# disanda/Deep-GAN-Encoders

Hardware: AMD Instinct MI355X
Metric: encoder-train images/sec (E_align_s2 step, StyleGAN2 FFHQ-1024) (higher is better)
Workload: dtype bf16; 1 GPU; E_align_s2 two-phase step, StyleGAN2-1024 G (train mode) + BE(startf=16, L=9) + LPIPS-VGG16 (seeded stand-in weights), batch 8/GPU; global_batch=8, img_size=1024, parallelism=dp1

## Files before the change

### deep-gan-encoders_amd/_lib.py

```python
import ctypes as C
import os

_HERE = os.path.dirname(os.path.abspath(__file__))
LIB_PATH = os.environ.get("DGE_LIB_PATH", os.path.join(_HERE, "libdge_hip.so"))


class DgeError(RuntimeError):
    pass


class ConvDesc(C.Structure):
    _fields_ = [
        ("x", C.c_void_p), ("w_packed", C.c_void_p), ("y", C.c_void_p), ("addend", C.c_void_p), ("dot_src", C.c_void_p),
        ("in_scale", C.c_void_p), ("in_shift", C.c_void_p), ("out_scale", C.c_void_p),
        ("bias", C.c_void_p), ("noise", C.c_void_p), ("noise_w", C.c_void_p), ("stats", C.c_void_p),
        ("B", C.c_int), ("H", C.c_int), ("W", C.c_int), ("Cin", C.c_int), ("Cout", C.c_int),
        ("ksize", C.c_int), ("up", C.c_int), ("in_s2d", C.c_int), ("noise_batch", C.c_int), ("noise_w_per_channel", C.c_int),
        ("act", C.c_int), ("bias_scale", C.c_float), ("gain", C.c_float), ("add_scale", C.c_float),
        ("dtype", C.c_int), ("in_up2", C.c_int), ("in_relu", C.c_int), ("stats_slots", C.c_int), ("w_layout", C.c_int),
        ("prep", C.c_int), ("prep_gain", C.c_float), ("prep_noise", C.c_void_p), ("prep_ns", C.c_void_p), ("prep_noise_batch", C.c_int),
        ("prep_stats", C.c_void_p), ("mask_relu", C.c_int), ("in_t2d", C.c_int),
        ("rgb_w", C.c_void_p), ("rgb_style", C.c_void_p), ("rgb_bias", C.c_void_p), ("rgb_out", C.c_void_p), ("rgb_wscale", C.c_float),
        ("rgb_skip_y", C.c_int), ("pool_out", C.c_int), ("pool_mask", C.c_void_p),
        ("prefetch_w", C.c_void_p), ("prefetch_ntot", C.c_int), ("prefetch_cin", C.c_int), ("in_bwd_coef", C.c_void_p),
        ("in_bwd_extra", C.c_void_p), ("in_bwd_extra_scale", C.c_float), ("fr_img4", C.c_void_p), ("fr_out", C.c_void_p),
    ]


class ConvPPDesc(C.Structure):
    _fields_ = [
        ("x", C.c_void_p), ("w_pp", C.c_void_p), ("y", C.c_void_p), ("w_bstride", C.c_longlong),
        ("out_scale", C.c_void_p), ("bias", C.c_void_p), ("noise", C.c_void_p), ("noise_w", C.c_void_p),
        ("B", C.c_int), ("H", C.c_int), ("W", C.c_int), ("Cin", C.c_int), ("Cout", C.c_int),
        ("noise_batch", C.c_int), ("noise_w_per_channel", C.c_int), ("act", C.c_int), ("bias_scale", C.c_float), ("gain", C.c_float),
        ("dgrad", C.c_int), ("in_s2d", C.c_int), ("stats_slots", C.c_int), ("prep", C.c_int), ("prep_noise_batch", C.c_int), ("mask_relu", C.c_int),
        ("in_t2d", C.c_int), ("add_scale", C.c_float), ("prep_gain", C.c_float),
        ("dot_src", C.c_void_p), ("addend", C.c_void_p), ("stats", C.c_void_p), ("prep_stats", C.c_void_p), ("prep_noise", C.c_void_p), ("prep_ns", C.c_void_p),
    ]


class DenseLayer(C.Structure):
    _fields_ = [("w", C.c_void_p), ("bias", C.c_void_p), ("I", C.c_int), ("O", C.c_int), ("wscale", C.c_float), ("bscale", C.c_float),
                ("add", C.c_float), ("act", C.c_int), ("gain", C.c_float)]


class S2GradEntry(C.Structure):
    _fields_ = [("P", C.c_void_p), ("st", C.c_void_p), ("d", C.c_void_p), ("s", C.c_void_p), ("bias", C.c_void_p), ("wsq", C.c_void_p),
                ("gs", C.c_void_p), ("wstyle", C.c_void_p),
                ("nslot_p", C.c_int), ("nslot_s", C.c_int), ("in_c", C.c_int), ("out_c", C.c_int), ("row", C.c_int), ("bscale", C.c_float)]


class SumPlanarEntry(C.Structure):
    _fields_ = [("partial", C.c_void_p), ("out", C.c_void_p), ("nslot", C.c_int), ("C", C.c_int), ("NS", C.c_int), ("pad", C.c_int)]


class NoisePlan(C.Structure):
    _fields_ = [("maps", C.c_void_p), ("jobs", C.c_void_p), ("nmaps", C.c_int), ("Bn", C.c_int), ("n_pool0", C.c_int), ("n_pool1", C.c_int),
                ("n_mom", C.c_int), ("npairs", C.c_int), ("n_chunk", C.c_int), ("pad", C.c_int), ("n_total", C.c_longlong),
                ("lev_total", C.c_longlong)]


_P, _I, _F = C.c_void_p, C.c_int, C.c_float
SIGNATURES = {
    "dge_conv2d": [C.POINTER(ConvDesc), _P],
    "dge_fir_t2d": [_P, _P, _P, _I, _I, _I, _I, _I, _P],
    "dge_up_dgrad_small": [C.POINTER(ConvDesc), _P],
    "dge_up_dgrad_small_supported": [_I, _I, _I, _I, _I, _I],
    "dge_s2_style_grads": [C.POINTER(S2GradEntry), _I, _P, _I, _I, _I, _F, _P],
    "dge_conv_small_supported": [_I, _I, _I, _I, _I, _I, _I, _I],
    "dge_torgb_bwd_prep": [_P, _P, _P, _P, _P, _P, _I, _P, _P, _P, _I, _I, _I, _F, _F, _I, _P],
    "dge_demod_bwd_prep": [_P, _I, _P, _P, _P, _I, _I, _F, _P],
    "dge_sum_slots": [_P, _P, _I, _I, _I, _P],
    "dge_sum_slots_planar": [_P, _P, _I, _I, _I, _P],
    "dge_set_deterministic": [_I],
    "dge_get_deterministic": [],
    "dge_packed_n": [_I],
    "dge_pack_conv_weight": [_P, _P, _I, _I, _I, _I, _I, _F, _P],
    "dge_pack_conv_weights_multi": [_P, _P, _I, _I, _P],
    "dge_pack_desc_bytes": [],
    "dge_weight_sumsq": [_P, _P, _I, _I, _I, _F, _P],
    "dge_linear": [_P, _I, _P, _P, _P, _I, _I, _I, _I, _F, _F, _F, _I, _F, _I, _P],
    "dge_pixelnorm": [_P, _P, _I, _I, _F, _P],
    "dge_truncation": [_P, _P, _P, _I, _I, _I, _F, _I, _I, _P],
    "dge_torgb": [_P, _P, _P, _P, _P, _P, _I, _I, _I, _I, _F, _I, _P],
    "dge_conv_rgb_supported": [_I, _I, _I, _I, _I, _I, _I],
    "dge_conv_in_bwd_supported": [_I, _I, _I, _I, _I, _I, _I],
    "dge_conv_in_bwd_fromrgb_supported": [_I, _I, _I, _I, _I, _I, _I],
    "dge_conv_in_bwd_x_supported": [_I, _I, _I, _I, _I, _I, _I],
    "dge_conv_pool_supported": [_I, _I, _I, _I, _I, _I, _I],
    "dge_rgb_upsample_add": [_P, _P, _I, _I, _I, _P],
    "dge_nchw_to_nhwc": [_P, _P, _I, _I, _I, _I, _I, _P],
    "dge_nhwc_to_nchw": [_P, _P, _I, _I, _I, _I, _P],
    "dge_fromrgb": [_P, _P, _P, _P, _P, _I, _I, _I, _I, _P],
    "dge_fromrgb2": [_P, _P, _P, _P, _P, _P, _I, _I, _I, _I, _P],
    "dge_stats_finalize": [_P, _P, _P, _P, _I, _I, _I, _F, _P],
    "dge_stats_finalize_slots": [_P, _I, _P, _P, _P, _I, _I, _I, _F, _P],
    "dge_blend": [_P, _P, _P, _P, _P, _P, _I, _I, _I, _I, _I, _F, _F, _I, _P],
    "dge_loss_reduce": [_P, _P, _P, _I, _I, _I, _I, _I, _I, _I, _I, _P],
    "dge_ssim_fwd": [_P, _P, _P, _P, _I, _I, _I, _P],
    "dge_ssim_box7": [_P, _P, _P, _I, _I, _I, _F, _F, _F, _P],
    "dge_ssim_bwd": [_P, _P, _P, _P, _I, _I, _I, _F, _I, _P],
    "dge_space_loss_finalize": [_P, _P, _P, _P, _F, _F, _I, _P],
    "dge_space_loss_bwd": [_P, _P, _P, _P, _P, _I, _I, _I, _I, _I, _I, _I, _I, _F, _F, _I, _P],
    "dge_axpy_scalar": [_P, _P, _P, C.c_long, _F, _I, _P],
    "dge_lreq_adam_multi": [_I, _P, _P, _P, _P, _P, _F, _F, _P, _P, _P],
    "dge_modconv_bwd_prep": [_P, _P, _P, _P, _P, _P, _I, _I, _I, _I, _F, _I, _P],
    "dge_demod_bwd": [_P, _P, _P, _P, _P, _I, _I, _F, _P],
    "dge_linear_t": [_P, _I, _I, _P, _P, _P, _I, _I, _I, _I, _I, _F, _I, _P],
    "dge_torgb_bwd": [_P, _P, _P, _P, _P, _P, _I, _I, _I, _F, _I, _P],
    "dge_up2_bwd": [_P, _P, _I, _I, _I, _P],
    "dge_conv_wgrad": [_P, _P, _P, _P, _P, _I, _I, _I, _I, _I, _I, _I, _P],
    "dge_act_bwd": [_P, _P, _P, _P, _P, _I, _I, _I, _I, _I, _I, _F, _F, _I, _P],
    "dge_in_bwd_coef": [_P, _P, _P, _P, _P, _P, _I, _I, _I, _P],
    "dge_in_bwd_coef_slots": [_P, _I, _P, _P, _P, _P, _P, _I, _I, _I, _P],
    "dge_in_bwd": [_P, _P, _P, _P, _P, _P, _P, _I, _I, _I, _I, _I, _F, _I, _I, _P],
    "dge_chan_sum": [_P, _P, _I, _I, _I, _F, _I, _P],
    "dge_fromrgb_bwd": [_P, _P, _P, _P, _I, _I, _I, _I, _P],
    "dge_head_entry_size": [],
    "dge_heads_bwd": [_P, _I, _I, _P, _I, _P, _P, _P, _P, _I, _I, _P],
    "dge_head_rows_entry_size": [],
    "dge_heads_rows_fwd": [_P, _I, _P, _P, C.c_long, C.c_long, _I, _I, _I, _P],
    "dge_heads_rows_bwd": [_P, _I, _I, _P, C.c_long, C.c_long, _I, _P, _P, _P, _P, _I, _I, _P],
    "dge_dense_wgrad": [_P, _I, _P, _I, _P, _P, _I, _I, _I, _I, _P],
    "dge_lpips_prep": [_P, _P, _I, _I, _I, _P, _P, _I, _P],
    "dge_lpips_prep_bwd": [_P, _P, _I, _I, _I, _P, _F, _I, _I, _P],
    "dge_maxpool2": [_P, _P, _I, _I, _I, _I, _I, _P],
    "dge_maxpool2_bwd": [_P, _P, _P, _P, _I, _I, _I, _I, _I, _P],
    "dge_lpips_head": [_P, _P, _P, _P, _I, _I, _I, _F, _I, _P],
    "dge_mean": [_P, _P, _I, _P],
    "dge_blur_noise_act": [_P, _P, _P, _P, _P, _P, _I, _I, _I, _I, _I, _I, _I, _I, _P],
    "dge_affine_compose": [_P, _P, _P, _P, _P, _I, _I, _P],
    "dge_lerp_layers": [_P, _P, _I, _P, _P, _I, _I, _I, _P],
    "dge_linear_rows": [_P, _I, _P, _P, _P, _P, _P, _P, _I, _I, _I, _F, _F, _F, _P],
    "dge_demod_rows": [_P, _P, _P, _P, _P, _P, _P, _P, _I, _I, _F, _P],
    "dge_fromrgb_dgrad": [_P, _P, _P, _P, _I, _I, _I, _I, _P],
    "dge_nearest_up2": [_P, _P, _I, _I, _I, _I, _F, _I, _P],
    "dge_sg1_in_bwd_coef": [_P, _P, _P, _P, _P, _P, _I, _I, _I, _P],
    "dge_dot_stats": [_P, _P, _P, _I, _I, _I, _I, _P],
    "dge_nearest_up2_bwd": [_P, _P, _P, _P, _I, _I, _I, _I, _I, _P],
# ... 4 lines not shown
    "dge_slice_up_bwd": [_P, _P, _I, _I, _I, _I, _I, _I, _I, _P],
    "dge_softmax_rows": [_P, C.c_long, _I, _I, _P],
    "dge_softmax_rows_bwd": [_P, _P, C.c_long, _I, _I, _P],
    "dge_rgb_tanh_bwd": [_P, _P, _P, _I, _I, _I, _I, _P],
    "dge_sn_group": [_P, _I, _I, _I, _P, _F, _I, _P],
    "dge_sn_entry_size": [],
    "dge_cbn_sn_wgrad_entry_size": [],
    "dge_cbn_sn_wgrad_group": [_P, _I, C.c_longlong, _I, _P, _I, _I, _P, _P],
    "dge_upconv_supported": [_I, _I, _I],
    "dge_pack_upconv_weight": [_P, _P, _I, _I, _F, _I, _P],
    "dge_upconv_fir": [_P, _P, _P, _P, _P, _P, _I, _P, _I, _P, _F, _F, _I, _I, _I, _I, _I, _I, _I, _P],
    "dge_up_dgrad_stream_supported": [_I, _I, _I, _I, _I, _I],
    "dge_up_dgrad_stream": [_P, _P, _P, _P, _P, _P, _P, _P, _I, _I, _F, _P, _I, _P, _P, _I, _I, _I, _I, _I, _I, _P],
    "dge_cbn_affine": [_P, _P, _I, _P, _P, _F, _P, _P, _I, _I, _P],
    "dge_slice_up": [_P, _P, _I, _I, _I, _I, _I, _I, _I, _P],
    "dge_attention": [_P, _P, _P, _P, _I, _I, _I, _I, _I, _I, _P],
    "dge_rgb_tanh": [_P, _P, _I, _I, _I, _I, _P],
    "dge_guided_relu_bwd": [_P, _P, _P, C.c_long, _I, _I, _P],
    "dge_maxpool2_relu_bwd": [_P, _P, _P, _I, _I, _I, _I, _I, _I, _P],
    "dge_maxpool2_bwd_relu": [_P, _P, _P, _P, _I, _I, _I, _I, _I, _P],
    "dge_adaptive_pool7": [_P, _P, _I, _I, _I, _I, _I, _P],
    "dge_adaptive_pool7_bwd": [_P, _P, _I, _I, _I, _I, _I, _P],
    "dge_class_target": [_P, _P, _P, _P, _I, _I, _P],
    "dge_gather_row": [_P, _P, _P, _I, _I, _F, _P],
    "dge_class_target_rows": [_P, _P, _P, _P, _I, _I, _P],
    "dge_gather_rows": [_P, _P, _P, _I, _I, _P],
    "dge_campp_map": [_P, _P, _P, _P, _P, _I, _I, _I, _I, _I, _P],
    "dge_cam_resize": [_P, _P, _P, _I, _I, _I, _I, _I, _P],
    "dge_mask2cam_blocks": [_I],
    "dge_mask2cam": [_P, _P, _P, _P, _P, _P, _P, _I, _I, _P],
    "dge_mask2cam_rows": [_P, _P, _P, _P, _P, _P, _I, _I, _P],
    "dge_class_target_groups": [_P, _P, _P, _P, _I, _I, _I, _P],
    "dge_gather_row_groups": [_P, _P, _P, _I, _I, _I, _F, _P],
    "dge_mask2cam_groups": [_P, _P, _P, _P, _P, _P, _P, _I, _I, _I, _P],
    "dge_randn": [_P, _I, _P, _P, _P, _P, C.c_ulonglong, _P, _P],
    "dge_version": [],
    "dge_env_reload": [],
    "dge_blend_pool_mask": [_P, _P, _P, _P, _P, _I, _I, _I, _I, _F, _F, _I, _P],
    "dge_act_bwd_mask": [_P, _P, _P, _P, _P, _I, _I, _I, _I, _I, _F, _F, _I, _P],
    "dge_loss_reduce3": [_P, _P, _P, _I, _I, _I, _I, _P, _I, _P],
    "dge_crop_pool_multi": [_P, _P, _P, _P, _I, _I, _I, _I, _P],
    "dge_space_loss_bwd3": [_P, _P, _P, _P, _P, _I, _I, _I, _P, _P, _P, _P, _I, _P],
    "dge_space_loss_bwd_split": [_P, _P, _P, _P, _P, _I, _I, _I, _P, _P, _P, _P, _I, _P],
    "dge_in_bwd_fromrgb": [_P, _P, _P, _I, _P, _P, _P, _P, _I, _P, _P, _P, _I, _I, _I, _I, _I, _F, _I, _P],
    "dge_in_bwd_fromrgb_img": [_P, _P, _P, _I, _P, _P, _P, _P, _I, _P, _P, _P, _P, _P, _I, _I, _I, _I, _I, _F, _I, _P],
    "dge_affine_bwd_fromrgb_img": [_P, _P, _P, _P, _P, _P, _P, _P, _I, _I, _I, _I, _I, _F, _I, _P],
    "dge_in_bwd_fused": [_P, _P, _P, _I, _P, _P, _P, _P, _I, _P, _P, _P, _P, _I, _I, _I, _I, _I, _F, _I, _I, _P],
    "dge_sum_slots_planar_multi": [C.POINTER(SumPlanarEntry), _I, _P],
    "dge_heads_fwd": [_P, _I, _P, _P, _I, _I, _I, _P],
    "dge_conv_pp_supported": [_I, _I, _I, _I, _I, _I],
    "dge_pack_conv_pp": [_P, _P, _I, _I, _F, _P, _P, _F, _I, _I, _P],
    "dge_dense_chain": [_P, _I, C.POINTER(DenseLayer), _I, _P, _I, _I, _I, _F, _P],
    "dge_conv_wgrad_dots": [_P, _P, _P, _P, _P, _P, _P, _I, _I, _I, _I, _I, _I, _I, _P],
    "dge_pack_conv_pp_rows": [_P, _I, _P, _I, _I, _P, _I, _P, _F, _I, _I, _P],
    "dge_conv_pp": [C.POINTER(ConvPPDesc), _P],
    "dge_up_pp_supported": [_I, _I, _I, _I, _I, _I],
    "dge_pack_up_pp": [_P, _P, _I, _I, _P, _P, _F, _I, _P],
    "dge_up_pp": [_P, _P, C.c_longlong, _P, _P, _I, _P, _P, _F, _F, _I, _I, _I, _I, _I, _I, _P],
    "dge_latent_pnorm_fwd": [_P, _P, _P, C.c_long, _I, _P],
    "dge_latent_pnorm_bwd": [_P, _P, _P, _P, C.c_long, _I, _F, _P],
    "dge_wplus_lerp": [_P, _P, _I, _F, _P, _I, _I, _I, _P],
    "dge_wplus_lerp_bwd": [_P, _F, _P, C.c_long, _I, _P],
    "dge_embed_track": [_P, _P, _P, C.c_long, _P, _P, _P, _P, _P, _I, _I, _I, _F, _F, _P],
    "dge_loss_reduce_rows": [_P, _P, _P, _I, _I, _I, _I, _P, _I, _I, _P],
    "dge_ssim_fwd_rows": [_P, _P, _P, _P, _I, _I, _I, _P],
    "dge_space_loss_finalize_rows": [_P, _I, _P, _P, _P, _P, _P, _I, _I, _P, _P, _I, _P],
    "dge_space_loss_bwd_rows": [_P, _P, _P, _P, _P, _I, _I, _I, _I, _P, _P, _P, _P, _I, _I, _P],
    "dge_latent_pnorm_rows_fwd": [_P, _P, _P, _I, C.c_long, _I, _P],
    "dge_latent_pnorm_rows_bwd": [_P, _P, _P, _P, _I, C.c_long, _I, _F, _P],
    "dge_embed_track_rows": [_P, _P, _P, _I, C.c_long, _P, _P, _P, _P, _P, _I, _I, _I, _F, _F, _P],
    "dge_mapping_bwd": [_P, _I, C.POINTER(DenseLayer), _I, _P, _P, _I, _P, _P, _I, _I, _I, _F, _P],
    "dge_mapping_bwd_wide_work_bytes": [_I],
    "dge_mapping_bwd_wide": [_P, _I, C.POINTER(DenseLayer), _I, _P, _P, _I, _P, _P, _I, _I, _I, _F, _P, C.c_longlong, _P],
    "dge_quantize_u8": [_P, _I, _P, _I, _I, _I, _I, _P],
    "dge_image_metrics_u8_work_bytes": [_I, _I, _I],
    "dge_image_metrics_u8": [_P, _P, _I, _I, _I, _P, _P, _P, _P, _P],
    "dge_minmax_unit_slots": [C.c_long],
    "dge_minmax_unit": [_P, _P, C.c_long, _P, _P],
    "dge_s2_noise_grad": [_P, _P, _P, _P, _I, _I, _I, _I, _F, _I, _I, _P],
    "dge_noise_map_size": [],
    "dge_noise_job_size": [],
    "dge_noise_reg_work_bytes": [C.POINTER(NoisePlan)],
    "dge_noise_reg": [C.POINTER(NoisePlan), _P, _P, _P, _F, _I, _P, C.c_longlong, _P],
    "dge_noise_normalize_work_bytes": [C.POINTER(NoisePlan)],
    "dge_noise_normalize": [C.POINTER(NoisePlan), _P, _P, C.c_longlong, _P],
    "dge_adam_multi": [_I, _P, _P, _P, _P, _P, C.c_double, C.c_double, _F, _F, _F, _P, _P],
    "dge_w_broadcast": [_P, _P, _F, _P, _P, _I, _I, _I, _P],
    "dge_w_broadcast_bwd": [_P, _P, _I, _I, _I, _P],
    "dge_rows_mean_std_work_bytes": [C.c_longlong, _I],
    "dge_rows_mean_std": [_P, C.c_longlong, _I, _P, _P, _P, C.c_longlong, _P],
    "dge_area_pool_bwd": [_P, _P, _I, _I, _I, _I, _P],
}

_lib = None


def lib():
    global _lib
    if _lib is None:
        if not os.path.exists(LIB_PATH):
            raise DgeError(f"{LIB_PATH} is missing: build it with deep-gan-encoders_amd/csrc/build.sh "
                           "(__graft_entry__.build()). There is no fallback path.")
        _lib = C.CDLL(LIB_PATH)
        for name, args in SIGNATURES.items():
            fn = getattr(_lib, name)
            fn.argtypes = args
# ... 19 lines not shown
```

### deep-gan-encoders_amd/autograd_enc_bwd.py

```python
import os
from types import SimpleNamespace

import torch

from . import ops
from .enc_steps import blocks, conv_bwd, grads_in_order, heads_backward, red_param_grads, skip_bwd
from .weight_cache import pack_cache, packed

FUSE_IN_BWD = not os.environ.get("DGE_NO_FUSED_IN_BWD")
FUSE_IMG_GRAD = not os.environ.get("DGE_NO_FUSED_IMG_GRAD")

FROMRGB, BLOCK_INPUT, SEPARATE = "FromRGB reduction", "block input", "separate passes"


def _conv2_part(c, blk, rec, pre, Cc, C2, H, g_out, gms2):
    B, dev, dt, grads, params = c.B, c.dev, c.dt, c.grads, c.params
    x1 = rec["x1"]
    extra, extra_pool, extra_scale = None, False, 1.0
    g_pre2 = g_y2 = dots2 = None
    fuse2 = False
    if blk.has_last_conv:
        has3 = Cc != C2
        red2 = ops.zeros((3 if has3 else 2, C2), dev) if params else None
        g_pre2 = ops.act_bwd_mask(g_out, rec["m2"], rec["n2"], scale=0.111 * 0.25, red=red2, planar=True, defer=c.later)
        sum_g = red_param_grads(grads, pre, 2, red2, planar=True) if params else None
        gW2 = ops.zeros(tuple(blk.conv_2.weight.shape), dev) if params else None
        dots2 = ops.SlotStats(B, Cc, dev)
        if params and FUSE_IN_BWD and ops.conv_in_bwd_supported(B, H, H, C2, Cc, dt):
            fuse2 = ops.conv_wgrad_dots(g_pre2, x1, gW2, rec["sc2"], rec["sh2"], blk.conv_2.weight, dots2)
        if fuse2:
            grads[pre + "conv_2.weight"] = gW2
        else:
            g_y2, _ = conv_bwd(c.cache, grads, pre + "conv_2", blk.conv_2, g_pre2, x1, dt, H, rec["sc2"], rec["sh2"], params, dots=dots2,
                               dw=gW2)
        if has3:
            extra = skip_bwd(c.cache, grads, pre, blk, g_out, rec["xp"], dt, sum_g, params, post=c.post)
            extra_pool, extra_scale = True, 0.25
        else:
            extra, extra_pool, extra_scale = g_out, True, 0.889 * 0.25
    elif g_out is not None:
        if Cc != C2:
            raise ops.DgeError("E.BE: a gradient on the const output of a last block with a channel change (conv_3 on the unpooled "
                               "input) is not implemented; not reachable with maxf-clamped widths")
        g_y2 = ops.blend(g_out, alpha=0.111)
        dots2 = ops.dot_stats(g_y2, x1)
        extra, extra_pool, extra_scale = g_out, False, 0.889
    coef2 = (dots2, gms2, rec["musig2"], rec["sc2"], rec["sh2"], H * H)
    red1 = ops.zeros((2, Cc), dev) if params else None
    if fuse2:
        redp = ops.SlotStats(B, Cc, dev)
        g_pre1 = ops.conv2d(g_pre2, packed(c.cache, blk.conv_2, dt, ops.PACK_DGRAD, H), Cc, 3, dot_src=x1,
                            in_bwd=dict(coef=ops.in_bwd_coef(*coef2), noise=rec["n1"].reshape(B, H, H), red=redp))
        ops._sum_planar(redp.buf.view(-1, Cc, 2), red1, c.later)
    else:
        g_pre1 = ops.in_bwd(g_y2, x1, coef2, noise=rec["n1"], act=True, red=red1, planar=True, defer=c.later)
    if params:
        red_param_grads(grads, pre, 1, red1, planar=True)
    return g_pre1, extra, extra_pool, extra_scale


def _conv1_form(c, j, Cc, H, extra, extra_pool):
    if not FUSE_IN_BWD or not c.params:
        return SEPARATE
    if j == 0 and c.need_img:
        return SEPARATE
    if j == 0:
        ok = c.saved.get("img4") is not None and ops.conv_in_bwd_fromrgb_supported(c.B, H, H, Cc, Cc, c.dt)
        return FROMRGB if ok else SEPARATE
    ok = (extra is None or extra_pool) and ops.conv_in_bwd_x_supported(c.B, H, H, Cc, Cc, c.dt)
    return BLOCK_INPUT if ok else SEPARATE


def _img_grad_fused(c, Cc):
    return FUSE_IMG_GRAD and ops.in_bwd_fromrgb_img_supported(Cc, c.dt)


def _conv1_part(c, j, blk, rec, pre, Cc, H, g_pre1, gms1, extra, extra_pool, extra_scale):
    B, dev, dt, grads = c.B, c.dev, c.dt, c.grads
    x = rec["x"]
    gW1 = ops.zeros(tuple(blk.conv_1.weight.shape), dev) if c.params else None
    dots1 = ops.SlotStats(B, Cc, dev)
    form = _conv1_form(c, j, Cc, H, extra, extra_pool)
    if form != SEPARATE:
        covered = ops.conv_wgrad_dots(g_pre1, x, gW1, rec["sc1"], rec["sh1"], blk.conv_1.weight, dots1)
        if covered:
            grads[pre + "conv_1.weight"] = gW1
        else:
            form = SEPARATE
    coef1 = (dots1, gms1, rec["musig1"], rec["sc1"], rec["sh1"], H * H)
    if form == FROMRGB:
        frh = ops.SlotStats(B, Cc, dev)
        ops.conv2d(g_pre1, packed(c.cache, blk.conv_1, dt, ops.PACK_DGRAD, H), Cc, 3, dot_src=x, out=x.new_empty((1, 1, 1, 1)),
                   in_bwd=dict(coef=ops.in_bwd_coef(*coef1), fr=frh, img4=c.saved["img4"], extra=extra if extra_pool else None,
                               extra_scale=extra_scale))
        return None, ops._sum_planar(frh.buf.view(-1, Cc, 4), torch.empty((4, Cc), dtype=torch.float32, device=dev), c.later)
    if form == BLOCK_INPUT:
        return ops.conv2d(g_pre1, packed(c.cache, blk.conv_1, dt, ops.PACK_DGRAD, H), Cc, 3, dot_src=x,
                          in_bwd=dict(coef=ops.in_bwd_coef(*coef1), extra=extra, extra_scale=extra_scale)), None
    g_y1, _ = conv_bwd(c.cache, grads, pre + "conv_1", blk.conv_1, g_pre1, x, dt, H, rec["sc1"], rec["sh1"], c.params, dots=dots1, dw=gW1)
    if j == 0 and c.need_img and _img_grad_fused(c, Cc):
        c.g_img, fr = ops.in_bwd_fromrgb_img(g_y1, x, coef1, c.E.FromRGB.from_rgb.weight.detach(), c.saved["img"].float() if c.params else None,
                                             extra=extra, extra_pool=extra_pool, extra_scale=extra_scale, defer=c.later)
        return None, fr
    if j == 0 and Cc <= 512 and c.params and not c.need_img:
        return None, ops.in_bwd_fromrgb(g_y1, x, coef1, c.saved["img"].float(), extra=extra, extra_pool=extra_pool,
# ... 48 lines not shown
```

### deep-gan-encoders_amd/csrc/capi.hip

```cpp
#include <stdarg.h>
#include <stdio.h>
#include "common.h"
#include "conv_params.h"
#include "../../include/dge_hip.h"

static thread_local char g_err[512] = "";
void dge_set_error(const char* fmt, ...) {
    va_list ap; va_start(ap, fmt); vsnprintf(g_err, sizeof(g_err), fmt, ap); va_end(ap);
}
extern "C" const char* dge_last_error(void) { return g_err; }
static thread_local char g_kernel[160] = "";
void dge_note_kernel(const char* fmt, ...) {
    va_list ap; va_start(ap, fmt); vsnprintf(g_kernel, sizeof(g_kernel), fmt, ap); va_end(ap);
}
extern "C" const char* dge_last_kernel(void) { return g_kernel; }
extern "C" int dge_version(void) { return 100; }

#include <vector>
static std::vector<void (*)(const DgeDet*)>& det_setters() { static std::vector<void (*)(const DgeDet*)> v; return v; }
void dge_det_register(void (*setter)(const DgeDet*)) { det_setters().push_back(setter); }
static DgeDet g_det_host = {0, nullptr, nullptr, 0, 0};
int dge_det_upload_failed = 0;
bool dge_det_fits(long long ndomains, long long nslots, long long L) {
    return !g_det_host.enabled || (ndomains * nslots * L <= g_det_host.ws_floats && ndomains <= (long long)g_det_host.ncounters);
// ... 41 lines not shown
}
#include <mutex>
static std::once_flag g_env_once;
const DgeEnv& dge_env() { std::call_once(g_env_once, [] { if (!g_env_loaded) env_load(); }); return g_env; }
extern "C" void dge_env_reload(void) { env_load(); }

static int conv_desc_to_params(const dge_conv_desc* d, ConvParams& p, bool units) {
    DGE_CHECK(d && d->x && d->w_packed && d->y, "conv2d: null tensor");
    DGE_CHECK(d->B > 0 && d->H > 0 && d->W > 0 && d->Cin > 0 && d->Cout > 0, "conv2d: bad shape");
    DGE_CHECK(d->dtype == DGE_F32 || d->dtype == DGE_BF16, "conv2d: bad dtype %d", d->dtype);
    DGE_CHECK(!(d->up && d->stats), "conv2d: stats are not available in up mode");
    DGE_CHECK(!(d->up && d->in_s2d), "conv2d: up and in_s2d are exclusive");
    DGE_CHECK(!d->in_up2 || (!d->in_s2d && d->H % 2 == 0 && d->W % 2 == 0), "conv2d: in_up2 needs even H, W and no in_s2d");
    DGE_CHECK(!d->in_s2d || d->Cin % 4 == 0, "conv2d: in_s2d needs Cin %% 4 == 0");
    DGE_CHECK(!d->dot_src || d->stats || d->mask_relu || d->in_bwd_coef, "conv2d: dot_src needs a stats buffer");
    DGE_CHECK(!d->mask_relu || (d->dot_src && !d->prep && !d->up), "conv2d: mask_relu needs dot_src and excludes prep / up");
    DGE_CHECK(!d->in_relu || d->in_scale || d->in_shift, "conv2d: in_relu is applied together with the prologue affine");
    DGE_CHECK(d->gain > 0.f, "conv2d: gain must be positive (it is folded through the activation)");
    DGE_CHECK((((uintptr_t)d->in_scale | (uintptr_t)d->in_shift) & 15) == 0, "conv2d: in_scale/in_shift must be 16-byte aligned");
    DGE_CHECK(!d->noise || d->noise_w, "conv2d: noise without noise_w");
    p.x = d->x; p.w = d->w_packed; p.y = d->y; p.addend = d->addend; p.dot_src = d->dot_src;
    p.in_scale = d->in_scale; p.in_shift = d->in_shift; p.out_scale = d->out_scale;
    p.bias = d->bias; p.noise = d->noise; p.noise_w = d->noise_w; p.stats = d->stats;
    p.B = d->B; p.H = d->H; p.W = d->W; p.Cin = d->Cin; p.Cout = d->Cout;
    p.Ntot_valid = d->up ? 4 * d->Cout : d->Cout;
    p.Ntot = dge_packed_n(p.Ntot_valid);
    p.up = d->up; p.in_s2d = d->in_s2d; p.in_up2 = d->in_up2; p.in_relu = d->in_relu;
    const int OH = d->up ? 2 * d->H : d->H, OW = d->up ? 2 * d->W : d->W;
    p.noise_bstride = d->noise_batch > 1 ? OH * OW : 0;
    p.noise_w_stride = d->noise_w_per_channel ? 1 : 0;
    p.act = d->act; p.bias_scale = d->bias_scale; p.gain = d->gain; p.add_scale = d->add_scale;
    p.tiles_x = p.tiles_y = 0;
    p.w_frag = d->w_layout == 1 ? 1 : 0;
    p.prep = d->prep ? 1 : 0;
    p.mask_relu = d->mask_relu ? 1 : 0;
    p.in_t2d = d->in_t2d ? 1 : 0;
    DGE_CHECK(!d->in_t2d || (d->ksize == 3 && !d->up && !d->in_s2d && !d->in_up2 && !d->in_scale && !d->in_shift && (d->w_layout == 0 || units)),
              "conv2d: in_t2d is a plain 3x3 launch (no other read mode, no prologue affine, row-major weights)");
    p.prep_gain = d->prep_gain; p.prep_noise = d->prep_noise; p.prep_ns = d->prep_ns; p.prep_stats = d->prep_stats;
    p.prep_noise_bstride = d->prep_noise_batch > 1 ? OH * OW : 0;
    DGE_CHECK(!d->prep || (d->dot_src && d->prep_stats && d->prep_gain > 0.f && !d->up), "conv2d: prep needs dot_src, prep_stats, a positive prep_gain and no up mode");
    DGE_CHECK(!d->prep || !dge_get_deterministic(), "conv2d: the fused tail backward (prep) is not offered in deterministic mode; run dge_modconv_bwd_prep");
    DGE_CHECK(d->w_layout == 0 || d->w_layout == 1, "conv2d: bad w_layout %d", d->w_layout);
    p.stats_slots = d->stats_slots > 0 ? d->stats_slots : 1;
    p.rgb_w = d->rgb_out ? d->rgb_w : nullptr; p.rgb_style = d->rgb_style; p.rgb_bias = d->rgb_bias; p.rgb_out = d->rgb_out;
    p.rgb_wscale = d->rgb_wscale; p.rgb_skip_y = (d->rgb_out && d->rgb_skip_y) ? 1 : 0;
    p.pool_out = d->pool_out ? 1 : 0; p.pool_mask = d->pool_out ? (unsigned*)d->pool_mask : nullptr;
    const bool pf = d->w_layout == 1 && d->prefetch_w && d->prefetch_ntot >= 64 && d->prefetch_ntot % 64 == 0 &&
                    (d->prefetch_cin == 512 || d->prefetch_cin == 256);
    p.pf_w = pf ? d->prefetch_w : nullptr; p.pf_ntot = pf ? d->prefetch_ntot : 0; p.pf_cin = pf ? d->prefetch_cin : 0;
    p.in_coef = d->in_bwd_coef;
    p.in_extra = d->in_bwd_coef ? d->in_bwd_extra : nullptr; p.in_extra_scale = d->in_bwd_extra_scale;
    p.fr_img4 = d->in_bwd_coef ? d->fr_img4 : nullptr; p.fr_out = d->in_bwd_coef ? d->fr_out : nullptr;
    if (d->in_bwd_coef) {
        DGE_CHECK(!dge_get_deterministic(), "conv2d: in_bwd_coef is not offered in deterministic mode; run dge_in_bwd");
        DGE_CHECK(d->ksize == 3 && !d->up && dge_conv_stream_eligible(p, d->dtype, d->ksize), "conv2d: in_bwd_coef is offered where "
                  "dge_conv_in_bwd_supported() says so, with dot_src and prep_stats, without stats / prep");
    }
    if (d->pool_out)
        DGE_CHECK(!d->up && dge_conv_pool_ok(p, d->dtype, d->ksize), "conv2d: the pooled epilogue is offered where dge_conv_pool_supported() "
                  "says so (conv_2 of the first encoder blocks on the streaming kernel)");
    if (d->rgb_out) {
        DGE_CHECK(d->rgb_w && d->rgb_style && d->rgb_bias, "conv2d: rgb_out needs rgb_w, rgb_style, rgb_bias");
        DGE_CHECK(dge_conv_rgb_ok(p, d->dtype, d->ksize), "conv2d: the fused toRGB is offered where dge_conv_rgb_supported() says so "
                  "(bf16 3x3 32 -> 32 launches of the streaming kernel)");
    }
    return 0;
}

extern "C" int dge_conv2d(const dge_conv_desc* d, hipStream_t s) {
    ConvParams p;
    if (const int rc = conv_desc_to_params(d, p, false)) return rc;
    return dge_conv_launch(p, d->dtype, d->ksize, s);
}

extern "C" int dge_up_dgrad_small(const dge_conv_desc* d, hipStream_t s) {
    DGE_CHECK(d && d->in_t2d && d->w_layout == 1 && d->ksize == 3 && d->Cin % 4 == 0, "up_dgrad_small: an in_t2d launch with fragment-ordered unit weights");
    DGE_CHECK(!d->bias && !d->noise && d->act == DGE_ACT_NONE && !d->mask_relu && !d->in_bwd_coef && !d->rgb_out && !d->pool_out && !d->in_relu,
              "up_dgrad_small: data-gradient epilogue only (out_scale, addend, dot_src + stats, prep)");
    DGE_CHECK(dge_up_dgrad_small_supported(d->B, d->H, d->W, d->Cin / 4, d->Cout, d->dtype),
              "up_dgrad_small: unsupported launch %dx%d, %d <- %d channels, dtype %d", d->H, d->W, d->Cout, d->Cin / 4, d->dtype);
    ConvParams p;
    if (const int rc = conv_desc_to_params(d, p, true)) return rc;
    p.Cin = d->Cin / 4;
    return dge_up_dgrad_small_launch(p, s);
}

extern "C" int dge_conv_pool_supported(int B, int H, int W, int Cin, int Cout, int ksize, int dtype) {
    ConvParams p = {};
    p.B = B; p.H = H; p.W = W; p.Cin = Cin; p.Cout = Cout; p.Ntot_valid = Cout; p.Ntot = dge_packed_n(Cout);
    p.in_shift = (const float*)16; p.noise_w_stride = 1;
    return dge_conv_pool_ok(p, dtype, ksize) ? 1 : 0;
}

extern "C" int dge_conv_in_bwd_supported(int B, int H, int W, int Cin, int Cout, int ksize, int dtype) {
    ConvParams p = {};
    p.B = B; p.H = H; p.W = W; p.Cin = Cin; p.Cout = Cout; p.Ntot_valid = Cout; p.Ntot = dge_packed_n(Cout);
    p.dot_src = (const void*)16; p.prep_stats = (float*)16; p.in_coef = (const float*)16;
    return (ksize == 3 && !dge_get_deterministic() && dge_conv_stream_eligible(p, dtype, ksize)) ? 1 : 0;
}
extern "C" int dge_conv_in_bwd_x_supported(int B, int H, int W, int Cin, int Cout, int ksize, int dtype) {
    ConvParams p = {};
    p.B = B; p.H = H; p.W = W; p.Cin = Cin; p.Cout = Cout; p.Ntot_valid = Cout; p.Ntot = dge_packed_n(Cout);
    p.dot_src = (const void*)16; p.in_coef = (const float*)16;
    return (ksize == 3 && !dge_get_deterministic() && dge_conv_stream_eligible(p, dtype, ksize)) ? 1 : 0;
}
extern "C" int dge_conv_in_bwd_fromrgb_supported(int B, int H, int W, int Cin, int Cout, int ksize, int dtype) {
    ConvParams p = {};
    p.B = B; p.H = H; p.W = W; p.Cin = Cin; p.Cout = Cout; p.Ntot_valid = Cout; p.Ntot = dge_packed_n(Cout);
    p.dot_src = (const void*)16; p.in_coef = (const float*)16; p.fr_img4 = (const float*)16; p.fr_out = (float*)16;
    return (ksize == 3 && !dge_get_deterministic() && dge_conv_stream_eligible(p, dtype, ksize)) ? 1 : 0;
}

extern "C" int dge_conv_rgb_supported(int B, int H, int W, int Cin, int Cout, int ksize, int dtype) {
    ConvParams p = {};
    p.B = B; p.H = H; p.W = W; p.Cin = Cin; p.Cout = Cout; p.Ntot_valid = Cout; p.Ntot = dge_packed_n(Cout);
    return dge_conv_rgb_ok(p, dtype, ksize) ? 1 : 0;
}

__global__ void sum_slots_kernel(const float* __restrict__ partial, float* __restrict__ out, int nslot, int n, int accumulate) {
    const int i = blockIdx.x * blockDim.x + threadIdx.x;
    if (i >= n) return;
    float s = 0.f;
    int k = 0;
    for (; k + 8 <= nslot; k += 8) {
        float v[8];
#pragma unroll
        for (int j = 0; j < 8; j++) v[j] = partial[(size_t)(k + j) * n + i];
#pragma unroll
        for (int j = 0; j < 8; j++) s += v[j];
    }
    for (; k < nslot; k++) s += partial[(size_t)k * n + i];
    out[i] = accumulate ? out[i] + s : s;
}
__global__ void sum_slots_planar_kernel(const float* __restrict__ partial, float* __restrict__ out, int nslot, int C, int NS) {
    const int i = blockIdx.x * blockDim.x + threadIdx.x;
    if (i >= C * NS) return;
    float s = 0.f;
    int k = 0;
    for (; k + 8 <= nslot; k += 8) {
        float v[8];
#pragma unroll
        for (int j = 0; j < 8; j++) v[j] = partial[(size_t)(k + j) * C * NS + i];
#pragma unroll
        for (int j = 0; j < 8; j++) s += v[j];
    }
    for (; k < nslot; k++) s += partial[(size_t)k * C * NS + i];
    out[(size_t)(i % NS) * C + i / NS] = s;
}
extern "C" int dge_sum_slots_planar(const float* partial, float* out, int nslot, int C, int NS, hipStream_t s) {
    DGE_CHECK(nslot >= 1 && C >= 1 && NS >= 1, "sum_slots_planar: bad sizes");
    hipLaunchKernelGGL(sum_slots_planar_kernel, dim3((C * NS + 255) / 256), dim3(256), 0, s, partial, out, nslot, C, NS);
    DGE_LAUNCH_CHECK("sum_slots_planar");
// ... 40 lines not shown
```

### deep-gan-encoders_amd/csrc/conv_params.h

```cpp
#pragma once
#include <hip/hip_runtime.h>

struct ConvParams {
    const void* x;
    const void* w;
    void* y;
    const void* addend;
    const void* dot_src;
    const float* in_scale;
    const float* in_shift;
    const float* out_scale;
    const float* bias;
    const float* noise;
    const float* noise_w;
    float* stats;
    int stats_slots;
    int B, H, W, Cin, Cout;
    int Ntot;
    int Ntot_valid;
    int up;
    int in_s2d;
    int in_relu;
    int in_up2;
    int noise_bstride;
    int noise_w_stride;
    int act;
    float bias_scale, gain, add_scale;
    int tiles_x, tiles_y;
    int dbg;
    int w_frag;
    int prep;
    float prep_gain;
    const float* prep_noise;
    const float* prep_ns;
    int prep_noise_bstride;
    float* prep_stats;
    int mask_relu;
    int in_t2d;
    const float* rgb_w;
    const float* rgb_style;
    const float* rgb_bias;
    float* rgb_out;
    float rgb_wscale;
    int rgb_skip_y;
    int pool_out;
    unsigned* pool_mask;
    const void* pf_w;
    int pf_ntot, pf_cin;
    const float* in_coef;
    const void* in_extra; float in_extra_scale; const float* fr_img4; float* fr_out;
};

int dge_conv_launch(const ConvParams& p, int dtype, int ksize, hipStream_t s);
extern "C" int dge_conv_ntile(int ntot);

bool dge_conv_stream_eligible(const ConvParams& p, int dtype, int ksize);
int dge_conv_stream_launch(const ConvParams& p, hipStream_t s);
bool dge_conv_rgb_ok(const ConvParams& p, int dtype, int ksize);
bool dge_conv_pool_ok(const ConvParams& p, int dtype, int ksize);
bool dge_conv_small_shape_ok(int H, int W, int cin, int ntot, int ksize, int in_s2d, int in_up2, int dtype);
int dge_conv_small_launch(const ConvParams& p, hipStream_t s);
extern "C" int dge_up_dgrad_small_supported(int B, int H, int W, int C, int N, int dtype);
int dge_up_dgrad_small_launch(const ConvParams& p, hipStream_t s);
bool dge_conv_pw_eligible(const ConvParams& p, int dtype, int ksize);
int dge_conv_pw_launch(const ConvParams& p, hipStream_t s);
```

### deep-gan-encoders_amd/csrc/conv_stream.hip

```cpp
#include <type_traits>
#include "common.h"
#include <stdlib.h>
#include "conv_params.h"

namespace {

typedef __attribute__((ext_vector_type(4))) unsigned rsrc_t;
#define DGE_LDS " lds\n\t"

__device__ __forceinline__ unsigned rfl(unsigned v) { return __builtin_amdgcn_readfirstlane(v); }
__device__ __forceinline__ unsigned lds_off(const void* p) {
    return (unsigned)(size_t)(const __attribute__((address_space(3))) unsigned char*)p;
}
constexpr int ilog2(int v) { return v <= 1 ? 0 : 1 + ilog2(v >> 1); }

__device__ __forceinline__ rsrc_t make_rsrc(unsigned long long base, unsigned bytes) {
    rsrc_t r;
    r[0] = rfl((unsigned)base); r[1] = rfl((unsigned)(base >> 32) & 0xffffu); r[2] = rfl(bytes); r[3] = 0x00020000u;
    return r;
}

#define DGE_P(off) "buffer_load_dwordx4 %1, %3, 0 offen offset:" #off " lds\n\t"
#define DGE_PB(off) "buffer_load_dwordx4 %4, %3, 0 offen offset:" #off " lds\n\t"
#define DGE_M0 "s_mov_b32 m0, %2\n\ts_nop 0\n\t"
#define DGE_MASK(m) "s_mov_b64 %0, exec\n\ts_mov_b64 exec, " #m "\n\t"
#define DGE_UNMASK "s_mov_b64 exec, %0"
template <int CIN, int TEAM>
__device__ __forceinline__ void dma_row(int wave, unsigned voff, unsigned voff_b, unsigned voff_c, rsrc_t rs, rsrc_t rs_null,
                                        unsigned m0v, unsigned m0_dummy) {
    unsigned long long keep;
    if constexpr (CIN == 16 && TEAM == 1) {
        asm volatile(DGE_M0 DGE_P(0) DGE_MASK(0xf) DGE_P(1024) DGE_UNMASK : "=&s"(keep) : "v"(voff), "s"(m0v), "s"(rs) : "memory");
    } else if constexpr (CIN == 16 && TEAM == 2) {
        if (wave == 0) asm volatile(DGE_M0 DGE_P(0) : "=&s"(keep) : "v"(voff), "s"(m0v), "s"(rs) : "memory");
        else asm volatile(DGE_M0 DGE_MASK(0xf) DGE_P(1024) DGE_UNMASK : "=&s"(keep) : "v"(voff), "s"(m0v), "s"(rs) : "memory");
    } else if constexpr (CIN == 32 && TEAM == 1) {
        asm volatile(DGE_M0 DGE_P(0) DGE_P(1024) DGE_MASK(0xff) DGE_P(2048) DGE_UNMASK : "=&s"(keep) : "v"(voff), "s"(m0v), "s"(rs) : "memory");
    } else if constexpr (CIN == 32 && TEAM == 2) {
        if (wave == 0) asm volatile(DGE_M0 DGE_P(0) DGE_MASK(0xff) DGE_P(2048) DGE_UNMASK : "=&s"(keep) : "v"(voff), "s"(m0v), "s"(rs) : "memory");
        else asm volatile(DGE_M0 DGE_P(1024) "s_mov_b32 m0, %5\n\ts_nop 0\n\tbuffer_load_dwordx4 %1, %4, 0 offen lds"
                          : "=&s"(keep) : "v"(voff), "s"(m0v), "s"(rs), "s"(rs_null), "s"(m0_dummy) : "memory");
    } else if constexpr (CIN == 64 && TEAM == 1) {
        asm volatile(DGE_M0 DGE_P(0) DGE_PB(1024) DGE_P(2048) DGE_PB(3072)
                     "s_mov_b32 m0, %6\n\t" DGE_MASK(0xffff) "buffer_load_dwordx4 %5, %3, 0 offen lds\n\t" DGE_UNMASK
                     : "=&s"(keep) : "v"(voff), "s"(m0v), "s"(rs), "v"(voff_b), "v"(voff_c), "s"(m0v + 4096u) : "memory");
    } else {
        if (wave == 0)
            asm volatile(DGE_M0 DGE_P(0) DGE_P(2048)
                         "s_mov_b32 m0, %5\n\t" DGE_MASK(0xffff) "buffer_load_dwordx4 %4, %3, 0 offen lds\n\t" DGE_UNMASK
                         : "=&s"(keep) : "v"(voff), "s"(m0v), "s"(rs), "v"(voff_c), "s"(m0v + 4096u) : "memory");
        else
            asm volatile(DGE_M0 DGE_P(1024) DGE_P(3072) "s_mov_b32 m0, %5\n\ts_nop 0\n\tbuffer_load_dwordx4 %1, %4, 0 offen lds"
                         : "=&s"(keep) : "v"(voff_b), "s"(m0v), "s"(rs), "s"(rs_null), "s"(m0_dummy) : "memory");
    }
}
__device__ __forceinline__ void dma_piece(unsigned voff, rsrc_t rs, unsigned m0v) {
    asm volatile("s_mov_b32 m0, %1\n\ts_nop 0\n\tbuffer_load_dwordx4 %0, %2, 0 offen lds" : : "v"(voff), "s"(m0v), "s"(rs) : "memory");
}
template <int NP> __device__ __forceinline__ void dma_dot(unsigned voff, unsigned voff1, rsrc_t rs, unsigned m0v) {
    if constexpr (NP == 1)
        asm volatile("s_mov_b32 m0, %1\n\ts_nop 0\n\tbuffer_load_dwordx4 %0, %2, 0 offen lds" : : "v"(voff), "s"(m0v), "s"(rs) : "memory");
    else
        asm volatile("s_mov_b32 m0, %1\n\ts_nop 0\n\tbuffer_load_dwordx4 %0, %2, 0 offen lds\n\t"
                     "buffer_load_dwordx4 %3, %2, 0 offen offset:1024 lds" : : "v"(voff), "s"(m0v), "s"(rs), "v"(voff1) : "memory");
}

enum { FL_GEN = 0, FL_ENC = 1, FL_ENC_STATS = 2, FL_DOT = 3, FL_DOT_PREP = 4, FL_GEN_RGB = 5, FL_ENC_POOL = 6, FL_DOT_IN = 7, FL_DOT_FR = 8, FL_DOT_INX = 9 };

template <int CIN, int COUT, int FL>
struct SC {
    static constexpr int PXB = CIN * 2, CH = PXB / 16, LOGCH = ilog2(CH), KS = CIN / 16;
    static constexpr int TEAM = COUT == 64 ? 2 : 1;
    static constexpr int TPW = 4 / TEAM;
    static constexpr int MT = COUT / 32 > 0 ? COUT / 32 : 1;
    static constexpr int MTW = MT / TEAM;
    static constexpr int HW = 34, RB = HW * PXB;
    static constexpr int PIECES = (RB + 1023) / 1024;
    static constexpr bool PREP = FL == FL_DOT_PREP, RGB = FL == FL_GEN_RGB, POOL = FL == FL_ENC_POOL, FRB = FL == FL_DOT_FR, INX = FL == FL_DOT_INX, INB = FL == FL_DOT_IN || FRB || INX;
    static_assert(!RGB || COUT == 32 || (COUT == 64 && TEAM == 2), "fused toRGB: 32 output channels per wave, one wave or a 2-wave team per pixel");
    static constexpr bool DOT = FL == FL_DOT || PREP || INB, STATS = FL == FL_ENC_STATS, ENC = FL == FL_ENC || FL == FL_ENC_STATS || POOL;
    static constexpr bool NOISE = !DOT || PREP || (INB && !FRB && !INX);
    static constexpr int NR = 6;
    static constexpr int dot_depth(int nr) { for (int d = 4; d >= 1; d--) if (d <= nr - 3 && nr % (d + 1) == 0) return d; return 1; }
    static constexpr int D = DOT ? dot_depth(6) : 2;
    static constexpr int DR = DOT ? D + 1 : NR;
    static_assert(NR % DR == 0, "dot ring period");
    static constexpr int CPB = COUT * 2;
    static constexpr int CW = COUT / TEAM >= 32 ? 32 : 16;
    static constexpr int DCH = CW * MTW * 2 / 16;
    static constexpr int LOGDCH = ilog2(DCH);
    static constexpr int DROWB = 32 * DCH * 16, DPIECES = DROWB / 1024;
    static_assert(!DOT || MTW == 1, "data-gradient mode: one M tile per wave");
    static constexpr int XPW = TEAM == 2 ? (PIECES + 1) / 2 : PIECES;
    static constexpr int LPR = XPW + (DOT ? DPIECES : 0) + (FRB ? 2 : 0) + (INX ? 1 : 0);
    static constexpr int X_OFF = 0;
    static constexpr int XRING = NR * RB;
    static constexpr int N_OFF = (XRING + 1023) / 1024 * 1024;
    static constexpr int NRING = NOISE ? 2048 : 0;
    static_assert(NR <= 8, "a noise piece holds 8 rows");
    static constexpr int D_OFF = N_OFF + TEAM * NRING;
    static constexpr int DRING = DOT ? DR * DROWB : 0;
    static constexpr int E_OFF = D_OFF + TEAM * DRING;
    static constexpr int ERING = FRB ? 2 * DR * 512 : (INX ? DR * 1024 : 0);
    static_assert(!INX || (CIN == COUT && CIN >= 32), "block-input flavour: 32 -> 32, 64 -> 64");
    static_assert(!FRB || (CIN == 16 && COUT == 16 && TEAM == 1), "FromRGB reduction flavour: 16 -> 16");
    static constexpr int T_OFF = E_OFF + TEAM * ERING;
    static constexpr int TBYTES = 32 * MTW * 16 * 4;
    static constexpr int DUMMY_OFF = T_OFF + TEAM * TBYTES;
    static constexpr int RGBX_OFF = DUMMY_OFF + (TEAM == 2 ? 1024 : 0);
    static constexpr int LDS_BYTES = RGBX_OFF + (RGB && TEAM == 2 ? 1024 : 0);
    static constexpr int NEED = 4 * 9 * KS * MTW + 32 * MTW + 16 + (ENC ? 16 * MTW : 0) + (STATS || DOT ? 32 * MTW : 0) + (DOT ? 16 : 0) + (PREP ? 16 : 0) + (RGB ? 11 : 0) + (POOL ? 20 * MTW : 0) + 36;
    static constexpr int WPE = ((PREP || INB) && CIN == 64) ? 1 : (NEED <= 128 ? 4 : (NEED <= 168 ? 3 : 2));
    static_assert(D <= NR - 3, "the slot of the row being fetched must be dead");
    static_assert((D - 1) * LPR + 1 < 64, "vmcnt range");
};

template <int LOGC> __device__ __forceinline__ int chunk_swz(int px) { return (px >> (4 - LOGC)) & ((1 << LOGC) - 1); }

template <int CW> __device__ __forceinline__ int chan_of_row(int m) {
    const int j = m >> 3, k = (m >> 2) & 1, i = m & 3;
    if (CW == 16) return j < 2 ? 8 * k + 4 * j + i : -1;
    return 16 * (j >> 1) + 8 * k + 4 * (j & 1) + i;
}

template <int CIN, int COUT, int FL>
__global__ __launch_bounds__((64 * SC<CIN, COUT, FL>::TEAM * SC<CIN, COUT, FL>::TPW), (SC<CIN, COUT, FL>::WPE))
void conv_stream_kernel(ConvParams p, int nstrips, int nseg, int seg_rows, int njobs, int jobs_per_xcd) {
    using C = SC<CIN, COUT, FL>;
    extern __shared__ __attribute__((aligned(1024))) unsigned char lds_all[];
#ifdef DGE_SC_TIMING
    const long long tj0 = __builtin_readcyclecounter();
#endif
    const int lane = threadIdx.x & 63;
    const int wid = (int)rfl(threadIdx.x >> 6);
    const int team = wid / C::TEAM;
    const int wave = wid % C::TEAM;
    unsigned char* __restrict__ lds = lds_all + team * C::LDS_BYTES;
    const unsigned lds0 = lds_off(lds_all) + team * C::LDS_BYTES;
    const int n31 = lane & 31, kh = lane >> 5;

    int job = ((blockIdx.x & 7) * jobs_per_xcd + (blockIdx.x >> 3)) * C::TPW + team;
    if ((blockIdx.x >> 3) >= jobs_per_xcd || job >= njobs) return;
    const int strip = job % nstrips; job /= nstrips;
    const int seg = job % nseg;
    const int b = job / nseg;
    const int x0 = strip * 32;
    const int r0 = seg * seg_rows;
    const int rows = min(seg_rows, p.H - r0);
    const bool full_strip = x0 + 32 <= p.W;
    const bool edge_strip = x0 == 0 || x0 + 32 >= p.W;

    const unsigned xrow_bytes = (unsigned)p.W * C::PXB, yrow_bytes = (unsigned)p.W * C::CPB;
    const unsigned long long Xb = (unsigned long long)p.x + (unsigned long long)b * p.H * xrow_bytes;
    unsigned char* __restrict__ Yb = (unsigned char*)p.y + (size_t)b * p.H * yrow_bytes;
    const float* __restrict__ nzsrc = (C::PREP || C::INB) ? p.prep_noise : p.noise;
    const unsigned long long NZb = nzsrc ? (unsigned long long)(nzsrc + (size_t)b * ((C::PREP || C::INB) ? p.prep_noise_bstride : p.noise_bstride)) : Xb;
    const unsigned nzrow_bytes = nzsrc ? (unsigned)p.W * 4 : 0;
    const unsigned long long DOTb = C::DOT ? (unsigned long long)p.dot_src + (unsigned long long)b * p.H * yrow_bytes : Xb;

    unsigned voff, voff_b = 0, voff_c = 0;
    {
        const int px = lane >> C::LOGCH, cs = lane & (C::CH - 1);
        const int gx = x0 - 1 + px;
        voff = (unsigned)(gx * C::PXB + ((cs ^ chunk_swz<C::LOGCH>(px)) << 4));
        if constexpr (CIN == 64) {
            voff_b = (unsigned)(gx * C::PXB + ((cs ^ chunk_swz<C::LOGCH>(px + 8)) << 4));
            voff_c = voff + 4096;
        }
    }
    const unsigned nvoff = (unsigned)(((lane >> 3) * p.W + x0 + (lane & 7) * 4) * 4);
    unsigned dvoff = 0, dvoff1 = 0;
    if constexpr (C::DOT) {
        const int px = lane >> C::LOGDCH, cs = lane & (C::DCH - 1);
        const int chunk0 = wave * 4;
        dvoff = (unsigned)((x0 + px) * C::CPB + ((chunk0 + (cs ^ chunk_swz<C::LOGDCH>(px))) << 4));
        constexpr int PPP = 64 / C::DCH;
        dvoff1 = (unsigned)((x0 + px + PPP) * C::CPB + ((chunk0 + (cs ^ chunk_swz<C::LOGDCH>(px + PPP))) << 4)) - 1024u;
    }
    const rsrc_t rs_null = make_rsrc(Xb, 0);
    const unsigned exrow_bytes = (C::FRB || C::INX) ? (unsigned)(p.W >> 1) * C::CPB : 0u, imrow_bytes = C::FRB ? (unsigned)p.W * 16u : 0u;
    const unsigned long long EXb = ((C::FRB || C::INX) && p.in_extra) ? (unsigned long long)p.in_extra + (unsigned long long)b * (p.H >> 1) * exrow_bytes : Xb;
    const unsigned long long IMb = C::FRB ? (unsigned long long)p.fr_img4 + (unsigned long long)b * p.H * imrow_bytes : Xb;
    const unsigned evoff = C::INX ? (unsigned)(((x0 >> 1) + (lane >> 2)) * C::CPB + wave * 64 + (((lane & 3) ^ chunk_swz<2>(lane >> 2)) << 4))
                                  : (unsigned)((x0 >> 1) * 32 + (lane & 31) * 16);
    const unsigned ivoff = (unsigned)((x0 + (lane & 31)) * 16);

    unsigned long long xptr = Xb + (unsigned long long)(long long)(r0 - 1) * xrow_bytes;
    unsigned long long dptr = DOTb + (unsigned long long)(long long)(r0 - 2) * yrow_bytes;
    auto issue = [&](int h, int slot, int slot_d) {
        const int gy = r0 - 1 + h;
        const bool xv = (unsigned)gy < (unsigned)p.H && h <= rows + 1;
        const rsrc_t rx = make_rsrc(xptr, xv ? xrow_bytes : 0u);
        xptr += xrow_bytes;
        const unsigned m0x = lds0 + C::X_OFF + slot * C::RB;
        dma_row<CIN, C::TEAM>(wave, voff, voff_b, voff_c, rx, rs_null, m0x, lds0 + C::DUMMY_OFF);
        const bool ov = h >= 2 && h <= rows + 1;
        if constexpr (C::DOT) {
            const rsrc_t rd = make_rsrc(dptr, ov ? yrow_bytes : 0u);
            dptr += yrow_bytes;
            dma_dot<C::DPIECES>(dvoff, dvoff1, rd, lds0 + C::D_OFF + wave * C::DRING + slot_d * C::DROWB);
        }
        if constexpr (C::INX) {
            const int oy = gy - 1;
            const rsrc_t re = make_rsrc(EXb + (unsigned long long)(ov ? (oy >> 1) : 0) * exrow_bytes, (ov && p.in_extra) ? exrow_bytes : 0u);
            dma_piece(evoff, re, lds0 + C::E_OFF + wave * C::ERING + slot_d * 1024);
        }
        if constexpr (C::FRB) {
            const int oy = gy - 1;
            const rsrc_t re = make_rsrc(EXb + (unsigned long long)(ov ? (oy >> 1) : 0) * exrow_bytes, (ov && p.in_extra) ? exrow_bytes : 0u);
            const rsrc_t ri = make_rsrc(IMb + (unsigned long long)(ov ? oy : 0) * imrow_bytes, ov ? imrow_bytes : 0u);
            unsigned long long keep;
            asm volatile(DGE_MASK(0xffffffff) "s_mov_b32 m0, %2\n\ts_nop 0\n\tbuffer_load_dwordx4 %1, %3, 0 offen lds\n\t"
                         "s_mov_b32 m0, %4\n\ts_nop 0\n\tbuffer_load_dwordx4 %5, %6, 0 offen lds\n\t" DGE_UNMASK
                         : "=&s"(keep) : "v"(evoff), "s"(lds0 + C::E_OFF + slot_d * 512), "s"(re), "s"(lds0 + C::E_OFF + C::DR * 512 + slot_d * 512), "v"(ivoff), "s"(ri) : "memory");
        }
    };
    auto issue_noise = [&](int q, unsigned buf_off) {
        const int gy = r0 + q;
        const bool v = nzsrc != nullptr && gy < p.H && q < rows;
        const rsrc_t rn = make_rsrc(NZb + (unsigned long long)(v ? gy : 0) * nzrow_bytes, v ? (unsigned)(p.H - gy) * nzrow_bytes : 0u);
        dma_piece(nvoff, rn, lds0 + C::N_OFF + wave * C::NRING + buf_off);
    };
    asm volatile("s_waitcnt vmcnt(0)" ::: "memory");
    if constexpr (C::NOISE) issue_noise(0, 0u);
    StaticFor<C::D + 2>::run([&](auto hc) { constexpr int h = decltype(hc)::value; issue(h, h % C::NR, (h + C::NR - 2) % C::NR % C::DR); });

    uint4 wf[C::MTW][9][C::KS];
    float* __restrict__ TT = (float*)(lds + C::T_OFF + wave * C::TBYTES);
    {
        const bf16_t* __restrict__ Wp = (const bf16_t*)p.w;
        float sc[C::KS][8], rt[C::KS][8];
#pragma unroll
        for (int ks = 0; ks < C::KS; ks++) {
            const int k0 = ks * 16 + kh * 8;
#pragma unroll
            for (int e = 0; e < 8; e++) {
                sc[ks][e] = p.in_scale ? p.in_scale[b * CIN + k0 + e] : 1.f;
                const float sh = (C::ENC && p.in_shift) ? p.in_shift[b * CIN + k0 + e] : 0.f;
                rt[ks][e] = sc[ks][e] != 0.f ? sh / sc[ks][e] : 0.f;
            }
        }
#pragma unroll
        for (int mt = 0; mt < C::MTW; mt++) {
            const int cl = chan_of_row<C::CW>(n31);
            const int o = (wave * C::MTW + mt) * 32 + cl;
            const bool ov = cl >= 0 && o < COUT;
            float osc = p.gain;
            if (!C::DOT && p.out_scale && ov) osc *= p.out_scale[b * COUT + o];
            if (C::INB && ov) osc *= p.in_coef[((size_t)b * COUT + o) * 3];
            const int oc = ov ? o : 0;
            float c_bias = (!C::DOT && p.bias) ? p.bias[oc] : 0.f;
            float c_nw = (C::NOISE && p.noise) ? p.noise_w[oc * p.noise_w_stride] : 0.f;
            float c_osc = (C::DOT && !C::INB && p.out_scale) ? p.out_scale[b * COUT + oc] : 1.f;
            float c_in1 = 0.f, c_in2 = 0.f;
            if constexpr (C::INB) { c_in1 = p.in_coef[((size_t)b * COUT + oc) * 3 + 1]; c_in2 = p.in_coef[((size_t)b * COUT + oc) * 3 + 2]; }
            float tall = 0.f, tleft = 0.f, tright = 0.f;
            {
                const bf16_t* __restrict__ wrow = Wp + (size_t)(ov ? o : 0) * CIN + kh * 8;
#pragma unroll
                for (int tap = 0; tap < 9; tap++)
#pragma unroll
                    for (int ks = 0; ks < C::KS; ks++) wf[mt][tap][ks] = *(const uint4*)(wrow + (size_t)tap * p.Ntot * CIN + ks * 16);
            }
#pragma unroll
            for (int tap = 0; tap < 9; tap++) {
                float tt = 0.f;
#pragma unroll
                for (int ks = 0; ks < C::KS; ks++) {
                    uint4 v = ov ? wf[mt][tap][ks] : make_uint4(0, 0, 0, 0);
                    float f[8];
                    unpack16(v, f, (bf16_t*)nullptr);
#pragma unroll
                    for (int e = 0; e < 8; e++) f[e] *= sc[ks][e] * osc;
                    v = pack16(f, (bf16_t*)nullptr);
                    if constexpr (C::ENC) {
                        unpack16(v, f, (bf16_t*)nullptr);
#pragma unroll
                        for (int e = 0; e < 8; e++) tt += f[e] * rt[ks][e];
                    }
                    wf[mt][tap][ks] = v;
                }
                if constexpr (C::ENC) {
                    tt += __shfl_xor(tt, 32, 64);
                    if (kh == 0 && ov) TT[(mt * 32 + cl) * 16 + tap] = tt;
                    tall += tt;
                    if (tap % 3 == 0) tleft += tt;
                    if (tap % 3 == 2) tright += tt;
                }
            }
            if (kh == 0 && ov) {
                const int e = (mt * 32 + cl) * 16;
                float bb = (!C::DOT && p.bias) ? c_bias * p.bias_scale * p.gain : 0.f;
                if constexpr (C::ENC) { TT[e + 9] = tall; TT[e + 10] = tleft; TT[e + 11] = tright; bb += tall; }
                if constexpr (C::INB) bb = c_in2;
                TT[e + 12] = bb;
                TT[e + 13] = (C::NOISE && p.noise) ? c_nw * p.gain : 0.f;
                TT[e + 14] = C::INB ? c_in1 : c_osc;
            }
        }
    }
    auto chan_of_reg = [&](int mt, int r) { return mt * 32 + (C::CW == 16 ? 8 * kh + r : 16 * (r >> 3) + 8 * kh + (r & 7)); };
    constexpr int NREG = C::CW == 16 ? 8 : 16;
    f32x16_t biasv[C::MTW], zero16;
#pragma unroll
    for (int r = 0; r < 16; r++) zero16[r] = 0.f;
    float nwv[C::MTW][C::ENC ? 16 : 1], oscv[C::DOT ? 16 : 1];
#pragma unroll
    for (int mt = 0; mt < C::MTW; mt++)
#pragma unroll
        for (int r = 0; r < 16; r++) {
            const bool live = r < NREG;
            biasv[mt][r] = live ? TT[chan_of_reg(mt, r) * 16 + 12] : 0.f;
            if constexpr (C::ENC) nwv[mt][r] = live ? TT[chan_of_reg(mt, r) * 16 + 13] : 0.f;
            if constexpr (C::DOT) oscv[r] = live ? TT[chan_of_reg(mt, r) * 16 + 14] : 0.f;
            if constexpr (C::ENC) {
                const int gxl = x0 + n31;
                if (live && edge_strip && (gxl == 0 || gxl == p.W - 1)) {
                    const float* __restrict__ T = TT + chan_of_reg(mt, r) * 16;
                    biasv[mt][r] -= (gxl == 0 ? T[10] : 0.f) + (gxl == p.W - 1 ? T[11] : 0.f);
                }
            }
        }
    const float nw_uniform = (!C::ENC && C::NOISE && p.noise) ? p.noise_w[0] * p.gain : 0.f;
    const float slope = p.act == DGE_ACT_LRELU ? 0.2f : (p.act == DGE_ACT_RELU ? 0.f : 1.f);

    uint4 rgbA[C::RGB ? 2 : 1];
    float rgbb[3] = {0.f, 0.f, 0.f};
    if constexpr (C::RGB) {
        const int row = n31 & 7, part = n31 >> 3;
        const bool live = row < 3 && part < 2;
#pragma unroll
        for (int ks = 0; ks < 2; ks++) {
            float f[8];
#pragma unroll
            for (int e = 0; e < 8; e++) {
                const int c = wave * 32 + 16 * ks + 8 * kh + e;
                const float wv = live ? p.rgb_w[row * COUT + c] * p.rgb_wscale * p.rgb_style[b * COUT + c] : 0.f;
                const float hi = __uint_as_float(__float_as_uint(wv) & 0xffff0000u);
                f[e] = part == 0 ? hi : wv - hi;
            }
            rgbA[ks] = pack16(f, (bf16_t*)nullptr);
        }
#pragma unroll
        for (int k = 0; k < 3; k++) rgbb[k] = wave == 0 ? p.rgb_bias[k] : 0.f;
    }
    float rgbh[3] = {0.f, 0.f, 0.f};
    typedef __attribute__((address_space(3))) float* lds_wfp;
    auto rgb_flush = [&](int srow) {
        if (kh == 0 && x0 + n31 < p.W) {
            const unsigned a = lds0 + C::RGBX_OFF + (unsigned)(srow & 1) * 384 + n31 * 4;
            float* __restrict__ ro = p.rgb_out + ((size_t)b * 3 * p.H + (r0 + srow)) * p.W + x0 + n31;
            const size_t plane = (size_t)p.H * p.W;
#pragma unroll
// ... 4 lines not shown
    unsigned loff[3][C::KS];
#pragma unroll
    for (int dx = 0; dx < 3; dx++)
#pragma unroll
        for (int ks = 0; ks < C::KS; ks++) {
            const int px = n31 + dx;
            loff[dx][ks] = lds0 + C::X_OFF + px * C::PXB + (((ks * 2 + kh) ^ chunk_swz<C::LOGCH>(px)) << 4);
        }
    const unsigned nzoff = lds0 + C::N_OFF + wave * C::NRING + n31 * 4;
    unsigned doff[2] = {0, 0};
    if constexpr (C::DOT) {
#pragma unroll
        for (int q = 0; q < 2; q++)
            doff[q] = lds0 + C::D_OFF + wave * C::DRING + n31 * C::DCH * 16 + (((2 * q + kh) ^ chunk_swz<C::LOGDCH>(n31)) << 4);
    }
    typedef unsigned u32x4_t __attribute__((ext_vector_type(4)));
    typedef const __attribute__((address_space(3))) u32x4_t* lds_u4p;
    typedef const __attribute__((address_space(3))) float* lds_fp;
    auto lds_u4 = [&](unsigned a) { const u32x4_t t = *(lds_u4p)a; return make_uint4(t[0], t[1], t[2], t[3]); };
    auto lds_f = [&](unsigned a) { return *(lds_fp)a; };

    const int gx = x0 + n31;
    const bool pv = gx < p.W;
    const unsigned yoff = (unsigned)gx * C::CPB + (unsigned)(wave * C::MTW * 32 * 2) + kh * 16;
    const bool pool_lane = C::POOL && (n31 & 1) == 0 && pv;
    const unsigned py_voff = pool_lane ? (unsigned)(gx >> 1) * C::CPB + (unsigned)(wave * C::MTW * 64) + kh * 16 : 0x80000000u;
    const unsigned pm_voff = pool_lane ? ((unsigned)(gx >> 1) * (COUT / 8) + (unsigned)(wave * C::MTW * 4) + kh) * 4u : 0x80000000u;
    const unsigned pool_px = C::POOL ? (unsigned)(p.H >> 1) * (unsigned)(p.W >> 1) : 0u;
    const __amdgpu_buffer_rsrc_t rs_pool = __builtin_amdgcn_make_buffer_rsrc((unsigned char*)p.y + (size_t)b * pool_px * C::CPB, 0, (int)(pool_px * C::CPB), 0x00020000);
    const __amdgpu_buffer_rsrc_t rs_mask = __builtin_amdgcn_make_buffer_rsrc((C::POOL && p.pool_mask) ? (unsigned char*)p.pool_mask + (size_t)b * pool_px * (COUT / 8) * 4 : (unsigned char*)p.y, 0,
                                                                               (C::POOL && p.pool_mask) ? (int)(pool_px * (COUT / 8) * 4) : 0, 0x00020000);

    float s0[C::MTW][(C::STATS || C::DOT) ? 16 : 1], s1[C::MTW][(C::STATS || C::DOT) ? 16 : 1], s2[(C::PREP || C::INB) ? 16 : 1];
    if constexpr (C::STATS || C::DOT) {
#pragma unroll
        for (int mt = 0; mt < C::MTW; mt++)
#pragma unroll
            for (int r = 0; r < 16; r++) { s0[mt][r] = 0.f; s1[mt][r] = 0.f; }
    }
    if constexpr (C::PREP || C::INB) {
#pragma unroll
        for (int r = 0; r < 16; r++) s2[r] = 0.f;
    }
    float prow[C::POOL ? C::MTW : 1][C::POOL ? 16 : 1];
    unsigned psign[C::POOL ? C::MTW : 1];
    const float pg_pos = p.prep_gain, pg_neg = 0.2f * p.prep_gain, pz_pos = 1.f / p.prep_gain, pz_neg = 1.f / (0.2f * p.prep_gain);
    const float pns = (C::PREP && p.prep_noise && p.prep_ns) ? p.prep_ns[0] : 0.f;
    const float fr_es = (C::FRB || C::INX) ? p.in_extra_scale : 0.f;

#define DGE_T(k)
    auto step = [&](auto ic, int s, unsigned npar) {
        constexpr int I = decltype(ic)::value;
        DGE_T(0);
        constexpr int NAFTER = (C::D - 1) * C::LPR + ((C::NOISE && I >= 1 && I <= C::D - 1) ? 1 : 0);
        asm volatile("s_waitcnt vmcnt(%0)" :: "i"(NAFTER) : "memory");
        if constexpr (C::RGB && C::TEAM == 2) asm volatile("s_waitcnt lgkmcnt(0)" ::: "memory");
        if constexpr (C::TEAM == 2) __builtin_amdgcn_s_barrier();
        if constexpr (C::RGB && C::TEAM == 2) { if (wave == 0 && s > 0) rgb_flush(s - 1); }
        DGE_T(1);
        if constexpr (C::NOISE && I == 0) issue_noise(s + C::NR, npar ^ 1024u);
        issue(s + 2 + C::D, (I + 2 + C::D) % C::NR, (I + C::D) % C::DR);
        DGE_T(2);

        const int gy = r0 + s;
        constexpr int NQ = 9 * C::KS;
        constexpr int PF = NQ < 6 ? NQ : 6;
        auto frag_addr = [&](auto qc) {
            constexpr int q = decltype(qc)::value;
            constexpr int tap = q / C::KS, ks = q % C::KS, dy = tap / 3, dx = tap % 3;
            return loff[dx][ks] + (unsigned)(((I + dy) % C::NR) * C::RB);
        };
        float nz = 0.f;
        if constexpr (C::NOISE) nz = lds_f(nzoff + npar + I * 128);
        uint4 bq[PF];
        StaticFor<PF>::run([&](auto qc) { bq[decltype(qc)::value] = lds_u4(frag_addr(qc)); });
        f32x16_t acc[C::MTW];
        StaticFor<NQ>::run([&](auto qc) {
            constexpr int q = decltype(qc)::value;
            constexpr int tap = q / C::KS, ks = q % C::KS;
            const bf16x8_t bf = *(const bf16x8_t*)&bq[q % PF];
#pragma unroll
            for (int mt = 0; mt < C::MTW; mt++) {
                acc[mt] = __builtin_amdgcn_mfma_f32_32x32x16_bf16(*(const bf16x8_t*)&wf[mt][tap][ks], bf, q == 0 ? ((C::DOT && !C::INB) ? zero16 : biasv[mt]) : acc[mt], 0, 0, 0);
            }
            if constexpr (q + PF < NQ) bq[q % PF] = lds_u4(frag_addr(std::integral_constant<int, q + PF>{}));
        });

        __builtin_amdgcn_sched_group_barrier(0x100, PF + (C::NOISE ? 1 : 0), 0);
        StaticFor<NQ - PF>::run([&](auto) {
            __builtin_amdgcn_sched_group_barrier(0x008, C::MTW, 0);
            __builtin_amdgcn_sched_group_barrier(0x100, 1, 0);
        });
        __builtin_amdgcn_sched_group_barrier(0x008, PF * C::MTW, 0);
        DGE_T(3);
        unsigned char* __restrict__ yrow = Yb + (size_t)gy * yrow_bytes;
#pragma unroll
        for (int mt = 0; mt < C::MTW; mt++) {
            float v[16];
#pragma unroll
            for (int r = 0; r < 16; r++) v[r] = acc[mt][r];
            if constexpr (C::ENC) {
                const bool top = gy == 0, bot = gy == p.H - 1;
                if (top | bot) {
                    const float cl = gx == 0 ? 1.f : 0.f, cr = gx == p.W - 1 ? 1.f : 0.f;
#pragma unroll
                    for (int r = 0; r < NREG; r++) {
                        const float* __restrict__ T = TT + chan_of_reg(mt, r) * 16;
                        float corr = 0.f;
                        if (top) corr += T[0] + T[1] + T[2] - cl * T[0] - cr * T[2];
                        if (bot) corr += T[6] + T[7] + T[8] - cl * T[6] - cr * T[8];
                        v[r] -= corr;
                    }
                }
            }
            if constexpr (C::DOT) {
                uint4 dd[2];
                dd[0] = lds_u4(doff[0] + (I % C::DR) * C::DROWB);
                if constexpr (NREG == 16) dd[1] = lds_u4(doff[1] + (I % C::DR) * C::DROWB);
                const float nzs = C::PREP ? pns * nz : 0.f;
                float exf[8], exx[C::INX ? 2 : 1][8];
                if constexpr (C::INX) {
#pragma unroll
                    for (int q = 0; q < NREG / 8; q++)
                        unpack16(lds_u4(lds0 + C::E_OFF + wave * C::ERING + (I % C::DR) * 1024 + (n31 >> 1) * 64 + (((2 * q + kh) ^ chunk_swz<2>(n31 >> 1)) << 4)), exx[q], (bf16_t*)nullptr);
                }
                float4 fr_im = make_float4(0.f, 0.f, 0.f, 0.f);
                if constexpr (C::FRB) {
                    unpack16(lds_u4(lds0 + C::E_OFF + (I % C::DR) * 512 + (n31 >> 1) * 32 + kh * 16), exf, (bf16_t*)nullptr);
                    const uint4 t4 = lds_u4(lds0 + C::E_OFF + C::DR * 512 + (I % C::DR) * 512 + n31 * 16);
                    fr_im = make_float4(__uint_as_float(t4.x), __uint_as_float(t4.y), __uint_as_float(t4.z), __uint_as_float(t4.w));
                }
#pragma unroll
                for (int q = 0; q < NREG / 8; q++) {
                    float d[8];
                    unpack16(dd[q], d, (bf16_t*)nullptr);
#pragma unroll
                    for (int e = 0; e < 8; e++) {
                        const int r = 8 * q + e;
                        if constexpr (C::INX) {
                            v[r] = fmaf(fr_es, exx[C::INX ? q : 0][e], fmaf(oscv[r], d[e], v[r]));
                            continue;
                        }
                        if constexpr (C::FRB) {
                            const float gp = (fmaf(oscv[r], d[e], v[r]) + fr_es * exf[e]) * (d[e] > 0.f ? 1.f : 0.2f);
                            s0[0][r] = fmaf(gp, fr_im.x, s0[0][r]); s0[0][8 + r] = fmaf(gp, fr_im.y, s0[0][8 + r]);
                            s1[0][r] = fmaf(gp, fr_im.z, s1[0][r]); s1[0][8 + r] += gp;
// ... 160 lines not shown
                float va = 0.f, vc = 0.f, vt = 0.f;
#pragma unroll
                for (int r = 0; r < NREG; r++) {
                    float a = s0[mt][r], c = s1[mt][r], t2 = (C::PREP || C::INB) ? s2[r] : 0.f;
#pragma unroll
                    for (int m = 1; m < 32; m <<= 1) {
                        a += __shfl_xor(a, m, 64); c += __shfl_xor(c, m, 64);
                        if constexpr (C::PREP || C::INB) t2 += __shfl_xor(t2, m, 64);
                    }
                    if (n31 == r) { va = a; vc = c; vt = t2; }
                }
                if (n31 < NREG) {
                    const int ch = wave * C::MTW * 32 + chan_of_reg(mt, n31);
                    if constexpr (C::INB) {
                        if (PST) { atomicAdd(PST + ch * 2, vc); atomicAdd(PST + ch * 2 + 1, vt); }
                    } else if constexpr (C::PREP) {
                        atomicAdd(ST + ch * 2, va);
                        if (PST) { atomicAdd(PST + ch * 2, vt); atomicAdd(PST + ch * 2 + 1, vc); }
                    } else if (det) { dvec[ch * 2] = va; dvec[ch * 2 + 1] = vc; }
                    else { atomicAdd(ST + ch * 2, va); atomicAdd(ST + ch * 2 + 1, vc); }
                }
            }
            if (!C::PREP && !C::INB && det && det_arrive_wave(b, nseg * nstrips * C::TEAM)) {
                for (int idx = lane; idx < COUT * 2; idx += 64)
                    p.stats[(size_t)b * COUT * 2 + idx] = det_sum(b, nseg * nstrips, COUT * 2, idx);
            }
        }
    }
}

template <int CIN, int COUT, int FL>
int launch_stream(const ConvParams& p0, hipStream_t s) {
    using C = SC<CIN, COUT, FL>;
    ConvParams p = p0;
    auto kern = conv_stream_kernel<CIN, COUT, FL>;
    static int caps[16] = {0};
    int dev = 0;
    (void)hipGetDevice(&dev);
    int& cap = caps[dev >= 0 && dev < 16 ? dev : 0];
    if (!cap) {
        (void)hipFuncSetAttribute((const void*)kern, hipFuncAttributeMaxDynamicSharedMemorySize, C::LDS_BYTES * C::TPW);
        int occ = 0, ncu = 256;
        (void)hipDeviceGetAttribute(&ncu, hipDeviceAttributeMultiprocessorCount, dev);
        if (hipOccupancyMaxActiveBlocksPerMultiprocessor(&occ, (const void*)kern, 64 * C::TEAM * C::TPW, C::LDS_BYTES * C::TPW) != hipSuccess || occ < 1) occ = 1;
        cap = occ * ncu * C::TPW;
    }
    const int nstrips = (p.W + 31) / 32;
    int nseg = cap / (p.B * nstrips);
    if (dge_env().stream_nseg > 0) nseg = dge_env().stream_nseg;
    int maxseg = p.H / 16; if (maxseg < 1) maxseg = 1;
    if (nseg > maxseg) nseg = maxseg;
    if (nseg < 1) nseg = 1;
    int seg_rows = (p.H + nseg - 1) / nseg;
    if (C::POOL) seg_rows += seg_rows & 1;
    nseg = (p.H + seg_rows - 1) / seg_rows;
    const int njobs = p.B * nstrips * nseg;
    const int nwg = (njobs + C::TPW - 1) / C::TPW;
    const int jobs_per_xcd = (nwg + 7) / 8;
    const char* fl = FL == FL_GEN ? "gen" : (FL == FL_ENC ? "enc" : (FL == FL_ENC_STATS ? "enc_stats" : (FL == FL_DOT ? "dot" : (FL == FL_DOT_PREP ? "dot_prep" : (FL == FL_GEN_RGB ? "gen_rgb" : (FL == FL_DOT_IN ? "dot_in" : (FL == FL_DOT_FR ? "dot_fromrgb" : (FL == FL_DOT_INX ? "dot_inx" : "enc_pool"))))))));
    dge_note_kernel("conv_stream<bf16,%d,%d,%s>", CIN, COUT, fl);
    hipLaunchKernelGGL(kern, dim3((unsigned)(jobs_per_xcd * 8)), dim3(64 * C::TEAM * C::TPW), C::LDS_BYTES * C::TPW, s, p, nstrips, nseg, seg_rows, njobs, jobs_per_xcd);
    DGE_LAUNCH_CHECK("conv_stream");
    return 0;
}

template <int CIN, int COUT>
int launch_flavour(const ConvParams& p, hipStream_t s) {
    if (p.in_coef && p.fr_out) {
        if constexpr (CIN == 16 && COUT == 16) return launch_stream<CIN, COUT, FL_DOT_FR>(p, s);
        dge_set_error("conv_stream: the FromRGB reduction epilogue is built for 16 -> 16 only");
        return -1;
    }
    if (p.in_coef && !p.prep_stats) {
        if constexpr (CIN == COUT && CIN >= 32) return launch_stream<CIN, COUT, FL_DOT_INX>(p, s);
        dge_set_error("conv_stream: the block-input instance-norm backward epilogue is built for 32 -> 32 and 64 -> 64 only");
        return -1;
    }
    if (p.in_coef) {
        if constexpr ((CIN == 32 && COUT == 16) || (CIN == 64 && COUT == 32)) return launch_stream<CIN, COUT, FL_DOT_IN>(p, s);
        dge_set_error("conv_stream: the instance-norm backward epilogue is built for 32 -> 16 and 64 -> 32 only");
        return -1;
    }
    if (p.dot_src) {
        if constexpr (CIN == COUT && CIN >= 32) {
            if (p.prep) return launch_stream<CIN, COUT, FL_DOT_PREP>(p, s);
        }
        if (p.prep) { dge_set_error("conv_stream: the fused tail backward is built for 32->32 and 64->64 only"); return -1; }
        return launch_stream<CIN, COUT, FL_DOT>(p, s);
    }
    const bool enc = p.stats || p.in_shift || (p.noise && p.noise_w_stride != 0);
    if (p.rgb_out) {
        if constexpr ((CIN == 32 && COUT == 32) || (CIN == 64 && COUT == 64)) { if (!enc) return launch_stream<CIN, COUT, FL_GEN_RGB>(p, s); }
        dge_set_error("conv_stream: the fused toRGB is built for the generator flavour of 32 -> 32 and 64 -> 64 only");
        return -1;
    }
    if (p.pool_out) {
        if constexpr ((CIN == 16 && COUT == 32) || (CIN == 32 && COUT == 64)) { if (!p.stats) return launch_stream<CIN, COUT, FL_ENC_POOL>(p, s); }
        dge_set_error("conv_stream: the pooled epilogue is built for the encoder's 16 -> 32 and 32 -> 64 layers without statistics");
        return -1;
    }
    if constexpr (CIN == 64) {
        if (enc) { dge_set_error("conv_stream: encoder flavour with Cin = 64 is not built"); return -1; }
    } else {
        if (p.stats) return launch_stream<CIN, COUT, FL_ENC_STATS>(p, s);
        if (enc) return launch_stream<CIN, COUT, FL_ENC>(p, s);
    }
    return launch_stream<CIN, COUT, FL_GEN>(p, s);
}

}

bool dge_conv_stream_eligible(const ConvParams& p, int dtype, int ksize) {
    if (dtype != DGE_BF16 || ksize != 3 || p.up || p.in_s2d || p.in_up2 || p.in_relu || p.addend || p.mask_relu || p.in_t2d) return false;
    if (!(p.Cin == 16 || p.Cin == 32 || p.Cin == 64) || !(p.Cout == 16 || p.Cout == 32 || p.Cout == 64)) return false;
    if (p.W % 4 != 0 || p.W < 64 || p.H < 32) return false;
    if ((long)p.H * p.W < 128L * 128) return false;
    {
        const long px = (long)p.B * p.H * p.W;
        const bool enc = p.stats || p.in_shift || (p.noise && p.noise_w_stride != 0);
        if (!dge_env().force_stream) {
            if (!p.dot_src && px < (enc ? (1L << 20) : (1L << 18))) return false;
            if (p.dot_src && px < (1L << 16)) return false;
        }
    }
    if ((long)p.W * p.Cin * 2 >= (1L << 31) || (long)p.H * p.W * 64 * 2 >= (1L << 40)) return false;
    if (p.dot_src && !p.stats && !p.in_coef) return false;
    if (p.in_coef && !p.fr_out && p.prep_stats && !(p.dot_src && !p.prep && !p.stats && ((p.Cin == 32 && p.Cout == 16) || (p.Cin == 64 && p.Cout == 32)))) return false;
    if (p.in_coef && !p.fr_out && !p.prep_stats && !(p.dot_src && !p.prep && !p.stats && p.Cin == p.Cout && p.Cin >= 32 && p.H % 2 == 0 && p.W % 2 == 0)) return false;
    if (p.fr_out && !(p.in_coef && p.dot_src && p.fr_img4 && !p.prep && !p.stats && p.Cin == 16 && p.Cout == 16 && p.H % 2 == 0 && p.W % 2 == 0)) return false;
    if (p.prep && !(p.Cin == p.Cout && p.Cin >= 32)) return false;
    if (p.Cin == 64 && !p.dot_src && (p.stats || p.in_shift || (p.noise && p.noise_w_stride != 0))) return false;
    if (p.dot_src && (p.bias || p.noise || p.in_shift || p.act != DGE_ACT_NONE)) return false;
    if (p.noise && p.noise_w == nullptr) return false;
    if (dge_env().no_stream) return false;
    return true;
}

bool dge_conv_pool_ok(const ConvParams& p, int dtype, int ksize) {
    return ((p.Cin == 16 && p.Cout == 32) || (p.Cin == 32 && p.Cout == 64)) && !p.dot_src && !p.stats && !p.rgb_out && p.H % 2 == 0 && p.W % 2 == 0 &&
           dge_conv_stream_eligible(p, dtype, ksize);
}

bool dge_conv_rgb_ok(const ConvParams& p, int dtype, int ksize) {
    return ((p.Cin == 32 && p.Cout == 32) || (p.Cin == 64 && p.Cout == 64)) && !p.dot_src && !p.stats && !p.in_shift && !(p.noise && p.noise_w_stride != 0) &&
           dge_conv_stream_eligible(p, dtype, ksize);
}

int dge_conv_stream_launch(const ConvParams& p, hipStream_t s) {
#define GO(CI, CO) if (p.Cin == CI && p.Cout == CO) return launch_flavour<CI, CO>(p, s)
#ifdef DGE_SC_ONLY
#define GO2(...) GO(__VA_ARGS__)
    GO2(DGE_SC_ONLY);
#undef GO2
#else
    GO(16, 16); GO(16, 32); GO(16, 64); GO(32, 16); GO(32, 32); GO(32, 64); GO(64, 16); GO(64, 32); GO(64, 64);
#endif
#undef GO
    dge_set_error("conv_stream: unsupported channel configuration %d -> %d", p.Cin, p.Cout);
    return -1;
}
```

### deep-gan-encoders_amd/csrc/enc_bwd_kernels.hip

```cpp
#include <stdlib.h>
#include "common.h"
#include "../../include/dge_hip.h"

template <int NTAP>
__device__ __forceinline__ void wgrad_flush(const f32x16_t (&acc)[NTAP], float* smem, float* __restrict__ dW, int o0, int i0,
                                            int Co, int Ci, int tid, int lane, int wave) {
    float* red = smem;
    float* stage = smem + 4096;
#pragma unroll
    for (int t = 0; t < NTAP; t++) {
        __syncthreads();
#pragma unroll
        for (int r = 0; r < 16; r++) red[wave * 1024 + r * 64 + lane] = acc[t][r];
        __syncthreads();
#pragma unroll
        for (int q = 0; q < 4; q++) {
            const int e = tid + q * 256;
            const int r = e >> 6, ln = e & 63;
            const int ol = (r & 3) + 8 * (r >> 2) + 4 * (ln >> 5), il = ln & 31;
            stage[(ol * 32 + il) * NTAP + t] = (red[e] + red[1024 + e]) + (red[2048 + e] + red[3072 + e]);
        }
    }
    __syncthreads();
    const int ni = (Ci - i0 < 32 ? Ci - i0 : 32) * NTAP;
// ... 323 lines not shown
__global__ __launch_bounds__(256) void act_bwd_mask_kernel(const T* __restrict__ gup, const unsigned* __restrict__ mask,
                                                            const float* __restrict__ noise, T* __restrict__ gpre,
                                                            float* __restrict__ red_out, int H, int W, int C, float scale, float slope) {
    constexpr int EP = Elem<T>::PER16;
    __shared__ float red[256 * NS * EP];
    const int b = blockIdx.y;
    const int cpt = C / EP, ppi = 256 / cpt;
    const int chunk = threadIdx.x % cpt, slot = threadIdx.x / cpt;
    const int UW = W / 2, UHW = (H / 2) * UW, HW = H * W;
    float s[NS][EP];
#pragma unroll
    for (int k = 0; k < NS; k++)
#pragma unroll
        for (int e = 0; e < EP; e++) s[k][e] = 0.f;
    const int stride = gridDim.x * ppi;
    for (int q0 = blockIdx.x * ppi; q0 < UHW; q0 += 2 * stride) {
        const int qq[2] = {q0 + slot, q0 + slot + stride};
        bool ok[2]; uint4 gv[2]; unsigned mv[2]; int p00[2]; float nzv[2][4];
#pragma unroll
        for (int h = 0; h < 2; h++) {
            ok[h] = slot < ppi && qq[h] < UHW;
            gv[h] = make_uint4(0, 0, 0, 0); mv[h] = 0; p00[h] = 0;
#pragma unroll
            for (int c4 = 0; c4 < 4; c4++) nzv[h][c4] = 0.f;
            if (ok[h]) {
                gv[h] = *(const uint4*)(gup + ((size_t)b * UHW + qq[h]) * C + chunk * EP);
                mv[h] = mask[((size_t)b * UHW + qq[h]) * cpt + chunk];
                const int oy = qq[h] / UW, ox = qq[h] - oy * UW;
                p00[h] = (2 * oy) * W + 2 * ox;
                if (noise) {
#pragma unroll
                    for (int c4 = 0; c4 < 4; c4++) nzv[h][c4] = noise[(size_t)b * HW + p00[h] + (c4 >> 1) * W + (c4 & 1)];
                }
            }
        }
#pragma unroll
        for (int h = 0; h < 2; h++) {
            if (!ok[h]) continue;
            float g[EP];
            unpack16(gv[h], g, (T*)nullptr);
            const unsigned m = mv[h];
#pragma unroll
            for (int e = 0; e < EP; e++) { if constexpr (NS == 3) s[2][e] += g[e]; g[e] *= scale; }
#pragma unroll
            for (int c4 = 0; c4 < 4; c4++) {
                const int p = p00[h] + (c4 >> 1) * W + (c4 & 1);
                const float nz = nzv[h][c4];
                float o[EP];
#pragma unroll
                for (int e = 0; e < EP; e++) {
                    o[e] = g[e] * (((m >> (c4 * EP + e)) & 1u) ? 1.f : slope);
                    s[0][e] += o[e]; s[1][e] += o[e] * nz;
                }
                *(uint4*)(gpre + ((size_t)b * HW + p) * C + chunk * EP) = pack16(o, (T*)nullptr);
            }
        }
    }
    if (red_out) block_chan_flush<EP, NS>(s, cpt, ppi, red_out + (size_t)b * C * NS, C, red);
}

__global__ void in_bwd_coef_kernel(const float* __restrict__ dots, const float* __restrict__ gms, const float* __restrict__ musig,
                                   const float* __restrict__ sc, const float* __restrict__ sh, float* __restrict__ coef,
                                   int B, int C, float inv_n, int nslot) {
    const int idx = blockIdx.x * blockDim.x + threadIdx.x;
    if (idx >= B * C) return;
    const int b = idx / C, c = idx % C;
    const float r = sc[idx], s = sh[idx];
    float S2 = 0.f, S1 = 0.f;
    if (dots) {
        const float2 ss = sum_slot_pairs(dots + (size_t)idx * 2, (size_t)B * C * 2, nslot);
        S2 = ss.x; S1 = ss.y;
    }
    const float m1 = S1 * inv_n, m2 = (r * S2 + s * S1) * inv_n;
    const float mu = musig[(size_t)b * 2 * C + c], sg = musig[(size_t)b * 2 * C + C + c];
    const float gmu = gms ? gms[(size_t)b * 2 * C + c] : 0.f, gsg = gms ? gms[(size_t)b * 2 * C + C + c] : 0.f;
    const float k = sg > 0.f ? gsg * inv_n / sg : 0.f;
    coef[(size_t)idx * 3 + 0] = r;
    coef[(size_t)idx * 3 + 1] = -r * r * m2 + k;
    coef[(size_t)idx * 3 + 2] = -r * m1 - r * m2 * s + gmu * inv_n - k * mu;
}

struct InCoefSrc { const float* dots; const float* gms; const float* musig; const float* sc; const float* sh; int nslot, B; float inv_n; };
template <typename T, bool FR>
__global__ __launch_bounds__(256) void in_bwd_kernel(const T* __restrict__ gy, const T* __restrict__ X, const float* __restrict__ coef,
                                                      const T* __restrict__ extra, const float* __restrict__ noise,
                                                      T* __restrict__ gout, float* __restrict__ red_out, int H, int W, int C,
                                                      int extra_pool, float extra_scale, int act, InCoefSrc cs,
                                                      const float* __restrict__ img, float* __restrict__ fr_out) {
    constexpr int EP = Elem<T>::PER16;
    __shared__ float red[256 * (FR ? 4 : 2) * EP];
    __shared__ float lcoef[3 * 512];
    const int b = blockIdx.y;
    const int cpt = C / EP, ppi = 256 / cpt;
    const int chunk = threadIdx.x % cpt, slot = threadIdx.x / cpt;
    const int HW = H * W, UW = extra_pool ? W / 2 : W, UHW = extra_pool ? HW / 4 : HW;
    float s[FR ? 4 : 2][EP], A[EP], Bc[EP], Cc[EP];
    if (!coef) {
        for (int c = threadIdx.x; c < C; c += 256) {
            const int idx = b * C + c;
            const float r = cs.sc[idx], sft = cs.sh[idx];
            float S2 = 0.f, S1 = 0.f;
            if (cs.dots) { const float2 ss = sum_slot_pairs(cs.dots + (size_t)idx * 2, (size_t)cs.B * C * 2, cs.nslot); S2 = ss.x; S1 = ss.y; }
            const float m1 = S1 * cs.inv_n, m2 = (r * S2 + sft * S1) * cs.inv_n;
            const float mu = cs.musig[(size_t)b * 2 * C + c], sg = cs.musig[(size_t)b * 2 * C + C + c];
            const float gmu = cs.gms ? cs.gms[(size_t)b * 2 * C + c] : 0.f, gsg = cs.gms ? cs.gms[(size_t)b * 2 * C + C + c] : 0.f;
            const float k = sg > 0.f ? gsg * cs.inv_n / sg : 0.f;
            lcoef[c * 3 + 0] = r;
// ... 324 lines not shown
    const HeadEntry e = tab[blockIdx.z];
    const int lane = threadIdx.x & 63, wave = threadIdx.x >> 6;
    const int k = blockIdx.x * 64 + lane, b = blockIdx.y;
    if (blockIdx.x * 64 >= e.I) return;
    const int per = (O + 15) / 16, o0 = wave * per, o1 = min(O, o0 + per);
    float acc[8];
#pragma unroll
    for (int j = 0; j < 8; j++) acc[j] = 0.f;
    if (k < e.I) {
        const float* gr = g + (size_t)b * ldg + e.gcol;
        int o = o0;
        for (; o + 7 < o1; o += 8) {
#pragma unroll
            for (int j = 0; j < 8; j++) acc[j] += gr[o + j] * e.W[(size_t)(o + j) * e.I + k];
        }
        for (; o < o1; o++) acc[0] += gr[o] * e.W[(size_t)o * e.I + k];
    }
    part[wave][lane] = ((acc[0] + acc[1]) + (acc[2] + acc[3])) + ((acc[4] + acc[5]) + (acc[6] + acc[7]));
    __syncthreads();
    if (wave == 0 && k < e.I) {
        float s = 0.f;
#pragma unroll
        for (int j = 0; j < 16; j++) s += part[j][lane];
        gms_all[e.moff + (size_t)b * e.I + k] = s;
    }
}
__global__ void head_bwd_param_kernel(const HeadEntry* __restrict__ tab, const float* __restrict__ g, int ldg,
                                      const float* __restrict__ musig_all, float* __restrict__ gw_all, float* __restrict__ gb_all,
                                      int B, int O) {
    const HeadEntry e = tab[blockIdx.y];
    const int total = O * e.I;
    for (int idx = blockIdx.x * 256 + threadIdx.x; idx < total; idx += gridDim.x * 256) {
        const int o = idx / e.I, i = idx - o * e.I;
        float s = 0.f, sb = 0.f;
        for (int b = 0; b < B; b++) {
            const float gv = g[(size_t)b * ldg + e.gcol + o];
            s += gv * musig_all[e.moff + (size_t)b * e.I + i]; sb += gv;
        }
        gw_all[e.woff + idx] = s;
        if (i == 0) gb_all[e.boff + o] = sb;
    }
}

#define CHAN_OK(C, ep) ((C) % (ep) == 0 && (C) / (ep) <= 256 && 256 % ((C) / (ep)) == 0)

int dge_wgrad_dma_try(const void* g, const void* x, const float* sc, const float* sh, float* dw, int B, int H, int W, int cout, int cin,
                      const float* wdot, float* dots, int dots_slots, hipStream_t s);
extern "C" int dge_conv_wgrad_dots(const void* g, const void* x, const float* in_scale, const float* in_shift, float* dw, const float* w,
                                   float* dots, int dots_slots, int B, int H, int W, int cout, int cin, int dtype, hipStream_t s) {
    DGE_CHECK(g && x && dw && w && dots && in_scale && in_shift && dots_slots >= 1, "conv_wgrad_dots: null tensor");
    if (dtype != DGE_BF16) return 1;
    return dge_wgrad_dma_try(g, x, in_scale, in_shift, dw, B, H, W, cout, cin, w, dots, dots_slots, s);
}
extern "C" int dge_conv_wgrad(const void* g, const void* x, const float* in_scale, const float* in_shift, float* dw, int B, int H,
                              int W, int cout, int cin, int ksize, int dtype, hipStream_t s) {
    DGE_CHECK(ksize == 1 || ksize == 3, "conv_wgrad: ksize %d unsupported", ksize);
    const int ep = dtype == DGE_BF16 ? 8 : 4;
    DGE_CHECK(cout % ep == 0 && cin % ep == 0, "conv_wgrad: channels must be multiples of %d", ep);
    DGE_CHECK((in_scale == nullptr) == (in_shift == nullptr), "conv_wgrad: in_scale and in_shift go together");
    if (dtype == DGE_BF16 && ksize == 3) {
        const int r = dge_wgrad_dma_try(g, x, in_scale, in_shift, dw, B, H, W, cout, cin, nullptr, nullptr, 1, s);
        if (r <= 0) return r;
    }
    const bool tall = dtype == DGE_BF16 && H >= 16 && !dge_env().wgrad_th8;
    const int tx = (W + 15) / 16, ty = tall ? (H + 15) / 16 : (H + 7) / 8;
    const int ntiles = tx * ty * B;
    const int noi = ((cout + 31) / 32) * ((cin + 31) / 32);
    int groups = 512 / noi; if (groups < 1) groups = 1;
    if (dge_env().wgrad_groups > 0) groups = dge_env().wgrad_groups;
    if (groups > ntiles) groups = ntiles;
    dim3 grid(noi, groups);
    if (dtype == DGE_BF16) dge_note_kernel("conv_wgrad_tr<%d,%d>", ksize, tall ? 16 : 8);
    else dge_note_kernel("conv_wgrad<f32,%d>", ksize);
#define WG(T, KS) hipLaunchKernelGGL((conv_wgrad_kernel<T, KS>), grid, dim3(256), 0, s, (const T*)g, (const T*)x, in_scale, in_shift, dw, B, H, W, cout, cin, tx, ty, groups)
    if (dtype == DGE_BF16) {
#define WT(KS, TH) hipLaunchKernelGGL((conv_wgrad_tr_kernel<KS, TH>), grid, dim3(256), 0, s, (const bf16_t*)g, (const bf16_t*)x, in_scale, in_shift, dw, B, H, W, cout, cin, tx, ty, groups)
        if (ksize == 3) { if (tall) WT(3, 16); else WT(3, 8); }
        else { if (tall) WT(1, 16); else WT(1, 8); }
#undef WT
    }
    else { if (ksize == 3) WG(float, 3); else WG(float, 1); }
#undef WG
    DGE_LAUNCH_CHECK("conv_wgrad");
    return 0;
}

__global__ __launch_bounds__(256) void head_fwd_kernel(const HeadEntry* __restrict__ tab, const float* __restrict__ musig_all,
                                                       float* __restrict__ w, int ldw, int B, int O) {
    const HeadEntry e = tab[blockIdx.y];
    const int wave = (blockIdx.x * 256 + threadIdx.x) >> 6, lane = threadIdx.x & 63;
    if (wave >= B * O) return;
    const int b = wave / O, o = wave - b * O;
    const float* xr = musig_all + e.moff + (size_t)b * e.I;
    const float* wr = e.W + (size_t)o * e.I;
    float s = 0.f;
    for (int i = lane; i < e.I; i += 64) s = fmaf(xr[i], wr[i], s);
    s = wave_sum(s);
    if (lane == 0) w[(size_t)b * ldw + e.gcol + o] = s + (e.bias ? e.bias[o] : 0.f);
}
extern "C" int dge_heads_fwd(const void* dev_entries, int n, const float* musig_all, float* w, int ldw, int B, int O, hipStream_t s) {
    DGE_CHECK(n >= 1 && n <= 65535 && B >= 1 && O >= 1, "heads_fwd: bad sizes");
    hipLaunchKernelGGL(head_fwd_kernel, dim3((B * O * 64 + 255) / 256, n), dim3(256), 0, s, (const HeadEntry*)dev_entries, musig_all, w, ldw, B, O);
    DGE_LAUNCH_CHECK("heads_fwd");
    return 0;
}

// ... 279 lines not shown
```

### deep-gan-encoders_amd/csrc/wgrad_dma.hip

```cpp
#include <stdlib.h>
#include <type_traits>
#include "common.h"
#include "../../include/dge_hip.h"

namespace {

typedef __attribute__((ext_vector_type(4))) unsigned rsrc_t;
typedef short v4s_t __attribute__((ext_vector_type(4)));
typedef __attribute__((address_space(3))) v4s_t* lds_v4s_ptr;

__device__ __forceinline__ unsigned rfl(unsigned v) { return __builtin_amdgcn_readfirstlane(v); }
__device__ __forceinline__ unsigned lds_off(const void* p) {
    return (unsigned)(size_t)(const __attribute__((address_space(3))) unsigned char*)p;
}
__device__ __forceinline__ rsrc_t make_rsrc(unsigned long long base, unsigned bytes) {
    rsrc_t r;
    r[0] = rfl((unsigned)base); r[1] = rfl((unsigned)(base >> 32) & 0xffffu); r[2] = rfl(bytes); r[3] = 0x00020000u;
    return r;
}
__device__ __forceinline__ void dma16(unsigned voff, rsrc_t rs, unsigned m0v) {
    asm volatile("s_mov_b32 m0, %1\n\ts_nop 0\n\tbuffer_load_dwordx4 %0, %2, 0 offen lds" : : "v"(voff), "s"(m0v), "s"(rs) : "memory");
}
constexpr unsigned DEAD = 0x7fffffffu;

template <int TH_, int GP_, int XP_, int NW_, int NS_>
struct WCfg {
    static constexpr int TH = TH_, GP = GP_, XP = XP_, NW = NW_, NS = NS_;
    static constexpr int TW = 16, HH = TH + 2, HWD = TW + 2;
    static constexpr int GBYTES = TH * TW * GP;
    static constexpr int XBYTES = ((HH * HWD + 4) * XP + 1023) / 1024 * 1024;
    static constexpr int NGP = GBYTES / 1024, NXP = XBYTES / 1024, NP = NGP + NXP;
    static constexpr int PW = (NP + NW - 1) / NW;
    static constexpr int STAGE = GBYTES + XBYTES;
    static constexpr int RING = NS * STAGE;
    static constexpr int FLUSH = (NW * 1024 + 1024 * 9) * 4;
    static constexpr int MAIN = RING > FLUSH ? RING : FLUSH;
    static constexpr int GTAB_OFF = MAIN, TAB_OFF = GTAB_OFF + 9 * 32 * 4;
    static constexpr int RW = TH / NW;
    static_assert(TH % NW == 0 && (NS - 2) * PW <= 63 && GBYTES % 1024 == 0 && NS >= 2 && NS <= 5, "configuration");
    static int lds_bytes() { return TAB_OFF + 64 * 4; }
};

#ifdef DGE_WG_TIMING
__device__ long long wg_tlog[64 * 6];
#define DGE_WT(k) do { __builtin_amdgcn_sched_barrier(0); const long long t_ = __builtin_readcyclecounter(); __builtin_amdgcn_sched_barrier(0); \
                       if (tlogon && t - t_begin >= 8 && t - t_begin < 40) wg_tlog[(t - t_begin - 8) * 6 + k] = t_; } while (0)
#else
#define DGE_WT(k)
#endif

template <class C>
__global__ __launch_bounds__(C::NW * 64, 2) void wgrad_dma_kernel(const bf16_t* __restrict__ g, const bf16_t* __restrict__ X,
                                                                const float* __restrict__ sc, const float* __restrict__ sh,
                                                                float* __restrict__ dW, int B, int H, int W, int Co, int Ci,
                                                                int tiles_x, int tiles_y, int per_group, int gps,
                                                                const float* __restrict__ Wdot, float* __restrict__ dots, int dots_slots) {
    constexpr int TH = C::TH, GP = C::GP, XP = C::XP, NW = C::NW, NS = C::NS, NT = NW * 64;
    extern __shared__ __attribute__((aligned(1024))) unsigned char lds[];
    float* gtab = (float*)(lds + C::GTAB_OFF);
    float* sctab = (float*)(lds + C::TAB_OFF);
    float* ktab = sctab + 32;
    const int tid = threadIdx.x, lane = tid & 63;
    const int wave = __builtin_amdgcn_readfirstlane(tid >> 6);
    const int n_it = (Ci + 31) / 32;
    const int noi = gridDim.x, lin = blockIdx.x + noi * blockIdx.y;
    int grp_id = blockIdx.y, oi = blockIdx.x;
    if (!(gridDim.y & 7)) { const int slot = lin >> 3; grp_id = (slot / noi) * 8 + (lin & 7); oi = slot % noi; }
    const int o0 = (oi / n_it) * 32, i0 = (oi % n_it) * 32;
    const int tps = tiles_x * tiles_y;
    if (grp_id >= B * gps) return;
    const int smp = grp_id / gps, part = grp_id - smp * gps;
    const int t_begin = smp * tps + part * per_group;
    const int t_end = t_begin + per_group < (smp + 1) * tps ? t_begin + per_group : (smp + 1) * tps;
    if (t_begin >= t_end) return;
    const bool aff = sc != nullptr;
    if (aff && tid < 32) {
        const int ch = i0 + tid;
        sctab[tid] = ch < Ci ? sc[smp * Ci + ch] : 1.f;
        ktab[tid] = ch < Ci ? sh[smp * Ci + ch] : 0.f;
    }
    __syncthreads();
    f32x16_t acc[9];
#pragma unroll
    for (int t = 0; t < 9; t++)
#pragma unroll
        for (int r = 0; r < 16; r++) acc[t][r] = 0.f;

    constexpr int CG = GP / 16, CX = XP / 16, PPG = 1024 / GP, PPX = 1024 / XP;
    constexpr int PG = C::NGP / NW, PX = (C::NXP + NW - 1) / NW;
    static_assert(C::NGP % NW == 0 && PG + PX == C::PW, "piece split");
    const int cg = lane % CG, pg = lane / CG, cx = lane % CX, px = lane / CX;
    const bool g_alive = o0 + cg * 8 < Co, x_alive = i0 + cx * 8 < Ci;
    const bool last_x = wave + NW * (PX - 1) < C::NXP;
    const int pw_mine = PG + PX - (last_x ? 0 : 1);
    unsigned rel_g[PG], rel_x[PX];
#pragma unroll
    for (int j = 0; j < PG; j++) {
        const int q = (wave + NW * j) * PPG + pg;
        rel_g[j] = g_alive ? (unsigned)((((q >> 4) * W + (q & 15)) * Co + o0 + cg * 8) * 2) : DEAD;
    }
#pragma unroll
    for (int j = 0; j < PX; j++) {
        const int q = (wave + NW * j) * PPX + px, hy = q / C::HWD, hx = q - hy * C::HWD;
        rel_x[j] = (q < C::HH * C::HWD && x_alive) ? (unsigned)((((hy - 1) * W + (hx - 1)) * Ci + i0 + cx * 8) * 2) : DEAD;
    }
    const unsigned lds0 = lds_off(lds);
    const unsigned sample_g = (unsigned)H * W * Co * 2, sample_x = (unsigned)H * W * Ci * 2;
    int irem = t_begin - smp * tps, ity = irem / tiles_x, itx = irem - ity * tiles_x;
    auto issue = [&](int stage) {
        const unsigned mg = lds0 + stage * C::STAGE + wave * 1024, mx = mg + C::GBYTES;
        const int y0 = ity * TH, x0 = itx * 16;
        const rsrc_t rg = make_rsrc((unsigned long long)g + (unsigned long long)smp * sample_g, sample_g);
        const rsrc_t rx = make_rsrc((unsigned long long)X + (unsigned long long)smp * sample_x, sample_x);
        const unsigned gbase = (unsigned)((y0 * W + x0) * Co * 2), xbase = (unsigned)((y0 * W + x0) * Ci * 2);
        const bool interior = (y0 >= 1) & (y0 + TH + 1 <= H) & (x0 >= 1) & (x0 + 17 <= W);
        if (interior) {
#pragma unroll
            for (int j = 0; j < PG; j++) dma16(gbase + rel_g[j], rg, mg + j * NW * 1024);
#pragma unroll
            for (int j = 0; j < PX - 1; j++) dma16(xbase + rel_x[j], rx, mx + j * NW * 1024);
            if (last_x) dma16(xbase + rel_x[PX - 1], rx, mx + (PX - 1) * NW * 1024);
        } else {
#pragma unroll
            for (int j = 0; j < PG; j++) {
                const int q = (wave + NW * j) * PPG + pg;
                const bool ok = (rel_g[j] != DEAD) & (y0 + (q >> 4) < H) & (x0 + (q & 15) < W);
                dma16(ok ? gbase + rel_g[j] : DEAD, rg, mg + j * NW * 1024);
            }
#pragma unroll
            for (int j = 0; j < PX; j++) {
                const int q = (wave + NW * j) * PPX + px, hy = q / C::HWD, hx = q - hy * C::HWD;
                const bool ok = (rel_x[j] != DEAD) & ((unsigned)(y0 + hy - 1) < (unsigned)H) & ((unsigned)(x0 + hx - 1) < (unsigned)W);
                if (j < PX - 1 || last_x) dma16(ok ? xbase + rel_x[j] : DEAD, rx, mx + j * NW * 1024);
            }
        }
        if (++itx == tiles_x) { itx = 0; ++ity; }
    };
    auto wait_tile = [&](int nfly) {
        const bool full = pw_mine == C::PW;
#define DGE_W(N) asm volatile("s_waitcnt vmcnt(%0)" :: "i"(N) : "memory")
        if (nfly <= 0) DGE_W(0);
        else if (nfly == 1) { if (full) DGE_W(C::PW); else DGE_W(C::PW - 1); }
        else if (nfly == 2) { if (full) DGE_W(2 * C::PW > 63 ? 63 : 2 * C::PW); else DGE_W(2 * (C::PW - 1) > 63 ? 63 : 2 * (C::PW - 1)); }
        else { if (full) DGE_W(3 * C::PW > 63 ? 63 : 3 * C::PW); else DGE_W(3 * (C::PW - 1) > 63 ? 63 : 3 * (C::PW - 1)); }
#undef DGE_W
    };

    const int grp = lane >> 4, li = lane & 15, kg = lane >> 5;
    const int frag_g = (kg * 8 + (li >> 2)) * GP + (GP == 64 ? (grp & 1) * 32 : 0) + (li & 3) * 8;
    const int frag_x = (kg * 8 + (li >> 2)) * XP + (XP == 64 ? (grp & 1) * 32 : 0) + (li & 3) * 8;
    auto trd = [&](const unsigned char* p) { return __builtin_amdgcn_ds_read_tr16_b64_v4i16((lds_v4s_ptr)p); };

    float s_tot = 0.f, s_top = 0.f, s_bot = 0.f, s_lft = 0.f, s_rgt = 0.f, s_tl = 0.f, s_tr = 0.f, s_bl = 0.f, s_br = 0.f;
    int crem = t_begin - smp * tps, cty = crem / tiles_x, ctx = crem - cty * tiles_x;

    auto gather_sums = [&]() {
        float v[9] = {s_tot, s_top, s_bot, s_lft, s_rgt, s_tl, s_tr, s_bl, s_br};
        float* part = (float*)lds;
        __syncthreads();
#pragma unroll
        for (int k = 0; k < 9; k++) {
            v[k] += __shfl_xor(v[k], 32, 64);
            if (lane < 32) part[(wave * 9 + k) * 32 + lane] = v[k];
        }
        __syncthreads();
        for (int idx = tid; idx < 9 * 32; idx += NT) {
            float t = 0.f;
#pragma unroll
            for (int w = 0; w < NW; w++) t += part[w * 9 * 32 + idx];
            gtab[idx] = t;
        }
        __syncthreads();
    };

#pragma unroll
    for (int s = 0; s < NS - 1; s++) if (t_begin + s < t_end) issue(s);
    int stage = 0;
#ifdef DGE_WG_TIMING
    const bool tlogon = lin == 40 && tid == 0;
#endif
    for (int t = t_begin; t < t_end; t++) {
        const int younger = t_end - 1 - t;
        DGE_WT(0);
        wait_tile(younger < NS - 2 ? younger : NS - 2);
        DGE_WT(1);
        __syncthreads();
        DGE_WT(2);
        if (t + NS - 1 < t_end) issue(stage == 0 ? NS - 1 : stage - 1);
        DGE_WT(3);
        const unsigned char* sg = lds + stage * C::STAGE;
        const unsigned char* sx = sg + C::GBYTES;
        const int y0 = cty * TH, x0 = ctx * 16;
        const bool edge_tile = (y0 == 0) | (y0 + TH >= H) | (x0 == 0) | (x0 + 16 >= W);
        uint4 av[2];
        uint4 xv[2][3];
        uint32_t xw[2][3];
        auto frags = [&](int rr, uint4& a, uint4 (&x3)[3], uint32_t (&w3)[3]) {
            const int row = C::RW * wave + rr;
            const unsigned char* ga = sg + row * 16 * GP + frag_g;
            const v4s_t a0 = trd(ga), a1 = trd(ga + 4 * GP);
            const uint2 a01 = *(const uint2*)&a0, a23 = *(const uint2*)&a1;
            a = make_uint4(a01.x, a01.y, a23.x, a23.y);
#pragma unroll
            for (int dy = 0; dy < 3; dy++) {
                const unsigned char* xa = sx + (row + dy) * C::HWD * XP + frag_x;
                const v4s_t q0 = trd(xa), q1 = trd(xa + 4 * XP), q2 = trd(xa + 8 * XP);
                const uint2 w01 = *(const uint2*)&q0, w23 = *(const uint2*)&q1;
                x3[dy] = make_uint4(w01.x, w01.y, w23.x, w23.y);
                w3[dy] = (*(const uint2*)&q2).x;
            }
        };
        frags(0, av[0], xv[0], xw[0]);
        StaticFor<C::RW>::run([&](auto rc) {
            constexpr int rr = decltype(rc)::value;
            if constexpr (rr + 1 < C::RW) frags(rr + 1, av[(rr + 1) & 1], xv[(rr + 1) & 1], xw[(rr + 1) & 1]);
            const uint4 a4 = av[rr & 1];
            const bf16x8_t a = *(const bf16x8_t*)&a4;
#pragma unroll
            for (int dy = 0; dy < 3; dy++) {
                const uint4 v0 = xv[rr & 1][dy];
                const uint32_t w4 = xw[rr & 1][dy];
                const uint4 b1 = make_uint4(__builtin_amdgcn_alignbit(v0.y, v0.x, 16), __builtin_amdgcn_alignbit(v0.z, v0.y, 16),
                                            __builtin_amdgcn_alignbit(v0.w, v0.z, 16), __builtin_amdgcn_alignbit(w4, v0.w, 16));
                const uint4 b2 = make_uint4(v0.y, v0.z, v0.w, w4);
                acc[dy * 3 + 0] = __builtin_amdgcn_mfma_f32_32x32x16_bf16(a, *(const bf16x8_t*)&v0, acc[dy * 3 + 0], 0, 0, 0);
                acc[dy * 3 + 1] = __builtin_amdgcn_mfma_f32_32x32x16_bf16(a, *(const bf16x8_t*)&b1, acc[dy * 3 + 1], 0, 0, 0);
                acc[dy * 3 + 2] = __builtin_amdgcn_mfma_f32_32x32x16_bf16(a, *(const bf16x8_t*)&b2, acc[dy * 3 + 2], 0, 0, 0);
            }
            if (aff) {
                const bf16x2_t one2 = {(__bf16)1.0f, (__bf16)1.0f};
                float rs = __builtin_amdgcn_fdot2_f32_bf16(*(const bf16x2_t*)&a4.x, one2, 0.f, false);
                rs = __builtin_amdgcn_fdot2_f32_bf16(*(const bf16x2_t*)&a4.y, one2, rs, false);
                rs = __builtin_amdgcn_fdot2_f32_bf16(*(const bf16x2_t*)&a4.z, one2, rs, false);
                rs = __builtin_amdgcn_fdot2_f32_bf16(*(const bf16x2_t*)&a4.w, one2, rs, false);
                s_tot += rs;
                if (edge_tile) {
                    const int gy = y0 + C::RW * wave + rr;
                    const float ftop = gy == 0 ? 1.f : 0.f, fbot = gy == H - 1 ? 1.f : 0.f;
                    const float fl = (x0 == 0 && kg == 0) ? __uint_as_float(a4.x << 16) : 0.f;
                    const int pc = W - 1 - x0;
                    float fr = 0.f;
                    if ((unsigned)pc < 16u) {
                        const int ws = (pc & 7) >> 1;
                        const uint32_t wv = ws == 0 ? a4.x : (ws == 1 ? a4.y : (ws == 2 ? a4.z : a4.w));
                        fr = (pc >> 3) == kg ? __uint_as_float((pc & 1) ? (wv & 0xffff0000u) : (wv << 16)) : 0.f;
                    }
                    s_top = fmaf(ftop, rs, s_top); s_bot = fmaf(fbot, rs, s_bot);
                    s_lft += fl; s_rgt += fr;
                    s_tl = fmaf(ftop, fl, s_tl); s_tr = fmaf(ftop, fr, s_tr);
                    s_bl = fmaf(fbot, fl, s_bl); s_br = fmaf(fbot, fr, s_br);
                }
            }
        });
#ifdef DGE_WG_TIMING
        asm volatile("s_nop 0" :: "v"(acc[0][0]), "v"(acc[8][15]));
#endif
        DGE_WT(4);
        if (++ctx == tiles_x) { ctx = 0; ++cty; }
        stage = stage + 1 == NS ? 0 : stage + 1;
    }
    if (aff) gather_sums();
    float* red = (float*)lds;
    float* stg = red + NW * 1024;
    float d_s2 = 0.f, d_s1 = 0.f;
    static_assert(NT % 64 == 0, "flush: a thread's elements share the input channel");
#pragma unroll
    for (int t = 0; t < 9; t++) {
        __syncthreads();
#pragma unroll
        for (int r = 0; r < 16; r++) red[wave * 1024 + r * 64 + lane] = acc[t][r];
        __syncthreads();
        for (int e = tid; e < 1024; e += NT) {
            const int r = e >> 6, ln = e & 63;
            const int ol = (r & 3) + 8 * (r >> 2) + 4 * (ln >> 5), il = ln & 31;
            float s = 0.f;
#pragma unroll
            for (int w = 0; w < NW; w++) s += red[w * 1024 + e];
            if (aff) {
                const int dy = t / 3, dx = t - dy * 3;
                float G = gtab[ol];
                if (dy != 1) G -= gtab[(dy == 0 ? 32 : 64) + ol];
                if (dx != 1) G -= gtab[(dx == 0 ? 96 : 128) + ol];
                if (dy != 1 && dx != 1) G += gtab[160 + 32 * ((dy >> 1) * 2 + (dx >> 1)) + ol];
                if (dots) {
                    const float wv = (o0 + ol < Co && i0 + il < Ci) ? bf2f(f2bf(Wdot[((size_t)(o0 + ol) * Ci + i0 + il) * 9 + t])) : 0.f;
                    d_s2 = fmaf(wv, s, d_s2); d_s1 = fmaf(wv, G, d_s1);
                }
                s = fmaf(s, sctab[il], ktab[il] * G);
            }
            stg[(ol * 32 + il) * 9 + t] = s;
        }
    }
    __syncthreads();
    if (dots) {
        red[tid * 2] = d_s2; red[tid * 2 + 1] = d_s1;
        __syncthreads();
        if (tid < 64) {
            const int il = tid & 31, k = tid >> 5;
            float v = 0.f;
            for (int j = 0; j < NT / 32; j++) v += red[(il + 32 * j) * 2 + k];
            if (i0 + il < Ci) atomicAdd(dots + ((size_t)(grp_id % dots_slots) * B * Ci + (size_t)smp * Ci + i0 + il) * 2 + k, v);
        }
    }
    const int ni = (Ci - i0 < 32 ? Ci - i0 : 32) * 9;
    if (det_on()) {
        const int L = 1024 * 9, nslots = B * gps;
        float* dslot = det_slot(oi, noi, grp_id, nslots, L);
        for (int idx = tid; idx < L; idx += NT) dslot[idx] = stg[idx];
        if (det_arrive_wg(oi, nslots)) {
            for (int idx = tid; idx < L; idx += NT) {
                const int ol = idx / (32 * 9), j = idx - ol * (32 * 9);
                if (o0 + ol < Co && j < ni) dW[((size_t)(o0 + ol) * Ci + i0) * 9 + j] += det_sum(oi, nslots, L, idx);
            }
        }
        return;
    }
    for (int idx = tid; idx < 1024 * 9; idx += NT) {
        const int ol = idx / (32 * 9), j = idx - ol * (32 * 9);
        if (o0 + ol < Co && j < ni) atomicAdd(dW + ((size_t)(o0 + ol) * Ci + i0) * 9 + j, stg[idx]);
    }
}

template <class C>
int launch(const void* g, const void* x, const float* sc, const float* sh, float* dw, int B, int H, int W, int cout, int cin,
           const float* wdot, float* dots, int dots_slots, hipStream_t s) {
    const int tx = (W + 15) / 16, ty = (H + C::TH - 1) / C::TH;
    const int tps = tx * ty;
    const int noi = ((cout + 31) / 32) * ((cin + 31) / 32);
    const int lds_bytes = C::lds_bytes();
    static int attr_bytes[16] = {0};
    int dev = 0;
    (void)hipGetDevice(&dev);
    auto kern = wgrad_dma_kernel<C>;
    if (dev < 0 || dev >= 16 || attr_bytes[dev] < lds_bytes) {
        const hipError_t e = hipFuncSetAttribute((const void*)kern, hipFuncAttributeMaxDynamicSharedMemorySize, lds_bytes);
        if (e != hipSuccess) {
            dge_set_error("wgrad_dma: cannot raise the dynamic LDS limit to %d bytes: %s", lds_bytes, hipGetErrorString(e));
            return -3;
        }
        if (dev >= 0 && dev < 16) attr_bytes[dev] = lds_bytes;
    }
    const int wg_per_cu = 2 * lds_bytes <= 160 * 1024 ? 2 : 1;
    const int groups_env = dge_env().wgrad_groups;
    int gps = groups_env > 0 ? groups_env : (256 * wg_per_cu + noi * B - 1) / (noi * B);
    gps = gps < 1 ? 1 : (gps > tps ? tps : gps);
    const int per = (tps + gps - 1) / gps;
    gps = (tps + per - 1) / per;
    const int groups = B * gps;
    const int groups8 = groups < 8 ? groups : (groups + 7) / 8 * 8;
    if (!dge_det_fits(noi, (long long)B * gps, 1024 * 9)) return 1;
    dge_note_kernel("wgrad_dma<%d,%d,%d,%d>", C::TH, C::GP, C::XP, C::NS);
    hipLaunchKernelGGL(kern, dim3(noi, groups8), dim3(C::NW * 64), lds_bytes, s, (const bf16_t*)g, (const bf16_t*)x, sc, sh, dw, B, H, W,
                       cout, cin, tx, ty, per, gps, wdot, dots, dots_slots < 1 ? 1 : dots_slots);
    DGE_LAUNCH_CHECK("wgrad_dma");
    return 0;
}

}

#ifdef DGE_WG_TIMING
extern "C" int dge_wgrad_tlog(long long* out, int n) {
    return (int)hipMemcpyFromSymbol(out, HIP_SYMBOL(wg_tlog), (size_t)n * sizeof(long long), 0, hipMemcpyDeviceToHost);
}
#endif
int dge_wgrad_dma_try(const void* g, const void* x, const float* sc, const float* sh, float* dw, int B, int H, int W, int cout, int cin,
                      const float* wdot, float* dots, int dots_slots, hipStream_t s) {
    static int off = -1;
    if (off < 0) off = getenv("DGE_NO_WGRAD_DMA") ? 1 : 0;
    if (off) return 1;
    if (cout % 8 || cin % 8) return 1;
    if (dots && (!sc || !wdot || !dge_det_fits(1LL << 40, 1, 1))) return 1;
    if ((size_t)H * W * cout * 2 >= (1u << 30) || (size_t)H * W * cin * 2 >= (1u << 30)) return 1;
    const int tps = ((W + 15) / 16) * ((H + 15) / 16);
    const int noi = ((cout + 31) / 32) * ((cin + 31) / 32);
    if (tps < 16 || noi * B > 1024) return 1;
    const bool g32 = cout <= 16, x32 = cin <= 16;
    {
        static const int cfg = getenv("DGE_WGRAD_CFG") ? atoi(getenv("DGE_WGRAD_CFG")) : 0;
#define WTRY(...) return launch<WCfg<__VA_ARGS__>>(g, x, sc, sh, dw, B, H, W, cout, cin, wdot, dots, dots_slots, s)
        if (cfg == 1) { if (g32 && x32) WTRY(8, 32, 32, 4, 5); if (!g32 && x32) WTRY(8, 64, 32, 4, 4); if (!g32 && !x32) WTRY(8, 64, 64, 4, 4); }
        if (cfg == 2) { if (g32 && x32) WTRY(16, 32, 32, 4, 4); if (!g32 && x32) WTRY(16, 64, 32, 4, 3); if (!g32 && !x32) WTRY(16, 64, 64, 4, 3); }
        if (cfg == 3) { if (g32 && x32) WTRY(8, 32, 32, 4, 3); if (!g32 && x32) WTRY(8, 64, 32, 4, 3); if (!g32 && !x32) WTRY(8, 64, 64, 4, 3); }
#undef WTRY
    }
    if (g32 && x32) return launch<WCfg<16, 32, 32, 4, 3>>(g, x, sc, sh, dw, B, H, W, cout, cin, wdot, dots, dots_slots, s);
    if (!g32 && x32) return launch<WCfg<16, 64, 32, 4, 2>>(g, x, sc, sh, dw, B, H, W, cout, cin, wdot, dots, dots_slots, s);
    if (g32 && !x32) return launch<WCfg<16, 32, 64, 4, 2>>(g, x, sc, sh, dw, B, H, W, cout, cin, wdot, dots, dots_slots, s);
    if (cin <= 32 && cout <= 64) return launch<WCfg<8, 64, 64, 4, 3>>(g, x, sc, sh, dw, B, H, W, cout, cin, wdot, dots, dots_slots, s);
    return launch<WCfg<16, 64, 64, 4, 2>>(g, x, sc, sh, dw, B, H, W, cout, cin, wdot, dots, dots_slots, s);
}
```

### deep-gan-encoders_amd/ops.py

```python
import ctypes as C
import math

import torch

from ._lib import lib, check, ConvDesc, ConvPPDesc, DgeError, last_kernel

F32, BF16 = 0, 1
ACT_NONE, ACT_LRELU, ACT_RELU, LIN_RSQRT = 0, 1, 2, 3
PACK_FWD, PACK_UPFOLD, PACK_DGRAD, PACK_UPFOLD_DGRAD, PACK_SG1_UP, PACK_SG1_UP_DGRAD, PACK_UPT2D_DGRAD = 0, 1, 2, 3, 4, 5, 6
PACK_UPT2D_UNITS = 7
PACK_FRAG = 0x100
import os as _os
import weakref as _weakref
KERNEL_LOG = None
PROFILE = None


class _ZeroArena:

    def __init__(self):
        self.buf, self.off, self.high, self.active = None, 0, 0, False


_ARENA = _ZeroArena()
# ... 363 lines not shown
        return stats.alloc(nslot), nslot, None
    if stats is None or nslot == 1 or not spread_plain:
        return stats, 1, None
    partial = zeros((nslot,) + tuple(stats.shape), device)
    return partial, nslot, lambda: sum_slots(partial, stats)


def _prep_values(prep, nslot):
    pn = prep.get("noise")
    return float(prep["gain"]), pn, prep.get("ns") if pn is not None else None, 1 if pn is None else pn.shape[0], prep["stats"].alloc(nslot)


def _set_prep(d, prep, nslot):
    gain, pn, ns, nb, st = _prep_values(prep, nslot)
    d.prep, d.prep_gain, d.prep_noise, d.prep_ns, d.prep_noise_batch, d.prep_stats = 1, gain, _f32(pn), _f32(ns), nb, _f32(st)


def _weight_images(in_scale, out_scale):
    t = in_scale if out_scale is None else out_scale
    return 1 if t is None else t.shape[0]


class _PrefetchChain:

    def __init__(self, on=True):
        self.on, self.prev, self.next = on, {}, {}

    def link(self, stream, w_packed):
        if not self.on:
            return None
        key = w_packed.data_ptr()
        prev = self.prev.get(stream)
        if prev is not None and prev != key:
            if len(self.next) > 512:
                self.next.clear()
            self.next[(stream, prev)] = (key, w_packed.shape[1], w_packed.shape[2], _weakref.ref(w_packed))
        self.prev[stream] = key
        nxt = self.next.get((stream, key))
        if nxt is None:
            return None
        t = nxt[3]()
        if t is None or t.data_ptr() != nxt[0]:
            del self.next[(stream, key)]
            return None
        return nxt[:3]


_PREFETCH = _PrefetchChain(on=not _os.environ.get("DGE_NO_PREFETCH"))


def conv2d(x, w_packed, cout, ksize=3, up=False, in_scale=None, in_shift=None, out_scale=None, bias=None,
           bias_scale=1.0, noise=None, noise_w=None, act=ACT_NONE, gain=1.0, addend=None, add_scale=1.0, stats=None,
           out=None, in_s2d=False, dot_src=None, in_up2=False, in_relu=False, prep=None, relu_mask=None, in_t2d=False, rgb=None, pool_out=False, pool_mask=False,
           in_bwd=None):
    B, H, W, Cin = x.shape
    if in_s2d:
        H, W, Cin = H // 2, W // 2, Cin * 4
    if in_up2:
        H, W = 2 * H, 2 * W
    if in_t2d:
        H, W = H - 1, W - 1
    dt = dtype_of(x)
    OH, OW = (2 * H, 2 * W) if up else (H, W)
    mask = None
    if pool_out:
        if out is not None or up:
            raise DgeError("conv2d: pool_out allocates its own result and excludes up")
        out = torch.empty((B, OH // 2, OW // 2, cout), dtype=x.dtype, device=x.device)
        if pool_mask:
            mask = torch.empty((B, (OH // 2) * (OW // 2), cout // 8), dtype=torch.int32, device=x.device)
    if out is None:
        out = torch.empty((B, OH, OW, cout), dtype=x.dtype, device=x.device)
    d = ConvDesc()
    d.pool_out, d.pool_mask = 1 if pool_out else 0, _p(mask)
    dot_src = _mask_as_dot_src("conv2d", relu_mask, dot_src, prep)
    d.mask_relu = 0 if relu_mask is None else 1
    d.in_t2d = 1 if in_t2d else 0
    d.x, d.w_packed, d.y, d.addend, d.dot_src = _p(x), _p(w_packed), _p(out), _p(addend), _p(dot_src)
    d.in_scale, d.in_shift, d.out_scale = _f32(in_scale), _f32(in_shift), _f32(out_scale)
    st, nslot, finish = _stats_target(stats, B, H, W, 16, x.device)
    d.bias, d.noise, d.noise_w, d.stats = _f32(bias), _f32(noise), _f32(noise_w), _f32(st)
    d.stats_slots = nslot
    d.B, d.H, d.W, d.Cin, d.Cout = B, H, W, Cin, cout
    d.ksize, d.up, d.in_s2d, d.in_up2 = ksize, 1 if up else 0, 1 if in_s2d else 0, 1 if in_up2 else 0
    d.in_relu = 1 if in_relu else 0
    d.w_layout = 1 if getattr(w_packed, "_dge_frag", False) else 0
    if d.w_layout:
        nxt = _PREFETCH.link(_stream().value or 0, w_packed)
        if nxt is not None:
            d.prefetch_w, d.prefetch_ntot, d.prefetch_cin = C.c_void_p(nxt[0]), int(nxt[1]), int(nxt[2])
    if prep is not None:
        if stats is None or dot_src is None:
            raise DgeError("conv2d: prep needs stats and dot_src")
        _set_prep(d, prep, nslot)
    if in_bwd is not None:
        if dot_src is None or stats is not None or prep is not None:
            raise DgeError("conv2d: in_bwd needs dot_src and excludes stats / prep")
        d.stats_slots = _stats_slots(B, H, W, 16)
        pn = in_bwd.get("noise")
        d.in_bwd_coef = _f32(in_bwd["coef"])
        d.prep_noise, d.prep_noise_batch = _f32(pn), 1 if pn is None else pn.shape[0]
        if in_bwd.get("fr") is not None:
            d.fr_img4, d.in_bwd_extra, d.in_bwd_extra_scale = _f32(in_bwd["img4"]), _p(in_bwd.get("extra")), float(in_bwd.get("extra_scale", 1.0))
            in_bwd["fr"].buf = zeros((d.stats_slots, B, cout, 4), x.device)
            d.fr_out = _f32(in_bwd["fr"].buf)
        elif in_bwd.get("red") is not None:
            d.prep_stats = _f32(in_bwd["red"].alloc(d.stats_slots))
        else:
            d.prep_noise = None
            d.in_bwd_extra, d.in_bwd_extra_scale = _p(in_bwd.get("extra")), float(in_bwd.get("extra_scale", 1.0))
    if rgb is not None:
        d.rgb_w, d.rgb_style, d.rgb_bias, d.rgb_out = _f32(rgb["w"]), _f32(rgb["style"]), _f32(rgb["bias"]), _f32(rgb["out"])
        d.rgb_wscale, d.rgb_skip_y = float(rgb["wscale"]), 1 if rgb.get("skip_y") else 0
    d.noise_batch = 1 if noise is None else noise.shape[0]
    d.noise_w_per_channel = 0 if (noise_w is None or noise_w.numel() == 1) else 1
    d.act, d.bias_scale, d.gain, d.add_scale, d.dtype = act, bias_scale, gain, add_scale, dt
    if w_packed.dtype != x.dtype:
        raise DgeError("conv2d: packed weight dtype differs from activation dtype")
    taps_cin = 9.0 * Cin if up else 9.0 * (Cin // 4) if (in_s2d or in_t2d) else float(ksize * ksize) * Cin
    skip_y = rgb is not None and rgb.get("skip_y")
    _launch(lib().dge_conv2d, (C.byref(d), _stream()), "dge_conv2d", taps_cin * cout * H * W * B, (B, H, W, Cin, cout, ksize, up, in_s2d),
            (x, None if skip_y else out, addend, dot_src, w_packed, rgb["out"] if rgb is not None else None))
    if finish is not None:
        finish()
    if skip_y:
        return None
    if pool_out and pool_mask:
        return out, mask
    return out


def conv_in_bwd_supported(B, H, W, cin, cout, dtype):
    return bool(lib().dge_conv_in_bwd_supported(int(B), int(H), int(W), int(cin), int(cout), 3, int(dtype)))


def conv_in_bwd_x_supported(B, H, W, cin, cout, dtype):
    return bool(lib().dge_conv_in_bwd_x_supported(int(B), int(H), int(W), int(cin), int(cout), 3, int(dtype)))


def conv_in_bwd_fromrgb_supported(B, H, W, cin, cout, dtype):
    return bool(lib().dge_conv_in_bwd_fromrgb_supported(int(B), int(H), int(W), int(cin), int(cout), 3, int(dtype)))


def up_pp_supported(B, H, W, cin, cout, dtype):
    return bool(lib().dge_up_pp_supported(int(B), int(H), int(W), int(cin), int(cout), int(dtype)))


def pack_up_pp(w_units, cout, cin, in_scale=None, out_scale=None, gain=1.0, out=None):
    if w_units.dtype != torch.bfloat16:
        raise DgeError("pack_up_pp: expects the bf16 units of pack_upconv_weight")
    nb = _weight_images(in_scale, out_scale)
    if out is None:
        out = torch.empty((nb, 9 * cin * cout), dtype=torch.bfloat16, device=w_units.device)
    check(lib().dge_pack_up_pp(_p(w_units), _p(out), int(cout), int(cin), _f32(in_scale), _f32(out_scale), float(gain), nb, _stream()),
          "dge_pack_up_pp")
    return out


def up_pp(x, w_img, cout, bias=None, bias_scale=1.0, noise=None, noise_w=None, act=ACT_NONE, gain=1.0):
    B, H, W, Cin = x.shape
    if x.dtype != torch.bfloat16 or not x.is_cuda:
        raise DgeError("up_pp: bf16 CUDA activations only (the HIP path has no CPU fallback)")
    y = torch.empty((B, 2 * H, 2 * W, cout), dtype=x.dtype, device=x.device)
    nbs = 0 if (noise is None or noise.shape[0] == 1) else 4 * H * W
    if noise_w is not None and noise_w.numel() != 1:
        raise DgeError("up_pp: one noise strength per layer (stylegan2_generator.py:911-916)")
    wbs = 0 if w_img.shape[0] == 1 else w_img.stride(0)

    _launch(lib().dge_up_pp, (_p(x), _p(w_img), int(wbs), _p(y), _f32(noise), nbs, _f32(noise_w), _f32(bias), float(bias_scale),
                              float(gain), int(act), B, H, W, Cin, int(cout), _stream()), "dge_up_pp",
            9.0 * Cin * cout * H * W * B, (B, H, W, Cin, cout, 3, "upfir", False), (x, y), wbytes=18 * Cin * cout * B, log=True)
    return y


def conv_pp_supported(B, H, W, cin, cout, dtype):
    return bool(lib().dge_conv_pp_supported(int(B), int(H), int(W), int(cin), int(cout), int(dtype)))


def pack_conv_pp(w, wscale=1.0, in_scale=None, out_scale=None, gain=1.0, dgrad=False, out=None):
    cout, cin = w.shape[0], w.shape[1]
    N, K = (cin, cout) if dgrad else (cout, cin)
    nb = _weight_images(in_scale, out_scale)
    if out is None:
        out = torch.empty((nb, 9 * N * K), dtype=torch.bfloat16, device=w.device)
    check(lib().dge_pack_conv_pp(_f32(w.detach().contiguous()), _p(out), N, K, float(wscale), _f32(in_scale), _f32(out_scale), float(gain),
                                 nb, 1 if dgrad else 0, _stream()), "dge_pack_conv_pp")
# ... 169 lines not shown
    B, FH, FW, Cc = g.shape
    H, W = FH // 2, FW // 2
    z = torch.empty((B, H + 1, W + 1, 4 * Cc), dtype=g.dtype, device=g.device)
    check(lib().dge_fir_t2d(_p(g), _f32(scale), _p(z), B, H, W, Cc, dtype_of(g), _stream()), "dge_fir_t2d")
    return z


def s2_style_grads(blocks, g_wp, wscale):
    from ._lib import S2GradEntry
    arr = (S2GradEntry * len(blocks))()
    B, nrows, K = g_wp.shape
    for e, blk in zip(arr, blocks):
        e.wstyle, e.row = _f32(blk["wstyle"]), int(blk["row"])
        if "gs" in blk:
            e.gs, e.in_c = _f32(blk["gs"]), blk["gs"].shape[1]
            continue
        P, st = blk["P"], blk["st"]
        e.nslot_p, e.nslot_s = 1, 1
        if isinstance(P, SlotStats):
            e.nslot_p, P = P.nslot, P.buf
        if isinstance(st, SlotStats):
            e.nslot_s, st = st.nslot, st.buf
        e.P, e.st, e.d, e.s, e.bias, e.wsq = _f32(P), _f32(st), _f32(blk["d"]), _f32(blk["s"]), _f32(blk["bias"]), _f32(blk["wsq"])
        e.out_c, e.in_c = blk["d"].shape[1], blk["s"].shape[1]
        e.bscale = float(blk["bscale"])
    check(lib().dge_s2_style_grads(arr, len(blocks), _p(g_wp), B, nrows, K, float(wscale), _stream()), "dge_s2_style_grads")
    return g_wp


def torgb_bwd(gimg, x, wrgb, style, wscale):
    B, H, W, Cc = x.shape
    gx = torch.empty_like(x)
    gs = zeros((B, Cc), x.device)
    check(lib().dge_torgb_bwd(_f32(gimg), _p(x), _f32(wrgb), _f32(style), _p(gx), _p(gs), B, H * W, Cc, float(wscale),
                              dtype_of(x), _stream()), "dge_torgb_bwd")
    return gx, gs


def up2_bwd(g):
    B, Cc, H, W = g.shape
    out = torch.empty((B, Cc, H // 2, W // 2), dtype=torch.float32, device=g.device)
    check(lib().dge_up2_bwd(_f32(g), _p(out), B * Cc, H // 2, W // 2, _stream()), "dge_up2_bwd")
    return out


def conv_wgrad(g, x, dw, in_scale=None, in_shift=None):
    B, H, W, Cin = x.shape
    cout, _, k, _ = dw.shape
    check(lib().dge_conv_wgrad(_p(g), _p(x), _f32(in_scale), _f32(in_shift), _f32(dw), B, H, W, cout, Cin, k, dtype_of(x),
                               _stream()), "dge_conv_wgrad")
    return dw


def conv_wgrad_dots(g, x, dw, in_scale, in_shift, w, dots):
    B, H, W, Cin = x.shape
    cout = dw.shape[0]
    if dw.shape[2] != 3 or is_deterministic():
        return False
    nslot = max(1, min(16, (H * W) // 4096))
    buf = dots.alloc(nslot)
    r = lib().dge_conv_wgrad_dots(_p(g), _p(x), _f32(in_scale), _f32(in_shift), _f32(dw), _f32(w.detach()), _f32(buf), nslot, B, H, W, cout, Cin,
                                  dtype_of(x), _stream())
    if r == 1:
        dots.buf, dots.nslot = None, 1
        return False
    check(r, "dge_conv_wgrad_dots")
    return True


class DeferredSums:

    def __init__(self):
        self.items = []

    def add(self, part, red):
        self.items.append((part, red))
        if len(self.items) == 32:
            self.flush()
        return red

    def flush(self):
        if not self.items:
            return
        from ._lib import SumPlanarEntry
        arr = (SumPlanarEntry * len(self.items))()
        for e, (part, red) in zip(arr, self.items):
            e.partial, e.out = _p(part), _p(red)
            e.nslot, e.C, e.NS = part.shape
        check(lib().dge_sum_slots_planar_multi(arr, len(self.items), _stream()), "dge_sum_slots_planar_multi")
        self.items = []


def _sum_planar(part, red, defer=None):
    if defer is not None:
        return defer.add(part, red)
    B, Cc, NS = part.shape
    check(lib().dge_sum_slots_planar(_p(part), _p(red), B, Cc, NS, _stream()), "dge_sum_slots_planar")
    return red


def act_bwd(gup, a, noise=None, pool=False, scale=1.0, red=None, slope=0.2, planar=False, defer=None):
    B, H, W, Cc = a.shape
    gpre = torch.empty_like(a)
    ncol = 2 if red is None else (red.shape[0] if planar else red.shape[-1])
    part = zeros((B, Cc, ncol), a.device) if red is not None else None
    check(lib().dge_act_bwd(_p(gup), _p(a), _f32(noise), _p(gpre), _f32(part), ncol, B, H, W, Cc,
                            1 if pool else 0, float(scale), float(slope), dtype_of(a), _stream()), "dge_act_bwd")
    if red is not None:
        _sum_planar(part, red, defer) if planar else _sum_over_batch(part, red)
    return gpre


def act_bwd_mask(gup, mask, noise, scale=1.0, red=None, slope=0.2, planar=False, defer=None):
    B, UH, UW, Cc = gup.shape
    H, W = 2 * UH, 2 * UW
    gpre = torch.empty((B, H, W, Cc), dtype=gup.dtype, device=gup.device)
    ncol = 2 if red is None else (red.shape[0] if planar else red.shape[-1])
    part = zeros((B, Cc, ncol), gup.device) if red is not None else None
    check(lib().dge_act_bwd_mask(_p(gup), _p(mask), _f32(noise), _p(gpre), _f32(part), ncol, B, H, W, Cc, float(scale), float(slope),
                                 dtype_of(gup), _stream()), "dge_act_bwd_mask")
    if red is not None:
        _sum_planar(part, red, defer) if planar else _sum_over_batch(part, red)
    return gpre


def in_bwd_coef(dots, gms, musig, sc, sh, npix):
    B, Cc = sc.shape
    coef = torch.empty((B, Cc, 3), dtype=torch.float32, device=sc.device)
    nslot = 1
    if isinstance(dots, SlotStats):
        nslot, dots = dots.nslot, dots.buf
    check(lib().dge_in_bwd_coef_slots(_f32(dots), nslot, _f32(gms), _f32(musig), _f32(sc), _f32(sh), _p(coef), B, Cc, int(npix),
                                      _stream()), "dge_in_bwd_coef")
    return coef


def in_bwd(gy, x, coef, extra=None, extra_pool=False, extra_scale=1.0, noise=None, act=False, red=None, planar=False, defer=None):
    B, H, W, Cc = x.shape
    gout = torch.empty_like(x)
    part = zeros((B, Cc, 2), x.device) if red is not None else None
    if isinstance(coef, tuple) and Cc > 512:
        coef = in_bwd_coef(*coef)
    if isinstance(coef, tuple):
        dots, gms, musig, sc, sh, npix = coef
        nslot = 1
        if isinstance(dots, SlotStats):
            nslot, dots = dots.nslot, dots.buf
        check(lib().dge_in_bwd_fused(_p(gy), _p(x), _f32(dots), nslot, _f32(gms), _f32(musig), _f32(sc), _f32(sh), int(npix), _p(extra),
                                     _f32(noise), _p(gout), _f32(part), B, H, W, Cc, 1 if extra_pool else 0, float(extra_scale),
                                     1 if act else 0, dtype_of(x), _stream()), "dge_in_bwd_fused")
    else:
        check(lib().dge_in_bwd(_p(gy), _p(x), _f32(coef), _p(extra), _f32(noise), _p(gout), _f32(part), B, H, W, Cc,
                               1 if extra_pool else 0, float(extra_scale), 1 if act else 0, dtype_of(x), _stream()), "dge_in_bwd")
    if red is not None:
        _sum_planar(part, red, defer) if planar else _sum_over_batch(part, red)
    return gout


def in_bwd_fromrgb(gy, x0, coef, img, extra=None, extra_pool=False, extra_scale=1.0, defer=None):
    B, H, W, Cc = x0.shape
    dots, gms, musig, sc, sh, npix = coef
    nslot = 1
    if isinstance(dots, SlotStats):
        nslot, dots = dots.nslot, dots.buf
    part = zeros((B, Cc, 4), x0.device)
    check(lib().dge_in_bwd_fromrgb(_p(gy), _p(x0), _f32(dots), nslot, _f32(gms), _f32(musig), _f32(sc), _f32(sh), int(npix), _p(extra),
                                   _f32(img.contiguous()), _p(part), B, H, W, Cc, 1 if extra_pool else 0, float(extra_scale),
                                   dtype_of(x0), _stream()), "dge_in_bwd_fromrgb")
    return _sum_planar(part, torch.empty((4, Cc), dtype=torch.float32, device=x0.device), defer)
# ... 753 lines not shown
```

### include/dge_hip.h

```cpp
#ifndef DGE_HIP_H
#define DGE_HIP_H
#include <stddef.h>
#ifdef __cplusplus
extern "C" {
#endif

typedef struct ihipStream_t* dge_stream_t;

#define DGE_DTYPE_F32 0
#define DGE_DTYPE_BF16 1
#define DGE_ACT_LINEAR 0
#define DGE_ACT_LRELU02 1
#define DGE_ACT_RELU_ 2
#define DGE_LIN_RSQRT 3
#define DGE_PACK_FWD 0
#define DGE_PACK_UPFOLD 1
#define DGE_PACK_DGRAD 2
#define DGE_PACK_UPFOLD_DGRAD 3
#define DGE_PACK_SG1_UP 4
#define DGE_PACK_SG1_UP_DGRAD 5
#define DGE_PACK_UPT2D_DGRAD 6
#define DGE_PACK_UPT2D_UNITS 7

const char* dge_last_error(void);
int dge_version(void);

typedef struct dge_conv_desc {
    const void* x;
    const void* w_packed;
    void* y;
    const void* addend;
    const void* dot_src;
    const float* in_scale;
    const float* in_shift;
    const float* out_scale;
    const float* bias;
    const float* noise;
    const float* noise_w;
    float* stats;
    int B, H, W, Cin, Cout;
    int ksize;
    int up;
    int in_s2d;
    int noise_batch;
    int noise_w_per_channel;
    int act;
    float bias_scale, gain, add_scale;
    int dtype;
    int in_up2;
    int in_relu;
    int stats_slots;
    int w_layout;
    int prep;
    float prep_gain;
    const float* prep_noise;
    const float* prep_ns;
    int prep_noise_batch;
    float* prep_stats;
    int mask_relu;
    int in_t2d;
    const float* rgb_w;
    const float* rgb_style;
    const float* rgb_bias;
    float* rgb_out;
    float rgb_wscale;
    int rgb_skip_y;
    int pool_out;
    void* pool_mask;
    const void* prefetch_w;
    int prefetch_ntot, prefetch_cin;
    const float* in_bwd_coef;
    const void* in_bwd_extra;
    float in_bwd_extra_scale;
    const float* fr_img4;
    float* fr_out;
} dge_conv_desc;
int dge_conv2d(const dge_conv_desc* d, dge_stream_t stream);
int dge_conv_small_supported(int H, int W, int cin, int ntot, int ksize, int in_s2d, int in_up2, int dtype);
#define DGE_PACK_FRAG 0x100
const char* dge_last_kernel(void);
void dge_env_reload(void);
int dge_sum_slots(const float* partial, float* out, int nslot, int n, int accumulate, dge_stream_t stream);
int dge_sum_slots_planar(const float* partial, float* out, int nslot, int C, int NS, dge_stream_t stream);
typedef struct dge_sum_planar_entry { const float* partial; float* out; int nslot, C, NS, pad; } dge_sum_planar_entry;
int dge_sum_slots_planar_multi(const dge_sum_planar_entry* entries, int n, dge_stream_t stream);

int dge_linear_rows(const float* x, int ldx_b, const int* row_xoff, const float* w, const float* bias, float* y,
                    const int* row_ybase, const int* row_ybstride, int B, int R, int K, float wscale, float bscale, float add,
                    dge_stream_t stream);
int dge_demod_rows(const float* s_all, const float* wsq_cat, const int* row_woff, const int* row_sbase, const int* row_cin,
                   float* d_all, const int* row_dbase, const int* row_dbstride, int B, int R, float eps, dge_stream_t stream);
int dge_set_deterministic(int on);
int dge_get_deterministic(void);
int dge_packed_n(int n_valid);
int dge_pack_conv_weight(const float* w_oihw, void* out, int cout, int cin, int ksize, int mode, int dtype,
                         float scale, dge_stream_t stream);
int dge_pack_conv_weights_multi(const long long* table_host, void* descs_dev, int n, int upload, dge_stream_t stream);
int dge_pack_desc_bytes(void);
int dge_weight_sumsq(const float* w_oihw, float* wsq, int cout, int cin, int ksize, float scale, dge_stream_t stream);

int dge_linear(const float* x, int ldx, const float* w, const float* bias, float* y, int ldy, int B, int I, int O,
               float wscale, float bscale, float add, int act, float gain, int square_input, dge_stream_t stream);
int dge_pixelnorm(const float* x, float* y, int B, int D, float eps, dge_stream_t stream);
typedef struct dge_dense_layer { const float* w; const float* bias; int I, O; float wscale, bscale, add; int act; float gain; } dge_dense_layer;
int dge_dense_chain(const float* x, int ldx, const dge_dense_layer* layers, int n, float* y, int ldy, int B, int pixelnorm, float eps,
                    dge_stream_t stream);
int dge_truncation(const float* w, const float* w_avg, float* wp, int B, int L, int D, float psi, int layers,
                   int w_is_wp, dge_stream_t stream);

int dge_torgb(const void* x, const float* wrgb, const float* style, const float* bias, const float* prev, float* img,
              int B, int H, int W, int cin, float wscale, int dtype, dge_stream_t stream);

int dge_conv_rgb_supported(int B, int H, int W, int Cin, int Cout, int ksize, int dtype);
int dge_conv_in_bwd_supported(int B, int H, int W, int Cin, int Cout, int ksize, int dtype);
int dge_conv_in_bwd_fromrgb_supported(int B, int H, int W, int Cin, int Cout, int ksize, int dtype);
int dge_conv_in_bwd_x_supported(int B, int H, int W, int Cin, int Cout, int ksize, int dtype);
int dge_conv_pool_supported(int B, int H, int W, int Cin, int Cout, int ksize, int dtype);
int dge_rgb_upsample_add(float* img, const float* prev, int BC, int H, int W, dge_stream_t stream);
int dge_nchw_to_nhwc(const float* src, void* dst, int B, int C, int HW, int src_B, int dtype, dge_stream_t stream);
int dge_nhwc_to_nchw(const void* src, float* dst, int B, int C, int HW, int dtype, dge_stream_t stream);

int dge_fromrgb(const float* img, const float* w, const float* bias, void* y, float* stats, int B, int HW, int C,
                int dtype, dge_stream_t stream);
int dge_fromrgb2(const float* img, const float* w, const float* bias, void* y, float* stats, float* img4, int B, int HW, int C,
                 int dtype, dge_stream_t stream);
int dge_stats_finalize(const float* stats, float* musig, float* sc, float* sh, int B, int C, int npix, float eps,
                       dge_stream_t stream);
int dge_stats_finalize_slots(const float* stats, int nslot, float* musig, float* sc, float* sh, int B, int C, int npix, float eps,
                             dge_stream_t stream);
int dge_blend(const void* x, const void* z, void* y, const float* sc, const float* sh, float* stats, int B, int OH,
              int OW, int C, int pool, float alpha, float beta, int dtype, dge_stream_t stream);

int dge_loss_reduce(const float* a, const float* b, float* sums7, int B, int C, int H, int W, int y0, int x0, int h, int w,
                    dge_stream_t stream);
int dge_ssim_fwd(const float* a, const float* b, float* ssim_sum, float* dmap, int BC, int h, int w, dge_stream_t stream);
int dge_ssim_box7(const float* a, const float* b, float* sums, int BC, int h, int w, float scale, float shift, float data_range,
                  dge_stream_t stream);
int dge_ssim_bwd(const float* a, const float* b, const float* dmap, float* g, int BC, int h, int w, float scale,
                 int accumulate, dge_stream_t stream);
int dge_space_loss_finalize(const float* sums7, const float* ssim_sum, const float* lpips, float* out8, float n,
                            float n_pooled, int image_space, dge_stream_t stream);
int dge_space_loss_bwd(const float* a, const float* b, const float* sums7, const float* g_pooled, float* g, int BC, int H,
                       int W, int y0, int x0, int h, int w, int k, float n, float weight, int accumulate, dge_stream_t stream);
int dge_loss_reduce3(const float* a, const float* b, float* sums, int B, int C, int H, int W, const int* wins, int nwin, dge_stream_t stream);
int dge_crop_pool_multi(const float* const* src, float* const* dst, const int* wins, const int* ks, int n, int BC, int H, int W,
                        dge_stream_t stream);
int dge_space_loss_bwd3(const float* a, const float* b, const float* const* sums7, const float* const* g_pooled, float* g, int BC, int H,
                        int W, const int* wins, const int* ks, const float* n, const float* weight, int nwin, dge_stream_t stream);
int dge_space_loss_bwd_split(const float* a, const float* b, const float* const* sums7, const float* const* g_pooled, float* const* g,
                             int BC, int H, int W, const int* wins, const int* ks, const float* n, const float* weight, int nwin,
                             dge_stream_t stream);
int dge_loss_reduce_rows(const float* a, const float* b, float* partials, int B, int C, int H, int W, const int* wins, int nwin, int nblk,
                         dge_stream_t stream);
int dge_ssim_fwd_rows(const float* a, const float* b, float* tile_sums, float* dmap, int BC, int h, int w, dge_stream_t stream);
int dge_space_loss_finalize_rows(const float* partials, int nblk, const float* const* ssim_tiles, const int* ssim_cnt,
                                 const float* const* lpips_val, float* sums7, float* out8, int B, int nwin, const float* n,
                                 const float* n_pooled, int image_space, dge_stream_t stream);
int dge_space_loss_bwd_rows(const float* a, const float* b, const float* sums7, const float* const* g_pooled, float* g, int B, int C,
                            int H, int W, const int* wins, const int* ks, const float* n, const float* weight, int nwin, int swap_ab,
                            dge_stream_t stream);
int dge_axpy_scalar(const float* x, const float* scalar, float* y, long n, float extra, int accumulate, dge_stream_t stream);

int dge_lreq_adam_multi(int ntensors, float* const* host_p, const float* const* host_g, float* const* host_v,
                        const long* host_n, const float* host_step, float beta2, float eps, const float* gscale,
                        const float* step_mult, dge_stream_t stream);

int dge_modconv_bwd_prep(const void* gx, const void* x, const float* d, const float* noise, void* gy, float* R, int B,
                         int HW, int C, int noise_batch, float gain, int dtype, dge_stream_t stream);
int dge_demod_bwd(const float* R, const float* d, const float* bias, const float* noise_strength, float* t, int B, int C,
                  float bscale, dge_stream_t stream);
int dge_linear_t(const float* x, int ldx, int incx, const float* w, const float* mul, float* y, int ldy, int incy, int B,
                 int O, int K, float scale, int accumulate, dge_stream_t stream);
int dge_torgb_bwd(const float* gimg, const void* x, const float* wrgb, const float* style, void* gx, float* gs, int B,
                  int HW, int C, float wscale, int dtype, dge_stream_t stream);
int dge_torgb_bwd_prep(const float* gimg, const void* x, const float* wrgb, const float* style, const float* noise,
                       const float* noise_strength, int noise_batch, void* gz, float* gs, float* P, int B, int HW, int C,
                       float wscale, float gain, int dtype, dge_stream_t stream);
int dge_fir_t2d(const void* g, const float* scale, void* z, int B, int H, int W, int C, int dtype, dge_stream_t stream);
typedef struct dge_s2_grad_entry {
    const float* P; const float* st; const float* d; const float* s; const float* bias; const float* wsq;
    const float* gs; const float* wstyle;
    int nslot_p, nslot_s, in_c, out_c, row;
    float bscale;
} dge_s2_grad_entry;
int dge_s2_style_grads(const dge_s2_grad_entry* entries, int n, float* g_wp, int B, int nrows, int K, float wscale, dge_stream_t stream);
int dge_demod_bwd_prep(const float* P, int nslot, const float* d, const float* bias, float* t, int B, int C, float bscale,
                       dge_stream_t stream);
int dge_up2_bwd(const float* g, float* gprev, int BC, int h, int w, dge_stream_t stream);

int dge_conv_wgrad(const void* g, const void* x, const float* in_scale, const float* in_shift, float* dw, int B, int H, int W,
                   int cout, int cin, int ksize, int dtype, dge_stream_t stream);
int dge_conv_wgrad_dots(const void* g, const void* x, const float* in_scale, const float* in_shift, float* dw, const float* w,
                        float* dots, int dots_slots, int B, int H, int W, int cout, int cin, int dtype, dge_stream_t stream);
int dge_act_bwd(const void* gup, const void* a, const float* noise, void* gpre, float* red, int red_cols, int B, int H, int W, int C,
                int pool, float scale, float slope, int dtype, dge_stream_t stream);
int dge_blend_pool_mask(const void* x, const void* z, void* y, float* stats, unsigned* mask, int B, int OH, int OW, int C, float alpha,
                        float beta, int dtype, dge_stream_t stream);
int dge_act_bwd_mask(const void* gup, const unsigned* mask, const float* noise, void* gpre, float* red, int red_cols, int B, int H, int W,
                     int C, float scale, float slope, int dtype, dge_stream_t stream);
int dge_fromrgb_dgrad(const void* gx, const void* x0, const float* w, float* gimg, int B, int HW, int C, int dtype, dge_stream_t stream);
int dge_nearest_up2(const void* x, void* y, int B, int H, int W, int C, float scale, int dtype, dge_stream_t stream);
int dge_in_bwd_coef(const float* dots, const float* gms, const float* musig, const float* sc, const float* sh, float* coef,
                    int B, int C, int npix, dge_stream_t stream);
int dge_in_bwd_coef_slots(const float* dots, int nslot, const float* gms, const float* musig, const float* sc, const float* sh,
                          float* coef, int B, int C, int npix, dge_stream_t stream);
int dge_in_bwd(const void* gy, const void* x, const float* coef, const void* extra, const float* noise, void* gout, float* red,
               int B, int H, int W, int C, int extra_pool, float extra_scale, int act, int dtype, dge_stream_t stream);
int dge_in_bwd_fused(const void* gy, const void* x, const float* dots, int nslot, const float* gms, const float* musig,
                     const float* sc, const float* sh, int npix, const void* extra, const float* noise, void* gout, float* red,
                     int B, int H, int W, int C, int extra_pool, float extra_scale, int act, int dtype, dge_stream_t stream);
int dge_chan_sum(const void* x, float* out, int B, int HW, int C, float scale, int dtype, dge_stream_t stream);
int dge_fromrgb_bwd(const void* gx, const void* x0, const float* img, float* out4, int B, int HW, int C, int dtype,
                    dge_stream_t stream);
int dge_in_bwd_fromrgb(const void* gy, const void* x0, const float* dots, int nslot, const float* gms, const float* musig,
                       const float* sc, const float* sh, int npix, const void* extra, const float* img, float* out4,
                       int B, int H, int W, int C, int extra_pool, float extra_scale, int dtype, dge_stream_t stream);
int dge_in_bwd_fromrgb_img(const void* gy, const void* x0, const float* dots, int nslot, const float* gms, const float* musig,
                           const float* sc, const float* sh, int npix, const void* extra, const float* w, const float* img, float* out4,
                           float* gimg, int B, int H, int W, int C, int extra_pool, float extra_scale, int dtype, dge_stream_t stream);
int dge_affine_bwd_fromrgb_img(const void* gy, const void* x0, const float* a, const void* extra, const float* w, const float* img, float* out4,
                               float* gimg, int B, int H, int W, int C, int extra_pool, float extra_scale, int dtype, dge_stream_t stream);
int dge_heads_fwd(const void* dev_entries, int n, const float* musig_all, float* w, int ldw, int B, int O, dge_stream_t stream);
int dge_head_entry_size(void);
int dge_heads_bwd(const void* dev_entries, int n, int max_I, const float* g, int ldg, const float* musig_all, float* gms_all,
                  float* gw_all, float* gb_all, int B, int O, dge_stream_t stream);
int dge_head_rows_entry_size(void);
int dge_heads_rows_fwd(const void* dev_entries, int n, const float* musig_all, float* w, long ldb, long ldr, int nrows, int B, int O,
                       dge_stream_t stream);
int dge_heads_rows_bwd(const void* dev_entries, int n, int max_I, const float* g, long ldb, long ldr, int nrows,
                       const float* musig_all, float* gms_all, float* gw_all, float* gb_all, int B, int O, dge_stream_t stream);
int dge_dense_wgrad(const float* gy, int ldgy, const float* x, int ldx, float* gw, float* gb, int B, int O, int I,
                    int accumulate, dge_stream_t stream);

int dge_lpips_prep(const float* img, void* x, int B, int HW, int cpad, const float* host_shift3, const float* host_scale3,
                   int dtype, dge_stream_t stream);
int dge_lpips_prep_bwd(const void* gx, float* gimg, int B, int HW, int cpad, const float* host_scale3, float factor,
                       int accumulate, int dtype, dge_stream_t stream);
int dge_maxpool2(const void* x, void* y, int B, int H, int W, int C, int dtype, dge_stream_t stream);
int dge_maxpool2_bwd(const void* gy, const void* x, const void* addend, void* gx, int B, int H, int W, int C, int dtype,
                     dge_stream_t stream);
int dge_lpips_head(const void* feat, const float* lin, float* val, void* g1, int B, int HW, int C, float gscale, int dtype,
                   dge_stream_t stream);
int dge_mean(const float* v, float* out, int n, dge_stream_t stream);

int dge_blur_noise_act(const void* x, const float* noise, const float* noise_w, const float* bias, void* y, float* stats,
                       int B, int H, int W, int C, int do_blur, int noise_batch, int act, int dtype, dge_stream_t stream);
// ... 182 lines not shown
```

Before: 380.0 images/sec.

## Fuse pooled activation-gradient expansion into encoder conv_2 wgrad and dgrad kernels

In the encoder block backward, the full-resolution pre-activation gradient of conv_2 is no longer written to memory. Both the weight-gradient/dots kernel and the dgrad conv now read the half-resolution upstream gradient plus the leaky-ReLU/pool mask and expand it on the fly in LDS. This removes a large write and two re-reads of a full-resolution bf16 tensor at the largest encoder resolutions. The cost is extra ALU work, more complex LDS staging with masked DMA loads, and a smaller ring depth (NR 4) in the new kernel flavour. The path is limited to bf16, non-deterministic mode and a 32->16 channel shape.

```diff
diff --git a/deep-gan-encoders_amd/_lib.py b/deep-gan-encoders_amd/_lib.py
--- a/deep-gan-encoders_amd/_lib.py
+++ b/deep-gan-encoders_amd/_lib.py
@@ -24,6 +24,7 @@
         ("rgb_skip_y", C.c_int), ("pool_out", C.c_int), ("pool_mask", C.c_void_p),
         ("prefetch_w", C.c_void_p), ("prefetch_ntot", C.c_int), ("prefetch_cin", C.c_int), ("in_bwd_coef", C.c_void_p),
         ("in_bwd_extra", C.c_void_p), ("in_bwd_extra_scale", C.c_float), ("fr_img4", C.c_void_p), ("fr_out", C.c_void_p),
+        ("x_pool_mask", C.c_void_p), ("x_pool_scale", C.c_float), ("x_pool_slope", C.c_float),
     ]
 
 
@@ -85,6 +86,7 @@
     "dge_torgb": [_P, _P, _P, _P, _P, _P, _I, _I, _I, _I, _F, _I, _P],
     "dge_conv_rgb_supported": [_I, _I, _I, _I, _I, _I, _I],
     "dge_conv_in_bwd_supported": [_I, _I, _I, _I, _I, _I, _I],
+    "dge_conv2_pooled_supported": [_I, _I, _I, _I, _I, _I],
     "dge_conv_in_bwd_fromrgb_supported": [_I, _I, _I, _I, _I, _I, _I],
     "dge_conv_in_bwd_x_supported": [_I, _I, _I, _I, _I, _I, _I],
     "dge_conv_pool_supported": [_I, _I, _I, _I, _I, _I, _I],
@@ -195,6 +197,7 @@
     "dge_pack_conv_pp": [_P, _P, _I, _I, _F, _P, _P, _F, _I, _I, _P],
     "dge_dense_chain": [_P, _I, C.POINTER(DenseLayer), _I, _P, _I, _I, _I, _F, _P],
     "dge_conv_wgrad_dots": [_P, _P, _P, _P, _P, _P, _P, _I, _I, _I, _I, _I, _I, _I, _P],
+    "dge_conv_wgrad_dots_pooled": [_P, _P, _F, _F, _P, _P, _P, _P, _P, _P, _I, _I, _I, _I, _I, _I, _I, _P],
     "dge_pack_conv_pp_rows": [_P, _I, _P, _I, _I, _P, _I, _P, _F, _I, _I, _P],
     "dge_conv_pp": [C.POINTER(ConvPPDesc), _P],
     "dge_up_pp_supported": [_I, _I, _I, _I, _I, _I],
diff --git a/deep-gan-encoders_amd/autograd_enc_bwd.py b/deep-gan-encoders_amd/autograd_enc_bwd.py
--- a/deep-gan-encoders_amd/autograd_enc_bwd.py
+++ b/deep-gan-encoders_amd/autograd_enc_bwd.py
@@ -9,6 +9,7 @@
 
 FUSE_IN_BWD = not os.environ.get("DGE_NO_FUSED_IN_BWD")
 FUSE_IMG_GRAD = not os.environ.get("DGE_NO_FUSED_IMG_GRAD")
+POOLED_GRAD = not os.environ.get("DGE_NO_POOLED_GRAD")
 
 FROMRGB, BLOCK_INPUT, SEPARATE = "FromRGB reduction", "block input", "separate passes"
 
@@ -17,16 +18,20 @@
     B, dev, dt, grads, params = c.B, c.dev, c.dt, c.grads, c.params
     x1 = rec["x1"]
     extra, extra_pool, extra_scale = None, False, 1.0
-    g_pre2 = g_y2 = dots2 = None
+    g_pre2 = g_y2 = dots2 = pool2 = None
     fuse2 = False
     if blk.has_last_conv:
         has3 = Cc != C2
         red2 = ops.zeros((3 if has3 else 2, C2), dev) if params else None
-        g_pre2 = ops.act_bwd_mask(g_out, rec["m2"], rec["n2"], scale=0.111 * 0.25, red=red2, planar=True, defer=c.later)
+        if POOLED_GRAD and params and FUSE_IN_BWD and ops.conv_in_bwd_supported(B, H, H, C2, Cc, dt) and ops.conv2_pooled_supported(B, H, H, C2, Cc, dt):
+            pool2 = (rec["m2"], 0.111 * 0.25, 0.2)
+        g_pre2 = ops.act_bwd_mask(g_out, rec["m2"], rec["n2"], scale=0.111 * 0.25, red=red2, planar=True, defer=c.later, store=pool2 is None)
         sum_g = red_param_grads(grads, pre, 2, red2, planar=True) if params else None
         gW2 = ops.zeros(tuple(blk.conv_2.weight.shape), dev) if params else None
         dots2 = ops.SlotStats(B, Cc, dev)
-        if params and FUSE_IN_BWD and ops.conv_in_bwd_supported(B, H, H, C2, Cc, dt):
+        if pool2 is not None:
+            fuse2 = ops.conv_wgrad_dots(g_out, x1, gW2, rec["sc2"], rec["sh2"], blk.conv_2.weight, dots2, g_pool=pool2)
+        elif params and FUSE_IN_BWD and ops.conv_in_bwd_supported(B, H, H, C2, Cc, dt):
             fuse2 = ops.conv_wgrad_dots(g_pre2, x1, gW2, rec["sc2"], rec["sh2"], blk.conv_2.weight, dots2)
         if fuse2:
             grads[pre + "conv_2.weight"] = gW2
@@ -49,8 +54,8 @@
     red1 = ops.zeros((2, Cc), dev) if params else None
     if fuse2:
         redp = ops.SlotStats(B, Cc, dev)
-        g_pre1 = ops.conv2d(g_pre2, packed(c.cache, blk.conv_2, dt, ops.PACK_DGRAD, H), Cc, 3, dot_src=x1,
-                            in_bwd=dict(coef=ops.in_bwd_coef(*coef2), noise=rec["n1"].reshape(B, H, H), red=redp))
+        g_pre1 = ops.conv2d(g_out if pool2 is not None else g_pre2, packed(c.cache, blk.conv_2, dt, ops.PACK_DGRAD, H), Cc, 3, dot_src=x1,
+                            in_bwd=dict(coef=ops.in_bwd_coef(*coef2), noise=rec["n1"].reshape(B, H, H), red=redp), x_pool=pool2)
         ops._sum_planar(redp.buf.view(-1, Cc, 2), red1, c.later)
     else:
         g_pre1 = ops.in_bwd(g_y2, x1, coef2, noise=rec["n1"], act=True, red=red1, planar=True, defer=c.later)
diff --git a/deep-gan-encoders_amd/csrc/capi.hip b/deep-gan-encoders_amd/csrc/capi.hip
--- a/deep-gan-encoders_amd/csrc/capi.hip
+++ b/deep-gan-encoders_amd/csrc/capi.hip
@@ -117,6 +117,9 @@
     p.in_coef = d->in_bwd_coef;
     p.in_extra = d->in_bwd_coef ? d->in_bwd_extra : nullptr; p.in_extra_scale = d->in_bwd_extra_scale;
     p.fr_img4 = d->in_bwd_coef ? d->fr_img4 : nullptr; p.fr_out = d->in_bwd_coef ? d->fr_out : nullptr;
+    p.xp_mask = d->x_pool_mask; p.xp_scale = d->x_pool_scale; p.xp_slope = d->x_pool_slope;
+    DGE_CHECK(!d->x_pool_mask || (d->in_bwd_coef && d->prep_stats && d->ksize == 3 && dge_conv2_pooled_supported(d->B, d->H, d->W, d->Cin, d->Cout, d->dtype)),
+              "conv2d: x_pool_mask is offered where dge_conv2_pooled_supported() says so, with in_bwd_coef and prep_stats");
     if (d->in_bwd_coef) {
         DGE_CHECK(!dge_get_deterministic(), "conv2d: in_bwd_coef is not offered in deterministic mode; run dge_in_bwd");
         DGE_CHECK(d->ksize == 3 && !d->up && dge_conv_stream_eligible(p, d->dtype, d->ksize), "conv2d: in_bwd_coef is offered where "
@@ -164,6 +167,14 @@
     p.dot_src = (const void*)16; p.prep_stats = (float*)16; p.in_coef = (const float*)16;
     return (ksize == 3 && !dge_get_deterministic() && dge_conv_stream_eligible(p, dtype, ksize)) ? 1 : 0;
 }
+bool dge_wgrad_dma_pooled_ok(int B, int H, int W, int cout, int cin);
+extern "C" int dge_conv2_pooled_supported(int B, int H, int W, int c2, int cc, int dtype) {
+    if (dtype != DGE_BF16 || dge_get_deterministic() || H % 2 || W % 2) return 0;
+    ConvParams p = {};
+    p.B = B; p.H = H; p.W = W; p.Cin = c2; p.Cout = cc; p.Ntot_valid = cc; p.Ntot = dge_packed_n(cc);
+    p.dot_src = (const void*)16; p.prep_stats = (float*)16; p.in_coef = (const float*)16; p.xp_mask = (const unsigned*)16;
+    return (dge_conv_stream_eligible(p, dtype, 3) && dge_wgrad_dma_pooled_ok(B, H, W, c2, cc)) ? 1 : 0;
+}
 extern "C" int dge_conv_in_bwd_x_supported(int B, int H, int W, int Cin, int Cout, int ksize, int dtype) {
     ConvParams p = {};
     p.B = B; p.H = H; p.W = W; p.Cin = Cin; p.Cout = Cout; p.Ntot_valid = Cout; p.Ntot = dge_packed_n(Cout);
diff --git a/deep-gan-encoders_amd/csrc/conv_params.h b/deep-gan-encoders_amd/csrc/conv_params.h
--- a/deep-gan-encoders_amd/csrc/conv_params.h
+++ b/deep-gan-encoders_amd/csrc/conv_params.h
@@ -49,6 +49,7 @@
     int pf_ntot, pf_cin;
     const float* in_coef;
     const void* in_extra; float in_extra_scale; const float* fr_img4; float* fr_out;
+    const unsigned* xp_mask; float xp_scale, xp_slope;
 };
 
 int dge_conv_launch(const ConvParams& p, int dtype, int ksize, hipStream_t s);
diff --git a/deep-gan-encoders_amd/csrc/conv_stream.hip b/deep-gan-encoders_amd/csrc/conv_stream.hip
--- a/deep-gan-encoders_amd/csrc/conv_stream.hip
+++ b/deep-gan-encoders_amd/csrc/conv_stream.hip
@@ -57,6 +57,11 @@
 __device__ __forceinline__ void dma_piece(unsigned voff, rsrc_t rs, unsigned m0v) {
     asm volatile("s_mov_b32 m0, %1\n\ts_nop 0\n\tbuffer_load_dwordx4 %0, %2, 0 offen lds" : : "v"(voff), "s"(m0v), "s"(rs) : "memory");
 }
+__device__ __forceinline__ void dma_piece_masked(unsigned voff, rsrc_t rs, unsigned m0v, unsigned long long mask) {
+    unsigned long long keep;
+    asm volatile("s_mov_b64 %0, exec\n\ts_mov_b64 exec, %4\n\ts_mov_b32 m0, %2\n\ts_nop 0\n\tbuffer_load_dwordx4 %1, %3, 0 offen lds\n\ts_mov_b64 exec, %0"
+                 : "=&s"(keep) : "v"(voff), "s"(m0v), "s"(rs), "s"(mask) : "memory");
+}
 template <int NP> __device__ __forceinline__ void dma_dot(unsigned voff, unsigned voff1, rsrc_t rs, unsigned m0v) {
     if constexpr (NP == 1)
         asm volatile("s_mov_b32 m0, %1\n\ts_nop 0\n\tbuffer_load_dwordx4 %0, %2, 0 offen lds" : : "v"(voff), "s"(m0v), "s"(rs) : "memory");
@@ -65,7 +70,7 @@
                      "buffer_load_dwordx4 %3, %2, 0 offen offset:1024 lds" : : "v"(voff), "s"(m0v), "s"(rs), "v"(voff1) : "memory");
 }
 
-enum { FL_GEN = 0, FL_ENC = 1, FL_ENC_STATS = 2, FL_DOT = 3, FL_DOT_PREP = 4, FL_GEN_RGB = 5, FL_ENC_POOL = 6, FL_DOT_IN = 7, FL_DOT_FR = 8, FL_DOT_INX = 9 };
+enum { FL_GEN = 0, FL_ENC = 1, FL_ENC_STATS = 2, FL_DOT = 3, FL_DOT_PREP = 4, FL_GEN_RGB = 5, FL_ENC_POOL = 6, FL_DOT_IN = 7, FL_DOT_FR = 8, FL_DOT_INX = 9, FL_DOT_INP = 10 };
 
 template <int CIN, int COUT, int FL>
 struct SC {
@@ -76,14 +81,14 @@
     static constexpr int MTW = MT / TEAM;
     static constexpr int HW = 34, RB = HW * PXB;
     static constexpr int PIECES = (RB + 1023) / 1024;
-    static constexpr bool PREP = FL == FL_DOT_PREP, RGB = FL == FL_GEN_RGB, POOL = FL == FL_ENC_POOL, FRB = FL == FL_DOT_FR, INX = FL == FL_DOT_INX, INB = FL == FL_DOT_IN || FRB || INX;
+    static constexpr bool PREP = FL == FL_DOT_PREP, RGB = FL == FL_GEN_RGB, POOL = FL == FL_ENC_POOL, FRB = FL == FL_DOT_FR, INX = FL == FL_DOT_INX, INP = FL == FL_DOT_INP, INB = FL == FL_DOT_IN || FRB || INX || INP;
     static_assert(!RGB || COUT == 32 || (COUT == 64 && TEAM == 2), "fused toRGB: 32 output channels per wave, one wave or a 2-wave team per pixel");
     static constexpr bool DOT = FL == FL_DOT || PREP || INB, STATS = FL == FL_ENC_STATS, ENC = FL == FL_ENC || FL == FL_ENC_STATS || POOL;
     static constexpr bool NOISE = !DOT || PREP || (INB && !FRB && !INX);
-    static constexpr int NR = 6;
+    static constexpr int NR = INP ? 4 : 6;
     static constexpr int dot_depth(int nr) { for (int d = 4; d >= 1; d--) if (d <= nr - 3 && nr % (d + 1) == 0) return d; return 1; }
     static constexpr int D = DOT ? dot_depth(6) : 2;
-    static constexpr int DR = DOT ? D + 1 : NR;
+    static constexpr int DR = INP ? NR : (DOT ? D + 1 : NR);
     static_assert(NR % DR == 0, "dot ring period");
     static constexpr int CPB = COUT * 2;
     static constexpr int CW = COUT / TEAM >= 32 ? 32 : 16;
@@ -101,18 +106,20 @@
     static constexpr int D_OFF = N_OFF + TEAM * NRING;
     static constexpr int DRING = DOT ? DR * DROWB : 0;
     static constexpr int E_OFF = D_OFF + TEAM * DRING;
-    static constexpr int ERING = FRB ? 2 * DR * 512 : (INX ? DR * 1024 : 0);
+    static constexpr int NPU = 18 * CH, PRND = (NPU + 63) / 64, PSLOT = NPU * 20, PLOADS = PRND + 1;
+    static constexpr int ERING = FRB ? 2 * DR * 512 : (INX ? DR * 1024 : (INP ? 2 * PSLOT : 0));
     static_assert(!INX || (CIN == COUT && CIN >= 32), "block-input flavour: 32 -> 32, 64 -> 64");
     static_assert(!FRB || (CIN == 16 && COUT == 16 && TEAM == 1), "FromRGB reduction flavour: 16 -> 16");
     static constexpr int T_OFF = E_OFF + TEAM * ERING;
     static constexpr int TBYTES = 32 * MTW * 16 * 4;
     static constexpr int DUMMY_OFF = T_OFF + TEAM * TBYTES;
     static constexpr int RGBX_OFF = DUMMY_OFF + (TEAM == 2 ? 1024 : 0);
-    static constexpr int LDS_BYTES = RGBX_OFF + (RGB && TEAM == 2 ? 1024 : 0);
+    static constexpr int LDS_BYTES = (RGBX_OFF + (RGB && TEAM == 2 ? 1024 : 0) + (INP ? 127 : 0)) / (INP ? 128 : 1) * (INP ? 128 : 1);
     static constexpr int NEED = 4 * 9 * KS * MTW + 32 * MTW + 16 + (ENC ? 16 * MTW : 0) + (STATS || DOT ? 32 * MTW : 0) + (DOT ? 16 : 0) + (PREP ? 16 : 0) + (RGB ? 11 : 0) + (POOL ? 20 * MTW : 0) + 36;
     static constexpr int WPE = ((PREP || INB) && CIN == 64) ? 1 : (NEED <= 128 ? 4 : (NEED <= 168 ? 3 : 2));
-    static_assert(D <= NR - 3, "the slot of the row being fetched must be dead");
+    static_assert(INP || D <= NR - 3, "the slot of the row being fetched must be dead");
     static_assert((D - 1) * LPR + 1 < 64, "vmcnt range");
+    static_assert(!INP || (TEAM == 1 && D == 2 && (CIN == 32 || CIN == 64)), "pooled-input flavour: one wave per strip, dot rows two steps ahead");
 };
 
 template <int LOGC> __device__ __forceinline__ int chunk_swz(int px) { return (px >> (4 - LOGC)) & ((1 << LOGC) - 1); }
@@ -184,6 +191,25 @@
     const unsigned evoff = C::INX ? (unsigned)(((x0 >> 1) + (lane >> 2)) * C::CPB + wave * 64 + (((lane & 3) ^ chunk_swz<2>(lane >> 2)) << 4))
                                   : (unsigned)((x0 >> 1) * 32 + (lane & 31) * 16);
     const unsigned ivoff = (unsigned)((x0 + (lane & 31)) * 16);
+    constexpr unsigned XP_NONE = 0xffffffffu;
+    unsigned xp_voff[C::INP ? C::PRND : 1], xp_mvoff = 0, xp_wr[C::INP ? C::PRND : 1][2];
+    const unsigned xprow_bytes = C::INP ? (unsigned)(p.W >> 1) * C::PXB : 0u, xpmrow_bytes = C::INP ? (unsigned)(p.W >> 1) * C::CH * 4u : 0u;
+    const unsigned long long XPb = C::INP ? (unsigned long long)p.x + (unsigned long long)b * (p.H >> 1) * xprow_bytes : Xb;
+    const unsigned long long XMb = C::INP ? (unsigned long long)p.xp_mask + (unsigned long long)b * (p.H >> 1) * xpmrow_bytes : Xb;
+    if constexpr (C::INP) {
+#pragma unroll
+        for (int k = 0; k < C::PRND; k++) {
+            const int u = lane + 64 * k, pp = u >> C::LOGCH, c = u & (C::CH - 1);
+            const bool alive = u < C::NPU;
+            xp_voff[k] = alive ? (unsigned)(((x0 >> 1) - 1 + pp) * C::PXB + (c << 4)) : 0x80000000u;
+#pragma unroll
+            for (int dx = 0; dx < 2; dx++) {
+                const int hp = 2 * pp - 1 + dx;
+                xp_wr[k][dx] = (alive && hp >= 0 && hp < C::HW) ? lds0 + C::X_OFF + hp * C::PXB + ((c ^ chunk_swz<C::LOGCH>(hp)) << 4) : XP_NONE;
+            }
+        }
+        xp_mvoff = (unsigned)(((x0 >> 1) - 1) * C::CH * 4 + lane * 16);
+    }
 
     unsigned long long xptr = Xb + (unsigned long long)(long long)(r0 - 1) * xrow_bytes;
     unsigned long long dptr = DOTb + (unsigned long long)(long long)(r0 - 2) * yrow_bytes;
@@ -193,7 +219,7 @@
         const rsrc_t rx = make_rsrc(xptr, xv ? xrow_bytes : 0u);
         xptr += xrow_bytes;
         const unsigned m0x = lds0 + C::X_OFF + slot * C::RB;
-        dma_row<CIN, C::TEAM>(wave, voff, voff_b, voff_c, rx, rs_null, m0x, lds0 + C::DUMMY_OFF);
+        if constexpr (!C::INP) dma_row<CIN, C::TEAM>(wave, voff, voff_b, voff_c, rx, rs_null, m0x, lds0 + C::DUMMY_OFF);
         const bool ov = h >= 2 && h <= rows + 1;
         if constexpr (C::DOT) {
             const rsrc_t rd = make_rsrc(dptr, ov ? yrow_bytes : 0u);
@@ -221,8 +247,71 @@
         const rsrc_t rn = make_rsrc(NZb + (unsigned long long)(v ? gy : 0) * nzrow_bytes, v ? (unsigned)(p.H - gy) * nzrow_bytes : 0u);
         dma_piece(nvoff, rn, lds0 + C::N_OFF + wave * C::NRING + buf_off);
     };
+    auto issue_pooled = [&](int j, int ps) {
+        if constexpr (C::INP) {
+            const int py = (r0 >> 1) + j;
+            const bool v = (unsigned)py < (unsigned)(p.H >> 1);
+            const rsrc_t rp = make_rsrc(XPb + (unsigned long long)(v ? py : 0) * xprow_bytes, v ? xprow_bytes : 0u);
+            const rsrc_t rm = make_rsrc(XMb + (unsigned long long)(v ? py : 0) * xpmrow_bytes, v ? xpmrow_bytes : 0u);
+            const unsigned m0p = lds0 + C::E_OFF + ps * C::PSLOT;
+#pragma unroll
+            for (int k = 0; k < C::PRND - 1; k++) dma_piece(xp_voff[k], rp, m0p + k * 1024);
+            dma_piece_masked(xp_voff[C::PRND - 1], rp, m0p + (C::PRND - 1) * 1024, (1ull << (C::NPU - 64 * (C::PRND - 1))) - 1ull);
+            dma_piece_masked(xp_mvoff, rm, m0p + C::NPU * 16, (1ull << (C::NPU / 4)) - 1ull);
+        }
+    };
+    typedef unsigned xu32x4_t __attribute__((ext_vector_type(4)));
+    const float xp_scale = p.xp_scale, xp_slope = p.xp_slope;
+    typedef unsigned short xu16x2_t __attribute__((ext_vector_type(2)));
+    typedef short xs16x2_t __attribute__((ext_vector_type(2)));
+    auto xp_load = [&](auto psc, uint4 (&pv)[C::INP ? C::PRND : 1], unsigned (&pm)[C::INP ? C::PRND : 1]) {
+        constexpr int PS = decltype(psc)::value;
+        const unsigned pb = lds0 + C::E_OFF + PS * C::PSLOT;
+#pragma unroll
+        for (int k = 0; k < C::PRND; k++) {
+            const xu32x4_t t = *(const __attribute__((address_space(3))) xu32x4_t*)(pb + (unsigned)(lane + 64 * k) * 16u);
+            pv[k] = make_uint4(t[0], t[1], t[2], t[3]);
+            pm[k] = *(const __attribute__((address_space(3))) unsigned*)(pb + C::NPU * 16 + (unsigned)(lane + 64 * k) * 4u);
+        }
+    };
+    auto xp_ab = [&](const uint4 (&pv)[C::INP ? C::PRND : 1], uint4 (&pa)[C::INP ? C::PRND : 1], uint4 (&pb)[C::INP ? C::PRND : 1]) {
+#pragma unroll
+        for (int k = 0; k < C::PRND; k++) {
+            float a[8], bs[8];
+            unpack16(pv[k], a, (bf16_t*)nullptr);
+#pragma unroll
+            for (int e = 0; e < 8; e++) { a[e] *= xp_scale; bs[e] = a[e] * xp_slope; }
+            pa[k] = pack16(a, (bf16_t*)nullptr);
+            pb[k] = pack16(bs, (bf16_t*)nullptr);
+        }
+    };
+    auto xp_expand = [&](auto dyc, auto xsc, const uint4 (&pa)[C::INP ? C::PRND : 1], const uint4 (&pb)[C::INP ? C::PRND : 1], const unsigned (&pm)[C::INP ? C::PRND : 1]) {
+        constexpr int DY = decltype(dyc)::value, XS = decltype(xsc)::value;
+#pragma unroll
+        for (int k = 0; k < C::PRND; k++) {
+            const unsigned h16 = DY ? (pm[k] >> 16) : (pm[k] & 0xffffu);
+            const unsigned hh = h16 | (h16 << 16);
+            const unsigned av[4] = {pa[k].x, pa[k].y, pa[k].z, pa[k].w}, bv[4] = {pb[k].x, pb[k].y, pb[k].z, pb[k].w};
+#pragma unroll
+            for (int dx = 0; dx < 2; dx++) {
+                xu32x4_t t;
+#pragma unroll
+                for (int i = 0; i < 4; i++) {
+                    const xu16x2_t sh = {(unsigned short)(15 - (8 * dx + 2 * i)), (unsigned short)(15 - (8 * dx + 2 * i + 1))};
+                    const xu16x2_t up = __builtin_bit_cast(xu16x2_t, hh) << sh;
+                    const unsigned msk = __builtin_bit_cast(unsigned, __builtin_bit_cast(xs16x2_t, up) >> (xs16x2_t){15, 15});
+                    t[i] = (av[i] & msk) | (bv[i] & ~msk);
+                }
+                if (xp_wr[k][dx] != XP_NONE) *(__attribute__((address_space(3))) xu32x4_t*)(xp_wr[k][dx] + (unsigned)(XS * C::RB)) = t;
+            }
+        }
+    };
     asm volatile("s_waitcnt vmcnt(0)" ::: "memory");
     if constexpr (C::NOISE) issue_noise(0, 0u);
+    if constexpr (C::INP) {
+        issue_pooled(-1, 1); issue_pooled(0, 0);
+        StaticFor<3>::run([&](auto hc) { constexpr int h = decltype(hc)::value; issue(h, 0, (h + 2) % C::DR); });
+    } else
     StaticFor<C::D + 2>::run([&](auto hc) { constexpr int h = decltype(hc)::value; issue(h, h % C::NR, (h + C::NR - 2) % C::NR % C::DR); });
 
     uint4 wf[C::MTW][9][C::KS];
@@ -299,6 +388,22 @@
             }
         }
     }
+    uint4 xpA[C::INP ? C::PRND : 1], xpB[C::INP ? C::PRND : 1]; unsigned xpM[C::INP ? C::PRND : 1];
+    if constexpr (C::INP) {
+        using std::integral_constant;
+        uint4 pv[C::PRND];
+        asm volatile("s_waitcnt vmcnt(0)" ::: "memory");
+        xp_load(integral_constant<int, 1>{}, pv, xpM);
+        xp_ab(pv, xpA, xpB);
+        xp_expand(integral_constant<int, 1>{}, integral_constant<int, 0>{}, xpA, xpB, xpM);
+        xp_load(integral_constant<int, 0>{}, pv, xpM);
+        xp_ab(pv, xpA, xpB);
+        xp_expand(integral_constant<int, 0>{}, integral_constant<int, 1>{}, xpA, xpB, xpM);
+        xp_expand(integral_constant<int, 1>{}, integral_constant<int, 2>{}, xpA, xpB, xpM);
+        asm volatile("s_waitcnt lgkmcnt(0)" ::: "memory");
+        issue_pooled(1, 1);
+        issue(3, 0, 1);
+    }
     auto chan_of_reg = [&](int mt, int r) { return mt * 32 + (C::CW == 16 ? 8 * kh + r : 16 * (r >> 3) + 8 * kh + (r & 7)); };
     constexpr int NREG = C::CW == 16 ? 8 : 16;
     f32x16_t biasv[C::MTW], zero16;
@@ -409,15 +514,23 @@
     auto step = [&](auto ic, int s, unsigned npar) {
         constexpr int I = decltype(ic)::value;
         DGE_T(0);
-        constexpr int NAFTER = (C::D - 1) * C::LPR + ((C::NOISE && I >= 1 && I <= C::D - 1) ? 1 : 0);
+        constexpr int IP = (I + C::NR - 1) % C::NR;
+        constexpr int NAFTER = C::INP ? (IP == 0 ? 1 : 0) + (IP % 2 == 0 ? C::PLOADS : 0) + C::DPIECES
+                                      : (C::D - 1) * C::LPR + ((C::NOISE && I >= 1 && I <= C::D - 1) ? 1 : 0);
         asm volatile("s_waitcnt vmcnt(%0)" :: "i"(NAFTER) : "memory");
         if constexpr (C::RGB && C::TEAM == 2) asm volatile("s_waitcnt lgkmcnt(0)" ::: "memory");
         if constexpr (C::TEAM == 2) __builtin_amdgcn_s_barrier();
         if constexpr (C::RGB && C::TEAM == 2) { if (wave == 0 && s > 0) rgb_flush(s - 1); }
         DGE_T(1);
         if constexpr (C::NOISE && I == 0) issue_noise(s + C::NR, npar ^ 1024u);
+        if constexpr (C::INP && I % 2 == 0) issue_pooled((s >> 1) + 2, (I >> 1) & 1);
         issue(s + 2 + C::D, (I + 2 + C::D) % C::NR, (I + C::D) % C::DR);
         DGE_T(2);
+        uint4 xpv[C::INP ? C::PRND : 1];
+        if constexpr (C::INP && I % 2 == 0) {
+            xp_load(std::integral_constant<int, ((I + 2) >> 1) & 1>{}, xpv, xpM);
+            __builtin_amdgcn_sched_barrier(0);
+        }
 
         const int gy = r0 + s;
         constexpr int NQ = 9 * C::KS;
@@ -449,6 +562,10 @@
             __builtin_amdgcn_sched_group_barrier(0x100, 1, 0);
         });
         __builtin_amdgcn_sched_group_barrier(0x008, PF * C::MTW, 0);
+        if constexpr (C::INP) {
+            if constexpr (I % 2 == 0) xp_ab(xpv, xpA, xpB);
+            xp_expand(std::integral_constant<int, I & 1>{}, std::integral_constant<int, (I + 3) % C::NR>{}, xpA, xpB, xpM);
+        }
         DGE_T(3);
         unsigned char* __restrict__ yrow = Yb + (size_t)gy * yrow_bytes;
 #pragma unroll
@@ -715,12 +832,12 @@
     if (nseg > maxseg) nseg = maxseg;
     if (nseg < 1) nseg = 1;
     int seg_rows = (p.H + nseg - 1) / nseg;
-    if (C::POOL) seg_rows += seg_rows & 1;
+    if (C::POOL || C::INP) seg_rows += seg_rows & 1;
     nseg = (p.H + seg_rows - 1) / seg_rows;
     const int njobs = p.B * nstrips * nseg;
     const int nwg = (njobs + C::TPW - 1) / C::TPW;
     const int jobs_per_xcd = (nwg + 7) / 8;
-    const char* fl = FL == FL_GEN ? "gen" : (FL == FL_ENC ? "enc" : (FL == FL_ENC_STATS ? "enc_stats" : (FL == FL_DOT ? "dot" : (FL == FL_DOT_PREP ? "dot_prep" : (FL == FL_GEN_RGB ? "gen_rgb" : (FL == FL_DOT_IN ? "dot_in" : (FL == FL_DOT_FR ? "dot_fromrgb" : (FL == FL_DOT_INX ? "dot_inx" : "enc_pool"))))))));
+    const char* fl = FL == FL_GEN ? "gen" : (FL == FL_ENC ? "enc" : (FL == FL_ENC_STATS ? "enc_stats" : (FL == FL_DOT ? "dot" : (FL == FL_DOT_PREP ? "dot_prep" : (FL == FL_GEN_RGB ? "gen_rgb" : ((FL == FL_DOT_IN || FL == FL_DOT_INP) ? "dot_in" : (FL == FL_DOT_FR ? "dot_fromrgb" : (FL == FL_DOT_INX ? "dot_inx" : "enc_pool"))))))));
     dge_note_kernel("conv_stream<bf16,%d,%d,%s>", CIN, COUT, fl);
     hipLaunchKernelGGL(kern, dim3((unsigned)(jobs_per_xcd * 8)), dim3(64 * C::TEAM * C::TPW), C::LDS_BYTES * C::TPW, s, p, nstrips, nseg, seg_rows, njobs, jobs_per_xcd);
     DGE_LAUNCH_CHECK("conv_stream");
@@ -740,6 +857,8 @@
         return -1;
     }
     if (p.in_coef) {
+        if constexpr (CIN == 32 && COUT == 16) { if (p.xp_mask) return launch_stream<CIN, COUT, FL_DOT_INP>(p, s); }
+        if (p.xp_mask) { dge_set_error("conv_stream: the pooled input is built for 32 -> 16 only"); return -1; }
         if constexpr ((CIN == 32 && COUT == 16) || (CIN == 64 && COUT == 32)) return launch_stream<CIN, COUT, FL_DOT_IN>(p, s);
         dge_set_error("conv_stream: the instance-norm backward epilogue is built for 32 -> 16 and 64 -> 32 only");
         return -1;
@@ -794,6 +913,8 @@
     if (p.prep && !(p.Cin == p.Cout && p.Cin >= 32)) return false;
     if (p.Cin == 64 && !p.dot_src && (p.stats || p.in_shift || (p.noise && p.noise_w_stride != 0))) return false;
     if (p.dot_src && (p.bias || p.noise || p.in_shift || p.act != DGE_ACT_NONE)) return false;
+    if (p.xp_mask && !(p.in_coef && !p.fr_out && p.prep_stats && p.Cin == 32 && p.Cout == 16 && p.H % 2 == 0 && p.W % 2 == 0 &&
+                       (dge_env().force_stream || (long)p.B * p.H * p.W >= (1L << 22)))) return false;
     if (p.noise && p.noise_w == nullptr) return false;
     if (dge_env().no_stream) return false;
     return true;
diff --git a/deep-gan-encoders_amd/csrc/enc_bwd_kernels.hip b/deep-gan-encoders_amd/csrc/enc_bwd_kernels.hip
--- a/deep-gan-encoders_amd/csrc/enc_bwd_kernels.hip
+++ b/deep-gan-encoders_amd/csrc/enc_bwd_kernels.hip
@@ -399,7 +399,7 @@
                     o[e] = g[e] * (((m >> (c4 * EP + e)) & 1u) ? 1.f : slope);
                     s[0][e] += o[e]; s[1][e] += o[e] * nz;
                 }
-                *(uint4*)(gpre + ((size_t)b * HW + p) * C + chunk * EP) = pack16(o, (T*)nullptr);
+                if (gpre) *(uint4*)(gpre + ((size_t)b * HW + p) * C + chunk * EP) = pack16(o, (T*)nullptr);
             }
         }
     }
@@ -830,6 +830,16 @@
     if (dtype != DGE_BF16) return 1;
     return dge_wgrad_dma_try(g, x, in_scale, in_shift, dw, B, H, W, cout, cin, w, dots, dots_slots, s);
 }
+int dge_wgrad_dma_pooled(const void* gup, const unsigned* mask, float scale, float slope, const void* x, const float* sc, const float* sh,
+                         float* dw, int B, int H, int W, int cout, int cin, const float* wdot, float* dots, int dots_slots, hipStream_t s);
+extern "C" int dge_conv_wgrad_dots_pooled(const void* gup, const unsigned* mask, float scale, float slope, const void* x, const float* in_scale,
+                                          const float* in_shift, float* dw, const float* w, float* dots, int dots_slots, int B, int H, int W,
+                                          int cout, int cin, int dtype, hipStream_t s) {
+    DGE_CHECK(gup && mask && x && dw && w && dots && in_scale && in_shift && dots_slots >= 1, "conv_wgrad_dots_pooled: null tensor");
+    DGE_CHECK(dge_conv2_pooled_supported(B, H, W, cout, cin, dtype), "conv_wgrad_dots_pooled: %d x %d, %d <- %d channels is not a launch "
+              "dge_conv2_pooled_supported() accepts", H, W, cout, cin);
+    return dge_wgrad_dma_pooled(gup, mask, scale, slope, x, in_scale, in_shift, dw, B, H, W, cout, cin, w, dots, dots_slots, s);
+}
 extern "C" int dge_conv_wgrad(const void* g, const void* x, const float* in_scale, const float* in_shift, float* dw, int B, int H,
                               int W, int cout, int cin, int ksize, int dtype, hipStream_t s) {
     DGE_CHECK(ksize == 1 || ksize == 3, "conv_wgrad: ksize %d unsupported", ksize);
diff --git a/deep-gan-encoders_amd/csrc/wgrad_dma.hip b/deep-gan-encoders_amd/csrc/wgrad_dma.hip
--- a/deep-gan-encoders_amd/csrc/wgrad_dma.hip
+++ b/deep-gan-encoders_amd/csrc/wgrad_dma.hip
@@ -37,6 +37,11 @@
     static constexpr int MAIN = RING > FLUSH ? RING : FLUSH;
     static constexpr int GTAB_OFF = MAIN, TAB_OFF = GTAB_OFF + 9 * 32 * 4;
     static constexpr int RW = TH / NW;
+    static constexpr int PGB = (TH / 2) * 8 * 64, PGB_PAD = (PGB + 1023) / 1024 * 1024, NPW = PGB / 1024;
+    static constexpr int STAGE_P = PGB_PAD + 1024 + XBYTES;
+    static constexpr int RING_P = NS * STAGE_P + 2 * GBYTES;
+    static constexpr int MAIN_P = RING_P > FLUSH ? RING_P : FLUSH;
+    static int lds_bytes_p() { return MAIN_P + 9 * 32 * 4 + 64 * 4; }
     static_assert(TH % NW == 0 && (NS - 2) * PW <= 63 && GBYTES % 1024 == 0 && NS >= 2 && NS <= 5, "configuration");
     static int lds_bytes() { return TAB_OFF + 64 * 4; }
 };
@@ -49,16 +54,19 @@
 #define DGE_WT(k)
 #endif
 
-template <class C>
+struct GPool { const bf16_t* gpool; const unsigned* gmask; float gscale, gslope; };
+
+template <class C, bool GPL>
 __global__ __launch_bounds__(C::NW * 64, 2) void wgrad_dma_kernel(const bf16_t* __restrict__ g, const bf16_t* __restrict__ X,
                                                                 const float* __restrict__ sc, const float* __restrict__ sh,
                                                                 float* __restrict__ dW, int B, int H, int W, int Co, int Ci,
                                                                 int tiles_x, int tiles_y, int per_group, int gps,
-                                                                const float* __restrict__ Wdot, float* __restrict__ dots, int dots_slots) {
+                                                                const float* __restrict__ Wdot, float* __restrict__ dots, int dots_slots, GPool gp) {
     constexpr int TH = C::TH, GP = C::GP, XP = C::XP, NW = C::NW, NS = C::NS, NT = NW * 64;
     extern __shared__ __attribute__((aligned(1024))) unsigned char lds[];
-    float* gtab = (float*)(lds + C::GTAB_OFF);
-    float* sctab = (float*)(lds + C::TAB_OFF);
+    constexpr int MAINB = GPL ? C::MAIN_P : C::MAIN;
+    float* gtab = (float*)(lds + MAINB);
+    float* sctab = gtab + 9 * 32;
     float* ktab = sctab + 32;
     const int tid = threadIdx.x, lane = tid & 63;
     const int wave = __builtin_amdgcn_readfirstlane(tid >> 6);
@@ -92,7 +100,7 @@
     const int cg = lane % CG, pg = lane / CG, cx = lane % CX, px = lane / CX;
     const bool g_alive = o0 + cg * 8 < Co, x_alive = i0 + cx * 8 < Ci;
     const bool last_x = wave + NW * (PX - 1) < C::NXP;
-    const int pw_mine = PG + PX - (last_x ? 0 : 1);
+    const int pw_mine = (GPL ? (wave < C::NPW ? 2 : 0) : PG) + PX - (last_x ? 0 : 1);
     unsigned rel_g[PG], rel_x[PX];
 #pragma unroll
     for (int j = 0; j < PG; j++) {
@@ -107,25 +115,48 @@
     const unsigned lds0 = lds_off(lds);
     const unsigned sample_g = (unsigned)H * W * Co * 2, sample_x = (unsigned)H * W * Ci * 2;
     int irem = t_begin - smp * tps, ity = irem / tiles_x, itx = irem - ity * tiles_x;
+    const int PH = H >> 1, PWd = W >> 1;
     auto issue = [&](int stage) {
-        const unsigned mg = lds0 + stage * C::STAGE + wave * 1024, mx = mg + C::GBYTES;
+        const unsigned mg = lds0 + stage * (GPL ? C::STAGE_P : C::STAGE) + wave * 1024, mx = mg + (GPL ? C::PGB_PAD + 1024 : C::GBYTES);
+        if constexpr (GPL) {
+            if (wave < C::NPW) {
+                const int ty0 = ity * (TH / 2), tx0 = itx * 8;
+                const int pxi = lane >> 2, pch = lane & 3;
+                const int Y = ty0 + 2 * wave + (pxi >> 3), Xq = tx0 + (pxi & 7);
+                const bool ok = (o0 + pch * 8 < Co) & (Y < PH) & (Xq < PWd);
+                const unsigned pbytes = (unsigned)PH * PWd * Co * 2, mbytes = (unsigned)PH * PWd * (Co >> 3) * 4;
+                const rsrc_t rp = make_rsrc((unsigned long long)gp.gpool + (unsigned long long)smp * pbytes, pbytes);
+                const rsrc_t rm = make_rsrc((unsigned long long)gp.gmask + (unsigned long long)smp * mbytes, mbytes);
+                dma16(ok ? (unsigned)(((Y * PWd + Xq) * Co + o0 + pch * 8) * 2) : DEAD, rp, mg);
+                const int Ym = ty0 + 2 * wave + ((lane & 15) >> 3), Xm = tx0 + (lane & 7);
+                const bool okm = (Ym < PH) & (Xm < PWd);
+                const unsigned moff = okm ? (unsigned)(((Ym * PWd + Xm) * (Co >> 3) + (o0 >> 3)) * 4) : DEAD;
+                unsigned long long keep;
+                asm volatile("s_mov_b64 %0, exec\n\ts_mov_b64 exec, 0xffff\n\ts_mov_b32 m0, %2\n\ts_nop 0\n\tbuffer_load_dwordx4 %1, %3, 0 offen lds\n\ts_mov_b64 exec, %0"
+                             : "=&s"(keep) : "v"(moff), "s"(lds0 + stage * C::STAGE_P + C::PGB_PAD + wave * 256), "s"(rm) : "memory");
+            }
+        }
         const int y0 = ity * TH, x0 = itx * 16;
         const rsrc_t rg = make_rsrc((unsigned long long)g + (unsigned long long)smp * sample_g, sample_g);
         const rsrc_t rx = make_rsrc((unsigned long long)X + (unsigned long long)smp * sample_x, sample_x);
         const unsigned gbase = (unsigned)((y0 * W + x0) * Co * 2), xbase = (unsigned)((y0 * W + x0) * Ci * 2);
         const bool interior = (y0 >= 1) & (y0 + TH + 1 <= H) & (x0 >= 1) & (x0 + 17 <= W);
         if (interior) {
-#pragma unroll
-            for (int j = 0; j < PG; j++) dma16(gbase + rel_g[j], rg, mg + j * NW * 1024);
+            if constexpr (!GPL) {
+#pragma unroll
+                for (int j = 0; j < PG; j++) dma16(gbase + rel_g[j], rg, mg + j * NW * 1024);
+            }
 #pragma unroll
             for (int j = 0; j < PX - 1; j++) dma16(xbase + rel_x[j], rx, mx + j * NW * 1024);
             if (last_x) dma16(xbase + rel_x[PX - 1], rx, mx + (PX - 1) * NW * 1024);
         } else {
-#pragma unroll
-            for (int j = 0; j < PG; j++) {
-                const int q = (wave + NW * j) * PPG + pg;
-                const bool ok = (rel_g[j] != DEAD) & (y0 + (q >> 4) < H) & (x0 + (q & 15) < W);
-                dma16(ok ? gbase + rel_g[j] : DEAD, rg, mg + j * NW * 1024);
+            if constexpr (!GPL) {
+#pragma unroll
+                for (int j = 0; j < PG; j++) {
+                    const int q = (wave + NW * j) * PPG + pg;
+                    const bool ok = (rel_g[j] != DEAD) & (y0 + (q >> 4) < H) & (x0 + (q & 15) < W);
+                    dma16(ok ? gbase + rel_g[j] : DEAD, rg, mg + j * NW * 1024);
+                }
             }
 #pragma unroll
             for (int j = 0; j < PX; j++) {
@@ -136,7 +167,17 @@
         }
         if (++itx == tiles_x) { itx = 0; ++ity; }
     };
+    auto wait_n = [&](int n) {
+#define DGE_WN(N) case N: asm volatile("s_waitcnt vmcnt(%0)" :: "i"(N) : "memory"); break
+        switch (n < 0 ? 0 : n) {
+            DGE_WN(0); DGE_WN(1); DGE_WN(2); DGE_WN(3); DGE_WN(4); DGE_WN(5); DGE_WN(6); DGE_WN(7); DGE_WN(8); DGE_WN(9); DGE_WN(10); DGE_WN(11);
+            DGE_WN(12); DGE_WN(13); DGE_WN(14); DGE_WN(15); DGE_WN(16);
+            default: asm volatile("s_waitcnt vmcnt(16)" ::: "memory"); break;
+        }
+#undef DGE_WN
+    };
     auto wait_tile = [&](int nfly) {
+        if constexpr (GPL) return;
         const bool full = pw_mine == C::PW;
 #define DGE_W(N) asm volatile("s_waitcnt vmcnt(%0)" :: "i"(N) : "memory")
         if (nfly <= 0) DGE_W(0);
@@ -173,8 +214,34 @@
         __syncthreads();
     };
 
+    const int ppx = tid >> 2, pcg = tid & 3, pyl = ppx >> 3, pxl = ppx & 7;
+    const bool p_unit = GPL && ppx < (TH / 2) * 8;
+    auto pg_expand = [&](int stg, int gbuf) {
+        if (!p_unit) return;
+        const unsigned char* sp = lds + stg * C::STAGE_P;
+        const uint4 pgv = *(const uint4*)(sp + wave * 1024 + lane * 16);
+        const unsigned pmv = *(const unsigned*)(sp + C::PGB_PAD + wave * 256 + (lane >> 2) * 16 + (lane & 3) * 4);
+        float f[8];
+        unpack16(pgv, f, (bf16_t*)nullptr);
+#pragma unroll
+        for (int e = 0; e < 8; e++) f[e] *= gp.gscale;
+        unsigned char* base = lds + NS * C::STAGE_P + gbuf * C::GBYTES + ((2 * pyl) * 16 + 2 * pxl) * GP + pcg * 16;
+#pragma unroll
+        for (int q = 0; q < 4; q++) {
+            float o[8];
+#pragma unroll
+            for (int e = 0; e < 8; e++) o[e] = f[e] * (((pmv >> (q * 8 + e)) & 1u) ? 1.f : gp.gslope);
+            *(uint4*)(base + ((q >> 1) * 16 + (q & 1)) * GP) = pack16(o, (bf16_t*)nullptr);
+        }
+    };
+    static_assert(!GPL || (GP == 64 && TH % 4 == 0 && C::NPW <= NW && (TH / 2) * 8 * 4 <= NT), "pooled form: 32-channel g tiles, one unit per thread");
 #pragma unroll
     for (int s = 0; s < NS - 1; s++) if (t_begin + s < t_end) issue(s);
+    if constexpr (GPL) {
+        const int yg = t_end - 1 - t_begin;
+        wait_n((yg < NS - 2 ? yg : NS - 2) * pw_mine);
+        pg_expand(0, 0);
+    }
     int stage = 0;
 #ifdef DGE_WG_TIMING
     const bool tlogon = lin == 40 && tid == 0;
@@ -183,13 +250,16 @@
         const int younger = t_end - 1 - t;
         DGE_WT(0);
         wait_tile(younger < NS - 2 ? younger : NS - 2);
+        if constexpr (GPL) {
+            asm volatile("s_waitcnt lgkmcnt(0)" ::: "memory");
+        }
         DGE_WT(1);
         __syncthreads();
         DGE_WT(2);
         if (t + NS - 1 < t_end) issue(stage == 0 ? NS - 1 : stage - 1);
         DGE_WT(3);
-        const unsigned char* sg = lds + stage * C::STAGE;
-        const unsigned char* sx = sg + C::GBYTES;
+        const unsigned char* sg = GPL ? lds + NS * C::STAGE_P + ((t - t_begin) & 1) * C::GBYTES : lds + stage * C::STAGE;
+        const unsigned char* sx = GPL ? lds + stage * C::STAGE_P + C::PGB_PAD + 1024 : sg + C::GBYTES;
         const int y0 = cty * TH, x0 = ctx * 16;
         const bool edge_tile = (y0 == 0) | (y0 + TH >= H) | (x0 == 0) | (x0 + 16 >= W);
         uint4 av[2];
@@ -256,6 +326,13 @@
         asm volatile("s_nop 0" :: "v"(acc[0][0]), "v"(acc[8][15]));
 #endif
         DGE_WT(4);
+        if constexpr (GPL) {
+            if (t + 1 < t_end) {
+                const int yg = t_end - 1 - (t + 1);
+                wait_n((yg < NS - 2 ? yg : NS - 2) * pw_mine);
+                pg_expand(stage + 1 == NS ? 0 : stage + 1, (t + 1 - t_begin) & 1);
+            }
+        }
         if (++ctx == tiles_x) { ctx = 0; ++cty; }
         stage = stage + 1 == NS ? 0 : stage + 1;
     }
@@ -321,17 +398,17 @@
     }
 }
 
-template <class C>
+template <class C, bool GPL = false>
 int launch(const void* g, const void* x, const float* sc, const float* sh, float* dw, int B, int H, int W, int cout, int cin,
-           const float* wdot, float* dots, int dots_slots, hipStream_t s) {
+           const float* wdot, float* dots, int dots_slots, hipStream_t s, GPool gp = GPool{nullptr, nullptr, 0.f, 0.f}) {
     const int tx = (W + 15) / 16, ty = (H + C::TH - 1) / C::TH;
     const int tps = tx * ty;
     const int noi = ((cout + 31) / 32) * ((cin + 31) / 32);
-    const int lds_bytes = C::lds_bytes();
+    const int lds_bytes = GPL ? C::lds_bytes_p() : C::lds_bytes();
     static int attr_bytes[16] = {0};
     int dev = 0;
     (void)hipGetDevice(&dev);
-    auto kern = wgrad_dma_kernel<C>;
+    auto kern = wgrad_dma_kernel<C, GPL>;
     if (dev < 0 || dev >= 16 || attr_bytes[dev] < lds_bytes) {
         const hipError_t e = hipFuncSetAttribute((const void*)kern, hipFuncAttributeMaxDynamicSharedMemorySize, lds_bytes);
         if (e != hipSuccess) {
@@ -351,7 +428,7 @@
     if (!dge_det_fits(noi, (long long)B * gps, 1024 * 9)) return 1;
     dge_note_kernel("wgrad_dma<%d,%d,%d,%d>", C::TH, C::GP, C::XP, C::NS);
     hipLaunchKernelGGL(kern, dim3(noi, groups8), dim3(C::NW * 64), lds_bytes, s, (const bf16_t*)g, (const bf16_t*)x, sc, sh, dw, B, H, W,
-                       cout, cin, tx, ty, per, gps, wdot, dots, dots_slots < 1 ? 1 : dots_slots);
+                       cout, cin, tx, ty, per, gps, wdot, dots, dots_slots < 1 ? 1 : dots_slots, gp);
     DGE_LAUNCH_CHECK("wgrad_dma");
     return 0;
 }
@@ -363,6 +440,26 @@
     return (int)hipMemcpyFromSymbol(out, HIP_SYMBOL(wg_tlog), (size_t)n * sizeof(long long), 0, hipMemcpyDeviceToHost);
 }
 #endif
+bool dge_wgrad_dma_pooled_ok(int B, int H, int W, int cout, int cin) {
+    static int off = -1;
+    if (off < 0) off = getenv("DGE_NO_WGRAD_DMA") ? 1 : 0;
+    if (off || H % 2 || W % 2) return false;
+    if (!(cout == 32 && cin == 16)) return false;
+    if (!dge_det_fits(1LL << 40, 1, 1)) return false;
+    if ((size_t)H * W * cout * 2 >= (1u << 30) || (size_t)H * W * cin * 2 >= (1u << 30)) return false;
+    const int tps = ((W + 15) / 16) * ((H + 15) / 16);
+    const int noi = ((cout + 31) / 32) * ((cin + 31) / 32);
+    return tps >= 16 && noi * B <= 1024;
+}
+int dge_wgrad_dma_pooled(const void* gup, const unsigned* mask, float scale, float slope, const void* x, const float* sc, const float* sh,
+                         float* dw, int B, int H, int W, int cout, int cin, const float* wdot, float* dots, int dots_slots, hipStream_t s) {
+    if (!dge_wgrad_dma_pooled_ok(B, H, W, cout, cin) || !sc || !wdot) { dge_set_error("wgrad_dma: pooled-gradient form not offered for this launch"); return -1; }
+    const GPool gp{(const bf16_t*)gup, mask, scale, slope};
+    const int r = launch<WCfg<16, 64, 32, 4, 2>, true>(nullptr, x, sc, sh, dw, B, H, W, cout, cin, wdot, dots, dots_slots, s, gp);
+    if (r == 1) { dge_set_error("wgrad_dma: pooled-gradient form refused after its predicate held"); return -1; }
+    return r;
+}
+
 int dge_wgrad_dma_try(const void* g, const void* x, const float* sc, const float* sh, float* dw, int B, int H, int W, int cout, int cin,
                       const float* wdot, float* dots, int dots_slots, hipStream_t s) {
     static int off = -1;
diff --git a/deep-gan-encoders_amd/ops.py b/deep-gan-encoders_amd/ops.py
--- a/deep-gan-encoders_amd/ops.py
+++ b/deep-gan-encoders_amd/ops.py
@@ -439,8 +439,12 @@
 def conv2d(x, w_packed, cout, ksize=3, up=False, in_scale=None, in_shift=None, out_scale=None, bias=None,
            bias_scale=1.0, noise=None, noise_w=None, act=ACT_NONE, gain=1.0, addend=None, add_scale=1.0, stats=None,
            out=None, in_s2d=False, dot_src=None, in_up2=False, in_relu=False, prep=None, relu_mask=None, in_t2d=False, rgb=None, pool_out=False, pool_mask=False,
-           in_bwd=None):
+           in_bwd=None, x_pool=None):
     B, H, W, Cin = x.shape
+    if x_pool is not None:
+        if in_bwd is None or in_bwd.get("red") is None or in_bwd.get("fr") is not None:
+            raise DgeError("conv2d: x_pool goes with in_bwd and its reductions")
+        H, W = 2 * H, 2 * W
     if in_s2d:
         H, W, Cin = H // 2, W // 2, Cin * 4
     if in_up2:
@@ -493,6 +497,8 @@
             d.fr_out = _f32(in_bwd["fr"].buf)
         elif in_bwd.get("red") is not None:
             d.prep_stats = _f32(in_bwd["red"].alloc(d.stats_slots))
+            if x_pool is not None:
+                d.x_pool_mask, d.x_pool_scale, d.x_pool_slope = _p(x_pool[0]), float(x_pool[1]), float(x_pool[2])
         else:
             d.prep_noise = None
             d.in_bwd_extra, d.in_bwd_extra_scale = _p(in_bwd.get("extra")), float(in_bwd.get("extra_scale", 1.0))
@@ -519,6 +525,10 @@
 
 def conv_in_bwd_supported(B, H, W, cin, cout, dtype):
     return bool(lib().dge_conv_in_bwd_supported(int(B), int(H), int(W), int(cin), int(cout), 3, int(dtype)))
+
+
+def conv2_pooled_supported(B, H, W, c2, cc, dtype):
+    return bool(lib().dge_conv2_pooled_supported(int(B), int(H), int(W), int(c2), int(cc), int(dtype)))
 
 
 def conv_in_bwd_x_supported(B, H, W, cin, cout, dtype):
@@ -794,9 +804,16 @@
     return dw
 
 
-def conv_wgrad_dots(g, x, dw, in_scale, in_shift, w, dots):
+def conv_wgrad_dots(g, x, dw, in_scale, in_shift, w, dots, g_pool=None):
     B, H, W, Cin = x.shape
     cout = dw.shape[0]
+    if g_pool is not None:
+        nslot = max(1, min(16, (H * W) // 4096))
+        buf = dots.alloc(nslot)
+        check(lib().dge_conv_wgrad_dots_pooled(_p(g), _p(g_pool[0]), float(g_pool[1]), float(g_pool[2]), _p(x), _f32(in_scale), _f32(in_shift),
+                                               _f32(dw), _f32(w.detach()), _f32(buf), nslot, B, H, W, cout, Cin, dtype_of(x), _stream()),
+              "dge_conv_wgrad_dots_pooled")
+        return True
     if dw.shape[2] != 3 or is_deterministic():
         return False
     nslot = max(1, min(16, (H * W) // 4096))
@@ -853,10 +870,10 @@
     return gpre
 
 
-def act_bwd_mask(gup, mask, noise, scale=1.0, red=None, slope=0.2, planar=False, defer=None):
+def act_bwd_mask(gup, mask, noise, scale=1.0, red=None, slope=0.2, planar=False, defer=None, store=True):
     B, UH, UW, Cc = gup.shape
     H, W = 2 * UH, 2 * UW
-    gpre = torch.empty((B, H, W, Cc), dtype=gup.dtype, device=gup.device)
+    gpre = torch.empty((B, H, W, Cc), dtype=gup.dtype, device=gup.device) if store else None
     ncol = 2 if red is None else (red.shape[0] if planar else red.shape[-1])
     part = zeros((B, Cc, ncol), gup.device) if red is not None else None
     check(lib().dge_act_bwd_mask(_p(gup), _p(mask), _f32(noise), _p(gpre), _f32(part), ncol, B, H, W, Cc, float(scale), float(slope),
diff --git a/include/dge_hip.h b/include/dge_hip.h
--- a/include/dge_hip.h
+++ b/include/dge_hip.h
@@ -74,6 +74,8 @@
     float in_bwd_extra_scale;
     const float* fr_img4;
     float* fr_out;
+    const unsigned* x_pool_mask;
+    float x_pool_scale, x_pool_slope;
 } dge_conv_desc;
 int dge_conv2d(const dge_conv_desc* d, dge_stream_t stream);
 int dge_conv_small_supported(int H, int W, int cin, int ntot, int ksize, int in_s2d, int in_up2, int dtype);
@@ -113,6 +115,7 @@
 
 int dge_conv_rgb_supported(int B, int H, int W, int Cin, int Cout, int ksize, int dtype);
 int dge_conv_in_bwd_supported(int B, int H, int W, int Cin, int Cout, int ksize, int dtype);
+int dge_conv2_pooled_supported(int B, int H, int W, int c2, int cc, int dtype);
 int dge_conv_in_bwd_fromrgb_supported(int B, int H, int W, int Cin, int Cout, int ksize, int dtype);
 int dge_conv_in_bwd_x_supported(int B, int H, int W, int Cin, int Cout, int ksize, int dtype);
 int dge_conv_pool_supported(int B, int H, int W, int Cin, int Cout, int ksize, int dtype);
@@ -192,6 +195,9 @@
                    int cout, int cin, int ksize, int dtype, dge_stream_t stream);
 int dge_conv_wgrad_dots(const void* g, const void* x, const float* in_scale, const float* in_shift, float* dw, const float* w,
                         float* dots, int dots_slots, int B, int H, int W, int cout, int cin, int dtype, dge_stream_t stream);
+int dge_conv_wgrad_dots_pooled(const void* gup, const unsigned* mask, float scale, float slope, const void* x, const float* in_scale,
+                               const float* in_shift, float* dw, const float* w, float* dots, int dots_slots, int B, int H, int W,
+                               int cout, int cin, int dtype, dge_stream_t stream);
 int dge_act_bwd(const void* gup, const void* a, const float* noise, void* gpre, float* red, int red_cols, int B, int H, int W, int C,
                 int pool, float scale, float slope, int dtype, dge_stream_t stream);
 int dge_blend_pool_mask(const void* x, const void* z, void* y, float* stats, unsigned* mask, int B, int OH, int OW, int C, float alpha,
```

Result: no change. 383.6 images/sec (median of 6 runs) (+0.9%).
